# MingyuKim87/Safe_Denoiser

Hardware: AMD Instinct MI355X
Metric: images/sec (512x512, 50 steps, SD-v1.4 + repellency) (higher is better)
Workload: dtype bf16; 1 GPU; README-default end to end (safree = svf = lra = true, safree_neg_prompt_config.json:26-28): token ids -> CLIP -> SAFREE projection -> DDPM 50 steps x UNet on 3 guidance branches with per-prompt text switching + safe_denoiser.yaml repellency (kernel_fast, M=515, sigma 3.15, scale .33, margin 1.6, window 780<=t<=1000) -> VAE decode -> uint8 512x512 images; SD-v1.4 UNet / CLIP / VAE with random weigh; guidance_branches=3, text_encoder_precision=bf16x3, prompts_per_batch=64, latent_repeat=3, renoise_draws_rank0=3520, parallelism=prompt-shard x1

## Files before the change

### include/sdn.h

```cpp
#ifndef SDN_H_
#define SDN_H_

#include <stddef.h>
#include <stdint.h>

#ifdef __cplusplus
extern "C" {
#endif

#define SDN_OK            0
#define SDN_E_INVALID    -1
#define SDN_E_LAUNCH     -2
#define SDN_E_WORKSPACE  -3
#define SDN_E_ARCH       -4

int sdn_abi_version(void);
const char* sdn_device_arch_host(void);


#define SDN_REPEL_RBF     0
#define SDN_REPEL_SPARSE  1
#define SDN_QNORM_NONE    0
#define SDN_QNORM_CHANNEL 1
#define SDN_OUT_REPELLED  0
#define SDN_OUT_NEG       1

typedef struct sdn_repel_params {
  int32_t n_query;
  int32_t n_ref;
  int32_t channels;
  int32_t hw;
  int32_t weight_fn;
  int32_t qnorm;
  float   sigma;
  float   radius;
  float   scale;
  float   epsilon;
  float   gate;
} sdn_repel_params;

size_t sdn_repel_workspace_bytes(int32_t n_query, int32_t n_ref, int32_t channels, int32_t hw);

int sdn_repel_apply(const sdn_repel_params* p_host, float* x, const float* proj_ref,
                    float* out_neg, float* out_den, int32_t* out_isneg,
                    void* workspace, size_t workspace_bytes, void* stream);

int sdn_repel_calibrate(const sdn_repel_params* p_host, const float* queries, const float* proj_ref,
                        float* out, void* workspace, size_t workspace_bytes, void* stream);


int sdn_cfg_combine(const float* model_out, int32_t n_prompt, int32_t n_branch, int64_t d,
                    float guidance_scale, float* eps, void* stream);

int sdn_sld_guidance(const float* model_out, int32_t n_prompt, int64_t d, float guidance_scale,
                     float sld_guidance_scale, float sld_threshold, float sld_momentum_scale, float sld_mom_beta,
                     int32_t apply_safety, float* momentum, float* eps, void* stream);

int sdn_cfg_combine_rows(const float* model_out, int32_t n_prompt, int32_t n_branch, int64_t d,
                         const float* guidance_rows, float* eps, void* stream);
int sdn_sld_guidance_rows(const float* model_out, int32_t n_prompt, int64_t d, const float* guidance_rows,
                          float sld_guidance_scale, float sld_threshold, float sld_momentum_scale, float sld_mom_beta,
                          int32_t apply_safety, float* momentum, float* eps, void* stream);

int sdn_pred_x0(const float* x, const float* eps, int64_t n, float sqrt_ac, float sqrt_one_minus_ac,
                float clip, float* x0, void* stream);

int sdn_sched_step(const float* x, const float* eps, const float* noise, int64_t n,
                   float sqrt_ac, float sqrt_one_minus_ac, float c_x0, float c_x, float c_eps, float sigma,
                   float clip, float* prev, void* stream);

int sdn_add_noise(const float* x0, const float* noise, int64_t n, float sqrt_ac, float sqrt_one_minus_ac,
                  float* out, void* stream);

int sdn_renoise_select(float* latents, const float* x0r, const float* noise, const int32_t* isneg,
                       int32_t n_prompt, int64_t d, float sqrt_ac, float sqrt_one_minus_ac, void* stream);

int sdn_flow_euler_step(const float* x, const float* v, int64_t n, float sigma, float sigma_next,
                        float* prev, void* stream);

int sdn_flow_endpoints(const float* x, const float* v, int64_t n, float sigma, float* x0, float* x1, void* stream);
int sdn_flow_renoise(const float* x0r, const float* x1, const float* z, int64_t n, float sigma_next,
                     float* out, void* stream);


#define SDN_A_PLAIN    0
#define SDN_A_CONV3X3  1
#define SDN_ACT_NONE   0
#define SDN_ACT_SILU   1
#define SDN_ACT_GEGLU  2
#define SDN_ACT_GELU_TANH 3
#define SDN_ACT_QUICK_GELU 4
#define SDN_ACT_GEGLU_TANH 5
#define SDN_ACT_GELU      7
#define SDN_ACT_RELU      9
#define SDN_OUT_BF16      0
#define SDN_OUT_F32       1
#define SDN_OUT_F32_NCHW  2

typedef struct sdn_gemm_desc {
  int32_t M, N, K;
  int32_t a_mode;
  int32_t K1;
  int32_t Hs, Ws, Cin;
  int32_t Ho, Wo, stride;
  int32_t upsample;
  int32_t act;
  int32_t out_kind;
  int32_t rows_per_batch;
  int32_t ld_rowbias;
  int32_t ld_rowgate;
  int32_t residual_bcast;
  int32_t n_valid;
  int32_t ldc;
  int32_t asym_pad;
  int32_t split_k;
  int32_t res_pre;
  int32_t x3_out;
  int32_t f32_stream;
} sdn_gemm_desc;

int sdn_gemm_bf16(const sdn_gemm_desc* d_host, const void* a, const void* a2, const void* w,
                  const float* bias, const float* rowbias, const float* rowgate, const void* residual, void* out,
                  void* stream);
int sdn_gemm_f16(const sdn_gemm_desc* d_host, const void* a, const void* a2, const void* w,
                 const float* bias, const float* rowbias, const float* rowgate, const void* residual, void* out,
                 void* stream);

int sdn_groupnorm_bf16(const void* x, const void* x2, int32_t batch, int32_t hw, int32_t c1, int32_t c2,
                       int32_t groups, float eps, int32_t silu, const float* gamma, const float* beta,
                       void* out, float* stats_ws, void* stream);
int sdn_groupnorm_f16(const void* x, const void* x2, int32_t batch, int32_t hw, int32_t c1, int32_t c2,
                      int32_t groups, float eps, int32_t silu, const float* gamma, const float* beta,
                      void* out, float* stats_ws, void* stream);

int sdn_layernorm_bf16(const void* x, int64_t rows, int32_t c, float eps, const float* gamma,
                       const float* beta, void* out, void* stream);
int sdn_layernorm_f16(const void* x, int64_t rows, int32_t c, float eps, const float* gamma,
                      const float* beta, void* out, void* stream);

int sdn_attention_bf16(const void* q, const void* k, const void* v, void* out, int32_t batch, int32_t heads,
                       int32_t nq, int32_t nk, int32_t head_dim, int32_t ldq, int32_t ldk, int32_t ldv,
                       int32_t ldo, float scale, void* stream);
int sdn_attention_f16(const void* q, const void* k, const void* v, void* out, int32_t batch, int32_t heads,
                      int32_t nq, int32_t nk, int32_t head_dim, int32_t ldq, int32_t ldk, int32_t ldv,
                      int32_t ldo, float scale, void* stream);

typedef struct sdn_attn_segment2 {
  const void* q2; const void* k2; const void* v2; void* out2;
  int32_t n1, ldq2, ldk2, ldv2, ldo2;
} sdn_attn_segment2;
int sdn_joint_attention(int32_t dtype, const void* q, const void* k, const void* v, void* out,
                        const sdn_attn_segment2* seg2_host, int32_t batch, int32_t heads, int32_t n_total,
                        int32_t head_dim, int32_t ldq, int32_t ldk, int32_t ldv, int32_t ldo, float scale,
                        void* stream);

int sdn_layernorm_mod_bf16(const void* x, int64_t rows, int32_t c, float eps, const float* scale, const float* shift,
                           int32_t ld_mod, int32_t rows_per_batch, void* out, void* stream);
int sdn_layernorm_mod_f16(const void* x, int64_t rows, int32_t c, float eps, const float* scale, const float* shift,
                          int32_t ld_mod, int32_t rows_per_batch, void* out, void* stream);

int sdn_patchify_bf16(const float* latents, int32_t batch, int32_t c, int32_t h, int32_t w, int32_t p, void* out, void* stream);
int sdn_patchify_f16(const float* latents, int32_t batch, int32_t c, int32_t h, int32_t w, int32_t p, void* out, void* stream);
int sdn_unpatchify_f32(const float* tokens, int32_t batch, int32_t c, int32_t h, int32_t w, int32_t p, float* out, void* stream);

int sdn_conv_in_bf16(const float* latents_nchw, const void* w, const float* bias, int32_t batch, int32_t cin,
                     int32_t h, int32_t wd, int32_t cout, void* out_nhwc, void* stream);
int sdn_conv_in_f16(const float* latents_nchw, const void* w, const float* bias, int32_t batch, int32_t cin,
                    int32_t h, int32_t wd, int32_t cout, void* out_nhwc, void* stream);

int sdn_timestep_embed_bf16(float timestep, int32_t batch, int32_t dim, void* out, void* stream);
int sdn_timestep_embed_f16(float timestep, int32_t batch, int32_t dim, void* out, void* stream);

int sdn_gemm_f32(const sdn_gemm_desc* d_host, const void* a, const void* a2, const void* w,
                 const float* bias, const float* rowbias, const float* rowgate, const void* residual, void* out,
                 void* stream);
int sdn_groupnorm_f32(const void* x, const void* x2, int32_t batch, int32_t hw, int32_t c1, int32_t c2,
                      int32_t groups, float eps, int32_t silu, const float* gamma, const float* beta,
                      void* out, float* stats_ws, void* stream);
int sdn_layernorm_f32(const void* x, int64_t rows, int32_t c, float eps, const float* gamma,
                      const float* beta, void* out, void* stream);
int sdn_attention_f32(const void* q, const void* k, const void* v, void* out, int32_t batch, int32_t heads,
                      int32_t nq, int32_t nk, int32_t head_dim, int32_t ldq, int32_t ldk, int32_t ldv,
                      int32_t ldo, float scale, void* stream);
int sdn_conv_in_f32(const float* latents_nchw, const void* w, const float* bias, int32_t batch, int32_t cin,
                    int32_t h, int32_t wd, int32_t cout, void* out_nhwc, void* stream);
int sdn_timestep_embed_f32(float timestep, int32_t batch, int32_t dim, void* out, void* stream);

int sdn_gemm_x3(const sdn_gemm_desc* d_host, const void* a, const void* a2, const void* w,
                const float* bias, const float* rowbias, const float* rowgate, const void* residual, void* out,
                void* stream);
int sdn_attention_x3(const void* q, const void* k, const void* v, void* out, int32_t batch, int32_t heads,
                     int32_t nq, int32_t nk, int32_t head_dim, int32_t ldq, int32_t ldk, int32_t ldv,
                     int32_t ldo, float scale, void* stream);

int sdn_layernorm_mod_f32(const void* x, int64_t rows, int32_t c, float eps, const float* scale, const float* shift,
                          int32_t ld_mod, int32_t rows_per_batch, void* out, void* stream);
int sdn_patchify_f32(const float* latents, int32_t batch, int32_t c, int32_t h, int32_t w, int32_t p, void* out, void* stream);
int sdn_joint_attention_f32(int32_t mode, const void* q, const void* k, const void* v, void* out,
                            const sdn_attn_segment2* seg2_host, int32_t batch, int32_t heads, int32_t n_total,
                            int32_t head_dim, int32_t ldq, int32_t ldk, int32_t ldv, int32_t ldo, float scale,
                            void* stream);

int sdn_split3(const float* x, const float* x2, int64_t rows, int32_t c1, int32_t c2, void* out_triple, void* stream);
int sdn_expand3_weights(const float* w, int64_t rows, int32_t cols, int32_t group, void* out_bf16, void* stream);
int sdn_groupnorm_f32_triple(const void* x, const void* x2, int32_t batch, int32_t hw, int32_t c1, int32_t c2, int32_t groups,
                             float eps, int32_t silu, const float* gamma, const float* beta, void* out_triple, float* stats_ws,
                             void* stream);
int sdn_layernorm_f32_triple(const void* x, int64_t rows, int32_t c, float eps, const float* gamma, const float* beta,
                             void* out_triple, void* stream);
int sdn_attention_x3_triple(const void* q, const void* k, const void* v, void* out_triple, int32_t batch, int32_t heads, int32_t nq,
                            int32_t nk, int32_t head_dim, int32_t ldq, int32_t ldk, int32_t ldv, int32_t ldo, float scale,
                            void* stream);
int sdn_attention_x3_pairs(const void* q, const void* k, const void* v, int32_t lo_offset_q, int32_t lo_offset_kv, void* out,
                           int32_t batch, int32_t heads, int32_t nq, int32_t nk, int32_t head_dim, int32_t ldq, int32_t ldk,
                           int32_t ldv, int32_t ldo, float scale, int32_t triple_out, void* stream);

int sdn_randn_philox_plan(int64_t numel, int32_t* grid_out, int64_t* offset_increment_out);
int sdn_randn_philox(const uint64_t* seeds, const uint64_t* offsets, const int32_t* rows, int32_t n_gen, int64_t numel,
                     float* out, void* stream);
int sdn_randn_philox_state(const uint64_t* seeds, uint64_t* offsets, const int32_t* flags, int32_t n_gen, int64_t numel,
                           float* out, void* stream);

typedef struct sdn_unet_config {
  int32_t in_channels, out_channels, sample_size;
  int32_t n_levels;
  int32_t block_out_channels[4];
  int32_t level_has_attn[4];
  int32_t layers_per_block;
  int32_t n_heads;
  int32_t cross_dim, text_len;
  int32_t norm_groups;
  int32_t dtype;
  int32_t latent_repeat;
} sdn_unet_config;

typedef struct sdn_unet sdn_unet;

#define SDN_P_VEC_F32     0
#define SDN_P_MAT         1
#define SDN_P_CONV3X3     2
#define SDN_P_GEGLU_MAT   3
#define SDN_P_GEGLU_VEC   4
#define SDN_P_POS_CROP    5
#define SDN_P_GLU_VALUE   7
#define SDN_P_GLU_GATE    8
#define SDN_P_DERIVED     6

typedef struct sdn_param_info {
  char     name[128];
  int32_t  kind;
  int32_t  rows, cols;
  int32_t  rows_padded;
  int64_t  offset;
} sdn_param_info;

int    sdn_unet_create(const sdn_unet_config* cfg_host, sdn_unet** out_host);
void   sdn_unet_destroy(sdn_unet* u);
int    sdn_unet_param_count(const sdn_unet* u);
int    sdn_unet_param_info(const sdn_unet* u, int32_t index, sdn_param_info* info_host);
size_t sdn_unet_weight_bytes(const sdn_unet* u);
size_t sdn_unet_workspace_bytes(sdn_unet* u, int32_t batch);
double sdn_unet_flops(sdn_unet* u, int32_t batch, double* attention_core_flops_host);

int sdn_unet_forward(sdn_unet* u, const void* weights, const float* latents, float timestep, const void* text,
                     float* out, int32_t batch, void* workspace, size_t workspace_bytes, void* stream);

typedef struct sdn_mmdit_config {
  int32_t in_channels, out_channels;
  int32_t sample_size, patch_size;
  int32_t num_layers;
  int32_t num_heads, head_dim;
  int32_t joint_dim, pooled_dim;
  int32_t text_len;
  int32_t time_dim;
  int32_t dtype;
} sdn_mmdit_config;
int sdn_mmdit_create(const sdn_mmdit_config* cfg_host, sdn_unet** out_host);
int sdn_mmdit_forward(sdn_unet* m, const void* weights, const float* latents, float timestep, const void* text,
                      const void* pooled, float* out, int32_t batch, void* workspace, size_t workspace_bytes,
                      void* stream);

int sdn_ln_fold(int32_t dtype, const void* w, const float* gamma, const float* beta, const float* bias, int32_t rows,
                int32_t cols, void* w_folded, float* c, float* d, void* stream);
int sdn_gemm_ln_bf16(const sdn_gemm_desc* desc, const void* a, const void* w_folded, const float* c, const float* d, float eps,
                     const float* row_stats, void* out, void* stream);
int sdn_gemm_ln_f16(const sdn_gemm_desc* desc, const void* a, const void* w_folded, const float* c, const float* d, float eps,
                    const float* row_stats, void* out, void* stream);
int sdn_row_stats_bf16(const void* x, int64_t rows, int32_t c, float eps, float* out, void* stream);
int sdn_row_stats_f16(const void* x, int64_t rows, int32_t c, float eps, float* out, void* stream);

int sdn_ffn_geglu_fused(int32_t dtype, int64_t M, int32_t C, const void* x, const float* row_stats, const void* w1_folded,
                        const float* c1, const float* d1, const void* w_cat, const float* b_cat, const void* residual, void* out,
                        float* col_stats, void* stream);

int sdn_gemm_k320(int32_t dtype, const sdn_gemm_desc* desc, const void* a, const void* w, const float* bias, const float* ln_c,
                  const float* ln_d, float ln_eps, const void* residual, void* out, void* stream);
int32_t sdn_gemm_k320_map(int32_t grid, int32_t col_groups, int32_t wg, int32_t* stream_out, int32_t* group_out);

int sdn_gemm_stats_bf16(const sdn_gemm_desc* desc, const void* a, const void* a2, const void* w, const float* bias,
                        const float* rowbias, const void* residual, void* out, float* col_stats, void* stream);
int sdn_gemm_stats_f16(const sdn_gemm_desc* desc, const void* a, const void* a2, const void* w, const float* bias,
                       const float* rowbias, const void* residual, void* out, float* col_stats, void* stream);
int sdn_groupnorm_cols_bf16(const void* x, const void* x2, int32_t batch, int32_t hw, int32_t c1, int32_t c2, int32_t groups,
                            float eps, int32_t silu, const float* gamma, const float* beta, void* out, float* stats_ws,
                            const float* cols1, const float* cols2, void* stream);
int sdn_groupnorm_cols_f16(const void* x, const void* x2, int32_t batch, int32_t hw, int32_t c1, int32_t c2, int32_t groups,
                           float eps, int32_t silu, const float* gamma, const float* beta, void* out, float* stats_ws,
                           const float* cols1, const float* cols2, void* stream);

int sdn_gemm_splitk_bf16(const sdn_gemm_desc* d, const void* a, const void* a2, const void* w, const float* bias,
                         const float* rowbias, const float* rowgate, const void* residual, void* out, void* partials,
                         size_t partial_bytes, void* stream);
int sdn_gemm_splitk_f16(const sdn_gemm_desc* d, const void* a, const void* a2, const void* w, const float* bias,
                        const float* rowbias, const float* rowgate, const void* residual, void* out, void* partials,
                        size_t partial_bytes, void* stream);

int sdn_conv_up4_weights(int32_t dtype, const void* w9, int32_t N, int32_t Cin, void* out, void* stream);

int sdn_repeat(const void* in, size_t bytes, int32_t rep, void* out, void* stream);

int sdn_unet_prepare(sdn_unet* u, void* weights, void* stream);

typedef struct sdn_vae_config {
  int32_t latent_channels, out_channels;
  int32_t sample_size;
  int32_t n_levels;
  int32_t block_out_channels[4];
  int32_t layers_per_block;
  int32_t norm_groups;
  int32_t dtype;
} sdn_vae_config;
int sdn_vae_decoder_create(const sdn_vae_config* cfg_host, sdn_unet** out_host);
int sdn_vae_decode(sdn_unet* vae, const void* weights, const float* latents, float latent_scale, float* image,
                   int32_t batch, void* workspace, size_t workspace_bytes, void* stream);
int sdn_vae_encoder_create(const sdn_vae_config* cfg_host, sdn_unet** out_host);
int sdn_vae_encode(sdn_unet* vae_encoder, const void* weights, const float* image, float* moments, int32_t batch,
                   void* workspace, size_t workspace_bytes, void* stream);
int sdn_gaussian_sample(const float* moments, const float* noise, int32_t batch, int32_t latent_channels, int32_t hw,
                        float scale, float* out, void* stream);
int sdn_image_postprocess(const float* image_nchw, int32_t batch, int32_t channels, int32_t height, int32_t width,
                          float* out_nhwc01, uint8_t* out_nhwc_u8, void* stream);
int sdn_latent_mix(const float* z, const float* w, const float* bias, int32_t batch, int32_t channels, int32_t hw,
                   float in_scale, float* out, void* stream);
int sdn_softmax_rows(int32_t dtype, const float* scores, int64_t ld_scores, int64_t rows, int32_t n, float scale,
                     void* out, int64_t ld_out, void* stream);
int sdn_transpose16(const void* in, int32_t rows, int32_t cols, int64_t ld_in, void* out, int64_t ld_out, void* stream);
int sdn_transpose32(const void* in, int32_t rows, int32_t cols, int64_t ld_in, void* out, int64_t ld_out, void* stream);

typedef struct sdn_clip_config {
  int32_t vocab_size;
  int32_t hidden_size, intermediate_size;
  int32_t num_layers, num_heads;
  int32_t max_position_embeddings;
  int32_t dtype;
} sdn_clip_config;
int sdn_clip_create(const sdn_clip_config* cfg_host, sdn_unet** out_host);
int sdn_clip_forward(sdn_unet* clip, const void* weights, const int32_t* input_ids, const int32_t* attention_mask,
                     void* last_hidden_state, int32_t batch, void* workspace, size_t workspace_bytes, void* stream);
int sdn_clip_embed(int32_t dtype, const int32_t* input_ids, const void* token_embedding, const void* position_embedding,
                   int64_t rows, int32_t seq_len, int32_t hidden, int32_t vocab, void* out, void* stream);
int sdn_masked_attention(int32_t dtype, const void* q, const void* k, const void* v, void* out, const int32_t* key_mask,
                         int32_t causal, int32_t batch, int32_t heads, int32_t n, int32_t head_dim, int32_t ldq,
                         int32_t ldk, int32_t ldv, int32_t ldo, float scale, void* stream);
int sdn_clip_embed_f32(const int32_t* input_ids, const void* token_embedding, const void* position_embedding, int64_t rows,
                       int32_t seq_len, int32_t hidden, int32_t vocab, void* out, void* stream);
int sdn_masked_attention_f32(const void* q, const void* k, const void* v, void* out, const int32_t* key_mask, int32_t causal,
                             int32_t batch, int32_t heads, int32_t n, int32_t head_dim, int32_t ldq, int32_t ldk, int32_t ldv,
                             int32_t ldo, float scale, void* stream);

typedef struct sdn_clip_proj_config {
  int32_t vocab_size;
  int32_t hidden_size, intermediate_size;
  int32_t num_layers, num_heads;
  int32_t max_position_embeddings;
  int32_t dtype;
  int32_t projection_dim;
  int32_t act;
  int32_t eos_token_id;
  int32_t hidden_tap;
} sdn_clip_proj_config;
int sdn_clip_proj_create(const sdn_clip_proj_config* cfg_host, sdn_unet** out_host);
int sdn_clip_proj_forward(sdn_unet* clip, const void* weights, const int32_t* input_ids, void* hidden, int64_t hidden_batch_stride,
                          int64_t hidden_row_stride, void* text_embeds, int64_t embeds_row_stride, int32_t batch, void* workspace,
                          size_t workspace_bytes, void* stream);
int sdn_clip_eos_rows(int32_t dtype, const int32_t* input_ids, const void* x, const float* gamma, const float* beta, int32_t batch,
                      int32_t seq_len, int32_t hidden, int32_t vocab, int32_t eos_token_id, float eps, void* out,
                      int32_t* positions, void* stream);
int sdn_copy_rows_strided(const void* src, int32_t batch, int32_t rows_per_batch, int32_t cols, int32_t elem_bytes, void* dst,
                          int64_t dst_batch_stride, int64_t dst_row_stride, void* stream);

typedef struct sdn_clip_vision_config {
  int32_t image_size, patch_size;
  int32_t hidden_size, intermediate_size;
  int32_t num_layers, num_heads;
  int32_t projection_dim;
  int32_t act;
  int32_t dtype;
} sdn_clip_vision_config;
int sdn_clip_vision_create(const sdn_clip_vision_config* cfg_host, sdn_unet** out_host);
int sdn_clip_vision_forward(sdn_unet* vision, const void* weights, const float* pixel_values, void* last_hidden_state,
                            void* image_embeds, int32_t batch, void* workspace, size_t workspace_bytes, void* stream);
int sdn_clip_patch_rows(int32_t dtype, const float* pixels, int32_t batch, int32_t image_size, int32_t patch_size, int32_t kpad,
                        void* out, void* stream);
int sdn_clip_vision_embed(int32_t dtype, const void* patch_proj, const float* class_embedding, const void* position_embedding,
                          const float* gamma, const float* beta, int32_t batch, int32_t tokens, int32_t hidden, float eps, void* out,
                          void* stream);
int sdn_clip_class_rows(int32_t dtype, const void* x, const float* gamma, const float* beta, int32_t batch, int32_t seq_len,
                        int32_t hidden, float eps, void* out, void* stream);
int sdn_image_resize_u8(const uint8_t* in, int32_t batch, int32_t in_size, int32_t out_size, const int32_t* coeffs,
                        const int32_t* bounds, int32_t ksize, uint8_t* tmp, uint8_t* out, void* stream);
int sdn_clip_normalize_u8(const uint8_t* in, int32_t batch, int32_t size, float mean_r, float mean_g, float mean_b, float std_r,
                          float std_g, float std_b, float* out, void* stream);
int sdn_embed_row_scores(const void* x, int32_t dtype_x, int64_t ldx, const void* y, int32_t dtype_y, int64_t ldy,
                         int32_t y_rows, int32_t rows, int32_t dim, int32_t normalize_y, float scale, float bias,
                         float* out, void* stream);
int sdn_embed_cross_mean(const void* x, int32_t dtype_x, int64_t ldx, int32_t rx, const void* y, int32_t dtype_y, int64_t ldy,
                         int32_t ry, int32_t dim, float* scratch, float* out, void* stream);
int sdn_image_resize_rect_u8(const uint8_t* in, int32_t batch, int32_t in_h, int32_t in_w, int32_t out_h, int32_t out_w,
                             const int32_t* coeffs_x, const int32_t* bounds_x, int32_t ksize_x, const int32_t* coeffs_y,
                             const int32_t* bounds_y, int32_t ksize_y, uint8_t* tmp, uint8_t* out_u8, float* out_f32, float mean_r,
                             float mean_g, float mean_b, float std_r, float std_g, float std_b, void* stream);

typedef struct sdn_t5_config {
  int32_t vocab_size;
  int32_t d_model, d_kv, d_ff;
  int32_t num_layers, num_heads;
  int32_t num_buckets, max_distance;
  float   eps;
  int32_t dtype;
} sdn_t5_config;
int sdn_t5_create(const sdn_t5_config* cfg_host, sdn_unet** out_host);
size_t sdn_t5_workspace_bytes(sdn_unet* t5, int32_t batch, int32_t n);
double sdn_t5_flops(sdn_unet* t5, int32_t batch, int32_t n, double* attention_core_flops_host);
int sdn_t5_forward(sdn_unet* t5, const void* weights, const int32_t* input_ids, const int32_t* attention_mask, int32_t n,
                   void* out, int32_t batch, void* workspace, size_t workspace_bytes, void* stream);
int sdn_rmsnorm(int32_t dtype, const void* x, int32_t x_is_f32, int64_t rows, int32_t c, float eps, const float* weight, void* out,
                void* stream);
int sdn_embed_tokens(int32_t dtype, const int32_t* input_ids, const void* token_embedding, int64_t rows, int32_t hidden,
                     int32_t vocab, float* out, void* stream);
int sdn_t5_bucket(int32_t relative_position, int32_t num_buckets, int32_t max_distance);
int sdn_t5_relative_bias(int32_t dtype, const void* table, int32_t num_buckets, int32_t max_distance, int32_t heads, int32_t n,
                         float* out, void* stream);
int sdn_bias_attention(int32_t dtype, const void* q, const void* k, const void* v, void* out, const float* bias,
                       const int32_t* key_mask, int32_t batch, int32_t heads, int32_t n, int32_t head_dim, int32_t ldq,
                       int32_t ldk, int32_t ldv, int32_t ldo, float scale, void* stream);

void sdn_unet_set_text_version(sdn_unet* u, uint64_t version);

void sdn_unet_set_graph_mode(sdn_unet* u, int32_t on);
void sdn_unet_set_split_k(sdn_unet* u, int32_t on);
void sdn_unet_set_conv_up4(sdn_unet* u, int32_t on);

typedef struct sdn_inception_config {
  int32_t image_size;
  int32_t normalize_input;
  int32_t dtype;
} sdn_inception_config;
typedef struct sdn_inception_conv {
  char    name[64];
  int32_t cin, cout, kh, kw, stride, pad_h, pad_w;
  int32_t kpad, n_padded;
} sdn_inception_conv;
int sdn_inception_create(const sdn_inception_config* cfg_host, sdn_unet** out_host);
int sdn_inception_conv_count(const sdn_unet* inception);
int sdn_inception_conv_info(const sdn_unet* inception, int32_t index, sdn_inception_conv* info_host);
int sdn_inception_forward(sdn_unet* inception, const void* weights, const float* pixels, float* features, int32_t batch, int32_t h,
                          int32_t w, int32_t resize, void* workspace, size_t workspace_bytes, void* stream);
#define SDN_POOL_MAX        0
#define SDN_POOL_AVG_NOPAD  1
int sdn_patch_rows_f32(const float* in, int32_t batch, int32_t h, int32_t w, int32_t c, int32_t kh, int32_t kw, int32_t stride_h,
                       int32_t stride_w, int32_t pad_h, int32_t pad_w, int32_t kpad, float* out, void* stream);
int sdn_pool3_f32(int32_t mode, const float* in, int32_t batch, int32_t h, int32_t w, int32_t c, int32_t stride, int32_t pad,
                  float* out, int32_t ldo, int32_t c0, void* stream);
int sdn_resize_bilinear_f32(const float* in_nchw, int32_t batch, int32_t h, int32_t w, int32_t out_h, int32_t out_w, float scale,
                            float shift, float* out_nhwc, void* stream);
int sdn_spatial_mean_f32(const float* in, int32_t batch, int32_t hw, int32_t c, float* out, void* stream);

typedef struct sdn_profile_row {
  char    kernel[24];
  int32_t launches;
  double  ms;
  double  flops;
  double  bytes;
} sdn_profile_row;
void sdn_unet_profile_next(sdn_unet* u);
int  sdn_unet_profile_read(sdn_unet* u, sdn_profile_row* rows_host, int32_t max_rows);

#ifdef __cplusplus
}
#endif
#endif
```

### safe_denoiser_amd/_lib.py

```python
from __future__ import annotations

import ctypes as C
import os

import torch

_HERE = os.path.dirname(os.path.abspath(__file__))
_LIB = None


class SdnUnavailable(RuntimeError):
    """libsdn.so is missing/unloadable, or there is no gfx950 device for a compute call."""


class SdnError(RuntimeError):
    """A libsdn entry point returned a negative status."""


_ERR = {-1: "SDN_E_INVALID (bad shape / null or misaligned pointer)", -2: "SDN_E_LAUNCH", -3: "SDN_E_WORKSPACE",
        -4: "SDN_E_ARCH"}


def lib_path() -> str:
    return os.environ.get("SDN_LIB", os.path.join(_HERE, "libsdn.so"))


class RepelParams(C.Structure):
    _fields_ = [("n_query", C.c_int32), ("n_ref", C.c_int32), ("channels", C.c_int32), ("hw", C.c_int32),
                ("weight_fn", C.c_int32), ("qnorm", C.c_int32), ("sigma", C.c_float), ("radius", C.c_float),
                ("scale", C.c_float), ("epsilon", C.c_float), ("gate", C.c_float)]


class GemmDesc(C.Structure):
    _fields_ = [(n, C.c_int32) for n in ("M", "N", "K", "a_mode", "K1", "Hs", "Ws", "Cin", "Ho", "Wo", "stride",
                                         "upsample", "act", "out_kind", "rows_per_batch", "ld_rowbias", "ld_rowgate",
                                         "residual_bcast", "n_valid", "ldc", "asym_pad", "split_k", "res_pre", "x3_out",
                                         "f32_stream")]


class UnetConfig(C.Structure):
    _fields_ = [("in_channels", C.c_int32), ("out_channels", C.c_int32), ("sample_size", C.c_int32),
                ("n_levels", C.c_int32), ("block_out_channels", C.c_int32 * 4), ("level_has_attn", C.c_int32 * 4),
                ("layers_per_block", C.c_int32), ("n_heads", C.c_int32), ("cross_dim", C.c_int32),
                ("text_len", C.c_int32), ("norm_groups", C.c_int32), ("dtype", C.c_int32), ("latent_repeat", C.c_int32)]


class ProfileRow(C.Structure):
    _fields_ = [("kernel", C.c_char * 24), ("launches", C.c_int32), ("ms", C.c_double), ("flops", C.c_double),
                ("bytes", C.c_double)]


class MmditConfig(C.Structure):
    _fields_ = [(n, C.c_int32) for n in ("in_channels", "out_channels", "sample_size", "patch_size", "num_layers",
                                         "num_heads", "head_dim", "joint_dim", "pooled_dim", "text_len", "time_dim",
                                         "dtype")]


class VaeConfig(C.Structure):
    _fields_ = [("latent_channels", C.c_int32), ("out_channels", C.c_int32), ("sample_size", C.c_int32),
                ("n_levels", C.c_int32), ("block_out_channels", C.c_int32 * 4), ("layers_per_block", C.c_int32),
                ("norm_groups", C.c_int32), ("dtype", C.c_int32)]


class ClipConfig(C.Structure):
    _fields_ = [(n, C.c_int32) for n in ("vocab_size", "hidden_size", "intermediate_size", "num_layers", "num_heads",
                                         "max_position_embeddings", "dtype")]


class ClipProjConfig(C.Structure):
    _fields_ = [(n, C.c_int32) for n in ("vocab_size", "hidden_size", "intermediate_size", "num_layers", "num_heads",
                                         "max_position_embeddings", "dtype", "projection_dim", "act", "eos_token_id", "hidden_tap")]


class ClipVisionConfig(C.Structure):
    _fields_ = [(n, C.c_int32) for n in ("image_size", "patch_size", "hidden_size", "intermediate_size", "num_layers", "num_heads",
                                         "projection_dim", "act", "dtype")]


class InceptionConfig(C.Structure):
    _fields_ = [(n, C.c_int32) for n in ("image_size", "normalize_input", "dtype")]


class InceptionConv(C.Structure):
    _fields_ = [("name", C.c_char * 64)] + [(n, C.c_int32) for n in ("cin", "cout", "kh", "kw", "stride", "pad_h", "pad_w", "kpad",
                                                                     "n_padded")]


class T5Config(C.Structure):
    _fields_ = [(n, C.c_int32) for n in ("vocab_size", "d_model", "d_kv", "d_ff", "num_layers", "num_heads", "num_buckets",
                                         "max_distance")] + [("eps", C.c_float), ("dtype", C.c_int32)]


class AttnSegment2(C.Structure):
    _fields_ = [("q2", C.c_void_p), ("k2", C.c_void_p), ("v2", C.c_void_p), ("out2", C.c_void_p), ("n1", C.c_int32),
                ("ldq2", C.c_int32), ("ldk2", C.c_int32), ("ldv2", C.c_int32), ("ldo2", C.c_int32)]


class ParamInfo(C.Structure):
    _fields_ = [("name", C.c_char * 128), ("kind", C.c_int32), ("rows", C.c_int32), ("cols", C.c_int32),
                ("rows_padded", C.c_int32), ("offset", C.c_int64)]


_vp, _i32, _i64, _f32, _sz = C.c_void_p, C.c_int32, C.c_int64, C.c_float, C.c_size_t

SIGNATURES = {
    "sdn_abi_version": (C.c_int, []),
    "sdn_device_arch_host": (C.c_char_p, []),
    "sdn_repel_workspace_bytes": (_sz, [_i32, _i32, _i32, _i32]),
    "sdn_repel_apply": (C.c_int, [C.POINTER(RepelParams), _vp, _vp, _vp, _vp, _vp, _vp, _sz, _vp]),
    "sdn_repel_calibrate": (C.c_int, [C.POINTER(RepelParams), _vp, _vp, _vp, _vp, _sz, _vp]),
    "sdn_cfg_combine": (C.c_int, [_vp, _i32, _i32, _i64, _f32, _vp, _vp]),
    "sdn_sld_guidance": (C.c_int, [_vp, _i32, _i64, _f32, _f32, _f32, _f32, _f32, _i32, _vp, _vp, _vp]),
    "sdn_cfg_combine_rows": (C.c_int, [_vp, _i32, _i32, _i64, _vp, _vp, _vp]),
    "sdn_sld_guidance_rows": (C.c_int, [_vp, _i32, _i64, _vp, _f32, _f32, _f32, _f32, _i32, _vp, _vp, _vp]),
    "sdn_pred_x0": (C.c_int, [_vp, _vp, _i64, _f32, _f32, _f32, _vp, _vp]),
    "sdn_sched_step": (C.c_int, [_vp, _vp, _vp, _i64, _f32, _f32, _f32, _f32, _f32, _f32, _f32, _vp, _vp]),
    "sdn_add_noise": (C.c_int, [_vp, _vp, _i64, _f32, _f32, _vp, _vp]),
    "sdn_renoise_select": (C.c_int, [_vp, _vp, _vp, _vp, _i32, _i64, _f32, _f32, _vp]),
    "sdn_flow_euler_step": (C.c_int, [_vp, _vp, _i64, _f32, _f32, _vp, _vp]),
    "sdn_flow_endpoints": (C.c_int, [_vp, _vp, _i64, _f32, _vp, _vp, _vp]),
    "sdn_flow_renoise": (C.c_int, [_vp, _vp, _vp, _i64, _f32, _vp, _vp]),
    "sdn_gemm_bf16": (C.c_int, [C.POINTER(GemmDesc), _vp, _vp, _vp, _vp, _vp, _vp, _vp, _vp, _vp]),
    "sdn_gemm_f16": (C.c_int, [C.POINTER(GemmDesc), _vp, _vp, _vp, _vp, _vp, _vp, _vp, _vp, _vp]),
    "sdn_ln_fold": (C.c_int, [_i32, _vp, _vp, _vp, _vp, _i32, _i32, _vp, _vp, _vp, _vp]),
    "sdn_gemm_ln_bf16": (C.c_int, [C.POINTER(GemmDesc), _vp, _vp, _vp, _vp, _f32, _vp, _vp, _vp]),
    "sdn_gemm_ln_f16": (C.c_int, [C.POINTER(GemmDesc), _vp, _vp, _vp, _vp, _f32, _vp, _vp, _vp]),
    "sdn_row_stats_bf16": (C.c_int, [_vp, _i64, _i32, _f32, _vp, _vp]),
    "sdn_row_stats_f16": (C.c_int, [_vp, _i64, _i32, _f32, _vp, _vp]),
    "sdn_ffn_geglu_fused": (C.c_int, [_i32, _i64, _i32, _vp, _vp, _vp, _vp, _vp, _vp, _vp, _vp, _vp, _vp, _vp]),
    "sdn_gemm_k320": (C.c_int, [_i32, C.POINTER(GemmDesc), _vp, _vp, _vp, _vp, _vp, _f32, _vp, _vp, _vp]),
    "sdn_gemm_k320_map": (_i32, [_i32, _i32, _i32, C.POINTER(_i32), C.POINTER(_i32)]),
    "sdn_gemm_stats_bf16": (C.c_int, [C.POINTER(GemmDesc), _vp, _vp, _vp, _vp, _vp, _vp, _vp, _vp, _vp]),
    "sdn_gemm_stats_f16": (C.c_int, [C.POINTER(GemmDesc), _vp, _vp, _vp, _vp, _vp, _vp, _vp, _vp, _vp]),
    "sdn_groupnorm_cols_bf16": (C.c_int, [_vp, _vp, _i32, _i32, _i32, _i32, _i32, _f32, _i32, _vp, _vp, _vp, _vp, _vp, _vp, _vp]),
    "sdn_groupnorm_cols_f16": (C.c_int, [_vp, _vp, _i32, _i32, _i32, _i32, _i32, _f32, _i32, _vp, _vp, _vp, _vp, _vp, _vp, _vp]),
    "sdn_gemm_splitk_bf16": (C.c_int, [C.POINTER(GemmDesc), _vp, _vp, _vp, _vp, _vp, _vp, _vp, _vp, _vp, _sz, _vp]),
    "sdn_gemm_splitk_f16": (C.c_int, [C.POINTER(GemmDesc), _vp, _vp, _vp, _vp, _vp, _vp, _vp, _vp, _vp, _sz, _vp]),
    "sdn_groupnorm_bf16": (C.c_int, [_vp, _vp, _i32, _i32, _i32, _i32, _i32, _f32, _i32, _vp, _vp, _vp, _vp, _vp]),
    "sdn_groupnorm_f16": (C.c_int, [_vp, _vp, _i32, _i32, _i32, _i32, _i32, _f32, _i32, _vp, _vp, _vp, _vp, _vp]),
    "sdn_layernorm_f16": (C.c_int, [_vp, _i64, _i32, _f32, _vp, _vp, _vp, _vp]),
    "sdn_conv_in_f16": (C.c_int, [_vp, _vp, _vp, _i32, _i32, _i32, _i32, _i32, _vp, _vp]),
    "sdn_timestep_embed_f16": (C.c_int, [_f32, _i32, _i32, _vp, _vp]),
    "sdn_layernorm_bf16": (C.c_int, [_vp, _i64, _i32, _f32, _vp, _vp, _vp, _vp]),
    "sdn_attention_bf16": (C.c_int, [_vp, _vp, _vp, _vp, _i32, _i32, _i32, _i32, _i32, _i32, _i32, _i32, _i32, _f32,
                                     _vp]),
    "sdn_attention_f16": (C.c_int, [_vp, _vp, _vp, _vp, _i32, _i32, _i32, _i32, _i32, _i32, _i32, _i32, _i32, _f32,
                                    _vp]),
    "sdn_conv_in_bf16": (C.c_int, [_vp, _vp, _vp, _i32, _i32, _i32, _i32, _i32, _vp, _vp]),
    "sdn_timestep_embed_bf16": (C.c_int, [_f32, _i32, _i32, _vp, _vp]),
    "sdn_gemm_f32": (C.c_int, [C.POINTER(GemmDesc), _vp, _vp, _vp, _vp, _vp, _vp, _vp, _vp, _vp]),
    "sdn_groupnorm_f32": (C.c_int, [_vp, _vp, _i32, _i32, _i32, _i32, _i32, _f32, _i32, _vp, _vp, _vp, _vp, _vp]),
    "sdn_layernorm_f32": (C.c_int, [_vp, _i64, _i32, _f32, _vp, _vp, _vp, _vp]),
    "sdn_attention_f32": (C.c_int, [_vp, _vp, _vp, _vp, _i32, _i32, _i32, _i32, _i32, _i32, _i32, _i32, _i32, _f32, _vp]),
    "sdn_randn_philox_plan": (C.c_int, [C.c_int64, C.POINTER(C.c_int32), C.POINTER(C.c_int64)]),
    "sdn_randn_philox": (C.c_int, [_vp, _vp, _vp, _i32, C.c_int64, _vp, _vp]),
    "sdn_randn_philox_state": (C.c_int, [_vp, _vp, _vp, _i32, C.c_int64, _vp, _vp]),
    "sdn_gemm_x3": (C.c_int, [C.POINTER(GemmDesc), _vp, _vp, _vp, _vp, _vp, _vp, _vp, _vp, _vp]),
    "sdn_attention_x3": (C.c_int, [_vp, _vp, _vp, _vp, _i32, _i32, _i32, _i32, _i32, _i32, _i32, _i32, _i32, _f32, _vp]),
    "sdn_conv_in_f32": (C.c_int, [_vp, _vp, _vp, _i32, _i32, _i32, _i32, _i32, _vp, _vp]),
    "sdn_timestep_embed_f32": (C.c_int, [_f32, _i32, _i32, _vp, _vp]),
    "sdn_unet_create": (C.c_int, [C.POINTER(UnetConfig), C.POINTER(_vp)]),
    "sdn_unet_destroy": (None, [_vp]),
    "sdn_unet_param_count": (C.c_int, [_vp]),
    "sdn_unet_param_info": (C.c_int, [_vp, _i32, C.POINTER(ParamInfo)]),
    "sdn_unet_weight_bytes": (_sz, [_vp]),
    "sdn_unet_workspace_bytes": (_sz, [_vp, _i32]),
    "sdn_unet_flops": (C.c_double, [_vp, _i32, C.POINTER(C.c_double)]),
    "sdn_unet_forward": (C.c_int, [_vp, _vp, _vp, _f32, _vp, _vp, _i32, _vp, _sz, _vp]),
    "sdn_mmdit_create": (C.c_int, [C.POINTER(MmditConfig), C.POINTER(_vp)]),
    "sdn_mmdit_forward": (C.c_int, [_vp, _vp, _vp, _f32, _vp, _vp, _vp, _i32, _vp, _sz, _vp]),
    "sdn_joint_attention": (C.c_int, [_i32, _vp, _vp, _vp, _vp, C.POINTER(AttnSegment2), _i32, _i32, _i32, _i32, _i32,
                                      _i32, _i32, _i32, _f32, _vp]),
    "sdn_layernorm_mod_bf16": (C.c_int, [_vp, _i64, _i32, _f32, _vp, _vp, _i32, _i32, _vp, _vp]),
    "sdn_layernorm_mod_f16": (C.c_int, [_vp, _i64, _i32, _f32, _vp, _vp, _i32, _i32, _vp, _vp]),
    "sdn_patchify_bf16": (C.c_int, [_vp, _i32, _i32, _i32, _i32, _i32, _vp, _vp]),
    "sdn_patchify_f16": (C.c_int, [_vp, _i32, _i32, _i32, _i32, _i32, _vp, _vp]),
    "sdn_unpatchify_f32": (C.c_int, [_vp, _i32, _i32, _i32, _i32, _i32, _vp, _vp]),
    "sdn_layernorm_mod_f32": (C.c_int, [_vp, _i64, _i32, _f32, _vp, _vp, _i32, _i32, _vp, _vp]),
    "sdn_patchify_f32": (C.c_int, [_vp, _i32, _i32, _i32, _i32, _i32, _vp, _vp]),
    "sdn_joint_attention_f32": (C.c_int, [_i32, _vp, _vp, _vp, _vp, C.POINTER(AttnSegment2), _i32, _i32, _i32, _i32, _i32,
                                          _i32, _i32, _i32, _f32, _vp]),
    "sdn_repeat": (C.c_int, [_vp, _sz, _i32, _vp, _vp]),
    "sdn_vae_decoder_create": (C.c_int, [C.POINTER(VaeConfig), C.POINTER(_vp)]),
    "sdn_vae_decode": (C.c_int, [_vp, _vp, _vp, _f32, _vp, _i32, _vp, _sz, _vp]),
    "sdn_vae_encoder_create": (C.c_int, [C.POINTER(VaeConfig), C.POINTER(_vp)]),
    "sdn_vae_encode": (C.c_int, [_vp, _vp, _vp, _vp, _i32, _vp, _sz, _vp]),
    "sdn_gaussian_sample": (C.c_int, [_vp, _vp, _i32, _i32, _i32, _f32, _vp, _vp]),
    "sdn_image_postprocess": (C.c_int, [_vp, _i32, _i32, _i32, _i32, _vp, _vp, _vp]),
    "sdn_latent_mix": (C.c_int, [_vp, _vp, _vp, _i32, _i32, _i32, _f32, _vp, _vp]),
    "sdn_softmax_rows": (C.c_int, [_i32, _vp, _i64, _i64, _i32, _f32, _vp, _i64, _vp]),
    "sdn_transpose16": (C.c_int, [_vp, _i32, _i32, _i64, _vp, _i64, _vp]),
    "sdn_transpose32": (C.c_int, [_vp, _i32, _i32, _i64, _vp, _i64, _vp]),
    "sdn_clip_create": (C.c_int, [C.POINTER(ClipConfig), C.POINTER(_vp)]),
    "sdn_clip_forward": (C.c_int, [_vp, _vp, _vp, _vp, _vp, _i32, _vp, _sz, _vp]),
    "sdn_clip_embed": (C.c_int, [_i32, _vp, _vp, _vp, _i64, _i32, _i32, _i32, _vp, _vp]),
    "sdn_masked_attention": (C.c_int, [_i32, _vp, _vp, _vp, _vp, _vp, _i32, _i32, _i32, _i32, _i32, _i32, _i32, _i32, _i32,
                                       _f32, _vp]),
    "sdn_clip_proj_create": (C.c_int, [C.POINTER(ClipProjConfig), C.POINTER(_vp)]),
    "sdn_clip_proj_forward": (C.c_int, [_vp, _vp, _vp, _vp, _i64, _i64, _vp, _i64, _i32, _vp, _sz, _vp]),
    "sdn_clip_eos_rows": (C.c_int, [_i32, _vp, _vp, _vp, _vp, _i32, _i32, _i32, _i32, _i32, _f32, _vp, _vp, _vp]),
    "sdn_copy_rows_strided": (C.c_int, [_vp, _i32, _i32, _i32, _i32, _vp, _i64, _i64, _vp]),
    "sdn_clip_vision_create": (C.c_int, [C.POINTER(ClipVisionConfig), C.POINTER(_vp)]),
    "sdn_clip_vision_forward": (C.c_int, [_vp, _vp, _vp, _vp, _vp, _i32, _vp, _sz, _vp]),
    "sdn_clip_patch_rows": (C.c_int, [_i32, _vp, _i32, _i32, _i32, _i32, _vp, _vp]),
    "sdn_clip_vision_embed": (C.c_int, [_i32, _vp, _vp, _vp, _vp, _vp, _i32, _i32, _i32, _f32, _vp, _vp]),
    "sdn_clip_class_rows": (C.c_int, [_i32, _vp, _vp, _vp, _i32, _i32, _i32, _f32, _vp, _vp]),
    "sdn_image_resize_u8": (C.c_int, [_vp, _i32, _i32, _i32, _vp, _vp, _i32, _vp, _vp, _vp]),
    "sdn_clip_normalize_u8": (C.c_int, [_vp, _i32, _i32, _f32, _f32, _f32, _f32, _f32, _f32, _vp, _vp]),
    "sdn_image_resize_rect_u8": (C.c_int, [_vp, _i32, _i32, _i32, _i32, _i32, _vp, _vp, _i32, _vp, _vp, _i32, _vp, _vp, _vp, _f32, _f32,
                                           _f32, _f32, _f32, _f32, _vp]),
    "sdn_inception_create": (C.c_int, [C.POINTER(InceptionConfig), C.POINTER(_vp)]),
    "sdn_inception_conv_count": (C.c_int, [_vp]),
    "sdn_inception_conv_info": (C.c_int, [_vp, _i32, C.POINTER(InceptionConv)]),
    "sdn_inception_forward": (C.c_int, [_vp, _vp, _vp, _vp, _i32, _i32, _i32, _i32, _vp, _sz, _vp]),
    "sdn_patch_rows_f32": (C.c_int, [_vp, _i32, _i32, _i32, _i32, _i32, _i32, _i32, _i32, _i32, _i32, _i32, _vp, _vp]),
    "sdn_pool3_f32": (C.c_int, [_i32, _vp, _i32, _i32, _i32, _i32, _i32, _i32, _vp, _i32, _i32, _vp]),
    "sdn_resize_bilinear_f32": (C.c_int, [_vp, _i32, _i32, _i32, _i32, _i32, _f32, _f32, _vp, _vp]),
    "sdn_spatial_mean_f32": (C.c_int, [_vp, _i32, _i32, _i32, _vp, _vp]),
    "sdn_embed_row_scores": (C.c_int, [_vp, _i32, _i64, _vp, _i32, _i64, _i32, _i32, _i32, _i32, _f32, _f32, _vp, _vp]),
    "sdn_embed_cross_mean": (C.c_int, [_vp, _i32, _i64, _i32, _vp, _i32, _i64, _i32, _i32, _vp, _vp, _vp]),
    "sdn_t5_create": (C.c_int, [C.POINTER(T5Config), C.POINTER(_vp)]),
    "sdn_t5_workspace_bytes": (_sz, [_vp, _i32, _i32]),
    "sdn_t5_flops": (C.c_double, [_vp, _i32, _i32, C.POINTER(C.c_double)]),
    "sdn_t5_forward": (C.c_int, [_vp, _vp, _vp, _vp, _i32, _vp, _i32, _vp, _sz, _vp]),
    "sdn_rmsnorm": (C.c_int, [_i32, _vp, _i32, _i64, _i32, _f32, _vp, _vp, _vp]),
    "sdn_embed_tokens": (C.c_int, [_i32, _vp, _vp, _i64, _i32, _i32, _vp, _vp]),
    "sdn_t5_bucket": (C.c_int, [_i32, _i32, _i32]),
    "sdn_t5_relative_bias": (C.c_int, [_i32, _vp, _i32, _i32, _i32, _i32, _vp, _vp]),
    "sdn_bias_attention": (C.c_int, [_i32, _vp, _vp, _vp, _vp, _vp, _vp, _i32, _i32, _i32, _i32, _i32, _i32, _i32, _i32, _f32,
                                     _vp]),
    "sdn_split3": (C.c_int, [_vp, _vp, _i64, _i32, _i32, _vp, _vp]),
    "sdn_expand3_weights": (C.c_int, [_vp, _i64, _i32, _i32, _vp, _vp]),
    "sdn_groupnorm_f32_triple": (C.c_int, [_vp, _vp, _i32, _i32, _i32, _i32, _i32, _f32, _i32, _vp, _vp, _vp, _vp, _vp]),
    "sdn_layernorm_f32_triple": (C.c_int, [_vp, _i64, _i32, _f32, _vp, _vp, _vp, _vp]),
    "sdn_attention_x3_triple": (C.c_int, [_vp, _vp, _vp, _vp, _i32, _i32, _i32, _i32, _i32, _i32, _i32, _i32, _i32, _f32, _vp]),
    "sdn_attention_x3_pairs": (C.c_int, [_vp, _vp, _vp, _i32, _i32, _vp, _i32, _i32, _i32, _i32, _i32, _i32, _i32, _i32, _i32, _f32, _i32, _vp]),
    "sdn_clip_embed_f32": (C.c_int, [_vp, _vp, _vp, _i64, _i32, _i32, _i32, _vp, _vp]),
    "sdn_masked_attention_f32": (C.c_int, [_vp, _vp, _vp, _vp, _vp, _i32, _i32, _i32, _i32, _i32, _i32, _i32, _i32, _i32, _f32, _vp]),
    "sdn_unet_prepare": (C.c_int, [_vp, _vp, _vp]),
    "sdn_unet_set_graph_mode": (None, [_vp, _i32]),
    "sdn_unet_set_text_version": (None, [_vp, C.c_uint64]),
    "sdn_unet_set_split_k": (None, [_vp, _i32]),
    "sdn_unet_set_conv_up4": (None, [_vp, _i32]),
    "sdn_conv_up4_weights": (C.c_int, [_i32, _vp, _i32, _i32, _vp, _vp]),
    "sdn_unet_profile_next": (None, [_vp]),
    "sdn_unet_profile_read": (C.c_int, [_vp, C.POINTER(ProfileRow), _i32]),
}


def lib():
    global _LIB
    if _LIB is None:
        path = lib_path()
        if not os.path.exists(path):
            raise SdnUnavailable(f"{path} not found: build it with `python -c 'import __graft_entry__ as g; g.build()'` "
                                 f"(or `make -C safe_denoiser_amd/csrc`).  There is no CPU fallback.")
        try:
            handle = C.CDLL(path)
        except OSError as e:
            raise SdnUnavailable(f"cannot load {path}: {e}") from e
        for name, (res, args) in SIGNATURES.items():
            fn = getattr(handle, name)
            fn.restype, fn.argtypes = res, args
        _LIB = handle
    return _LIB


def check(rc: int, what: str):
    if rc != 0:
        raise SdnError(f"{what} failed: {_ERR.get(rc, rc)}")


def require_gpu():
    if not torch.cuda.is_available():
        raise SdnUnavailable("no GPU visible: the safe-denoiser hot path only runs on an MI355X (gfx950); "
                             "there is no CPU fallback")


def dptr(t: torch.Tensor | None, dtype=None) -> int | None:
    if t is None:
        return None
    if not t.is_cuda:
        raise SdnUnavailable("tensor is not on the GPU: libsdn takes device pointers only (no CPU fallback)")
    if not t.is_contiguous():
        raise SdnError("tensor must be contiguous")
    if dtype is not None and t.dtype != dtype:
        raise SdnError(f"expected {dtype}, got {t.dtype}")
    return t.data_ptr()


def stream_ptr() -> int:
    return torch.cuda.current_stream().cuda_stream
```

### safe_denoiser_amd/csrc/sdn_norm.hip

```cpp
#include "sdn_common.h"
#include "sdn_ops.h"

namespace sdn_norm_detail {

typedef __attribute__((ext_vector_type(4))) unsigned int u32x4;
constexpr int THREADS = 256;
constexpr int GN_MAX_TILES = 128;

template <typename T>
__device__ __forceinline__ void unpack8(const u32x4 v, float* f) {
  f[0] = T::to_f(v.x & 0xffff); f[1] = T::to_f(v.x >> 16); f[2] = T::to_f(v.y & 0xffff); f[3] = T::to_f(v.y >> 16);
  f[4] = T::to_f(v.z & 0xffff); f[5] = T::to_f(v.z >> 16); f[6] = T::to_f(v.w & 0xffff); f[7] = T::to_f(v.w >> 16);
}
template <typename T>
__device__ __forceinline__ u32x4 pack8(const float* f) {
  return (u32x4){T::pack2(f[0], f[1]), T::pack2(f[2], f[3]), T::pack2(f[4], f[5]), T::pack2(f[6], f[7])};
}
__device__ __forceinline__ float silu_f(float v) { return v / (1.f + __expf(-v)); }

template <typename T>
__global__ void __launch_bounds__(THREADS)
k_gn_stats(const unsigned short* __restrict__ x, const unsigned short* __restrict__ x2, int hw, int c1, int c2,
           int groups, int rows_per_tile, int ct, int nch, float* __restrict__ partials) {
  extern __shared__ float lds[];
  const int C = c1 + c2, cpg = C / groups;
  const int b = blockIdx.x, tile = blockIdx.y, ntiles = gridDim.y;
  const int rt = THREADS / ct;
  const int cl = threadIdx.x % ct, rl = threadIdx.x / ct;
  const int r_lo = tile * rows_per_tile, r_hi = min(hw, r_lo + rows_per_tile);
  if (rl < rt) {
    for (int q = 0; q < nch; ++q) {
      const int ch0 = (cl + q * ct) * 8;
      const unsigned short* src; int ld, cc;
      if (ch0 < c1) { src = x; ld = c1; cc = ch0; } else { src = x2; ld = c2; cc = ch0 - c1; }
      float s[8], ss[8];
#pragma unroll
      for (int e = 0; e < 8; ++e) { s[e] = 0.f; ss[e] = 0.f; }
      for (int r = r_lo + rl; r < r_hi; r += 4 * rt) {
        u32x4 v[4];
#pragma unroll
        for (int j = 0; j < 4; ++j) {
          const int rr = min(r + j * rt, r_hi - 1);
          v[j] = *reinterpret_cast<const u32x4*>(src + ((long)b * hw + rr) * ld + cc);
        }
#pragma unroll
        for (int j = 0; j < 4; ++j) {
          if (r + j * rt < r_hi) {
            float f[8];
            unpack8<T>(v[j], f);
#pragma unroll
            for (int e = 0; e < 8; ++e) { s[e] += f[e]; ss[e] = fmaf(f[e], f[e], ss[e]); }
          }
        }
      }
#pragma unroll
      for (int e = 0; e < 8; ++e) {
        lds[((long)rl * C + ch0 + e) * 2 + 0] = s[e];
        lds[((long)rl * C + ch0 + e) * 2 + 1] = ss[e];
      }
    }
  }
  __syncthreads();
  if (threadIdx.x < groups) {
    const int gidx = threadIdx.x;
    float s = 0.f, ss = 0.f;
    for (int r = 0; r < rt; ++r)
      for (int c = gidx * cpg; c < (gidx + 1) * cpg; ++c) {
        s += lds[((long)r * C + c) * 2 + 0];
        ss += lds[((long)r * C + c) * 2 + 1];
      }
    float* o = partials + (((long)b * ntiles + tile) * groups + gidx) * 2;
    o[0] = s; o[1] = ss;
  }
}

__global__ void __launch_bounds__(512)
k_gn_finalize(const float* __restrict__ partials, int ntiles, int groups, float n, float eps,
              float* __restrict__ stats) {
  __shared__ float sh[64][8][2];
  const int b = blockIdx.x, gi = threadIdx.x >> 3, part = threadIdx.x & 7;
  if (gi < groups) {
    float s = 0.f, ss = 0.f;
    for (int t = part; t < ntiles; t += 8) {
      const float* p = partials + (((long)b * ntiles + t) * groups + gi) * 2;
      s += p[0]; ss += p[1];
    }
    sh[gi][part][0] = s; sh[gi][part][1] = ss;
  }
  __syncthreads();
  if (gi < groups && part == 0) {
    float s = 0.f, ss = 0.f;
#pragma unroll
    for (int k = 0; k < 8; ++k) { s += sh[gi][k][0]; ss += sh[gi][k][1]; }
    const float mean = s / n;
    const float var = fmaxf(ss / n - mean * mean, 0.f);
    stats[((long)b * groups + gi) * 2 + 0] = mean;
    stats[((long)b * groups + gi) * 2 + 1] = rsqrtf(var + eps);
  }
}

__global__ void __launch_bounds__(256)
k_gn_finalize_cols(const float* __restrict__ cols1, const float* __restrict__ cols2, int blocks_per_sample, int c1, int c2,
                   int groups, float n, float eps, float* __restrict__ stats) {
  __shared__ float red[8];
  const int C = c1 + c2, cpg = C / groups, b = blockIdx.x, gi = blockIdx.y;
  const int total = blocks_per_sample * cpg;
  float s = 0.f, q = 0.f;
  for (int e = threadIdx.x; e < total; e += 256) {
    const int t = e / cpg, c = gi * cpg + (e - t * cpg);
    const bool second = c >= c1;
    const float* src = second ? cols2 : cols1;
    const int cw = second ? c2 : c1, cc = second ? c - c1 : c;
    const float2 v = *reinterpret_cast<const float2*>(src + 2 * (((long)b * blocks_per_sample + t) * cw + cc));
    s += v.x; q += v.y;
  }
  s = block_sum<4>(s, red);
  q = block_sum<4>(q, red + 4);
  if (threadIdx.x == 0) {
    const float mean = s / n;
    const float var = fmaxf(q / n - mean * mean, 0.f);
    stats[((long)b * groups + gi) * 2 + 0] = mean;
    stats[((long)b * groups + gi) * 2 + 1] = rsqrtf(var + eps);
  }
}

template <typename T>
__global__ void __launch_bounds__(THREADS)
k_gn_apply(const unsigned short* __restrict__ x, const unsigned short* __restrict__ x2, int hw, int c1, int c2,
           int groups, int rows_per_block, int silu, const float* __restrict__ gamma,
           const float* __restrict__ beta, const float* __restrict__ stats, unsigned short* __restrict__ out) {
  extern __shared__ float aff[];
  const int C = c1 + c2, cpg = C / groups, cchunks = C / 8;
  const int b = blockIdx.x;
  float* ca = aff; float* cb = aff + C;
  for (int c = threadIdx.x; c < C; c += THREADS) {
    const int gi = c / cpg;
    const float mean = stats[((long)b * groups + gi) * 2 + 0], rstd = stats[((long)b * groups + gi) * 2 + 1];
    const float a = rstd * gamma[c];
    ca[c] = a; cb[c] = beta[c] - mean * a;
  }
  __syncthreads();
  const int r_lo = blockIdx.y * rows_per_block, r_hi = min(hw, r_lo + rows_per_block);
  const long total = (long)(r_hi - r_lo) * cchunks;
  for (long e = threadIdx.x; e < total; e += THREADS) {
    const int r = r_lo + (int)(e / cchunks), ch0 = (int)(e % cchunks) * 8;
    const unsigned short* src; int ld, cc;
    if (ch0 < c1) { src = x; ld = c1; cc = ch0; } else { src = x2; ld = c2; cc = ch0 - c1; }
    const u32x4 v = *reinterpret_cast<const u32x4*>(src + ((long)b * hw + r) * ld + cc);
    float f[8];
    unpack8<T>(v, f);
    const float4 a0 = *reinterpret_cast<const float4*>(ca + ch0), a1 = *reinterpret_cast<const float4*>(ca + ch0 + 4);
    const float4 b0 = *reinterpret_cast<const float4*>(cb + ch0), b1 = *reinterpret_cast<const float4*>(cb + ch0 + 4);
    const float am[8] = {a0.x, a0.y, a0.z, a0.w, a1.x, a1.y, a1.z, a1.w};
    const float bm[8] = {b0.x, b0.y, b0.z, b0.w, b1.x, b1.y, b1.z, b1.w};
#pragma unroll
    for (int k = 0; k < 8; ++k) {
      const float y = fmaf(f[k], am[k], bm[k]);
      f[k] = silu ? silu_f(y) : y;
    }
    *reinterpret_cast<u32x4*>(out + ((long)b * hw + r) * C + ch0) = pack8<T>(f);
  }
}

template <typename T, int NQ, int R>
__global__ void __launch_bounds__(THREADS)
k_layernorm(const unsigned short* __restrict__ x, long rows, int C, float eps, const float* __restrict__ gamma,
            const float* __restrict__ beta, unsigned short* __restrict__ out, int mod, int rows_per_batch, int ld_mod) {
  const int lane = threadIdx.x & 63;
  const long row0 = ((long)blockIdx.x * 4 + (threadIdx.x >> 6)) * R;
  if (row0 >= rows) return;
  const int cchunks = C / 8;
  float f[R][NQ][8];
  float s[R];
#pragma unroll
  for (int r = 0; r < R; ++r) {
    s[r] = 0.f;
    const long row = row0 + r < rows ? row0 + r : rows - 1;
#pragma unroll
    for (int q = 0; q < NQ; ++q) {
      const int cc = lane + q * 64;
      if (cc < cchunks) {
        unpack8<T>(*reinterpret_cast<const u32x4*>(x + row * C + cc * 8), f[r][q]);
#pragma unroll
        for (int k = 0; k < 8; ++k) s[r] += f[r][q][k];
      }
    }
  }
  float mean[R], rstd[R];
#pragma unroll
  for (int r = 0; r < R; ++r) mean[r] = wave_sum(s[r]) / (float)C;
#pragma unroll
  for (int r = 0; r < R; ++r) {
    float ss = 0.f;
#pragma unroll
    for (int q = 0; q < NQ; ++q) {
      const int cc = lane + q * 64;
      if (cc < cchunks) {
#pragma unroll
        for (int k = 0; k < 8; ++k) { const float d = f[r][q][k] - mean[r]; ss = fmaf(d, d, ss); }
      }
    }
    s[r] = ss;
  }
#pragma unroll
  for (int r = 0; r < R; ++r) rstd[r] = rsqrtf(wave_sum(s[r]) / (float)C + eps);
#pragma unroll
  for (int q = 0; q < NQ; ++q) {
    const int cc = lane + q * 64;
    if (cc < cchunks) {
      float gm[8], bt[8];
      auto load_affine = [&](const float* gp, const float* bp) {
        const float4 g0 = *reinterpret_cast<const float4*>(gp + cc * 8), g1 = *reinterpret_cast<const float4*>(gp + cc * 8 + 4);
        const float4 b0 = *reinterpret_cast<const float4*>(bp + cc * 8), b1 = *reinterpret_cast<const float4*>(bp + cc * 8 + 4);
        gm[0] = g0.x; gm[1] = g0.y; gm[2] = g0.z; gm[3] = g0.w; gm[4] = g1.x; gm[5] = g1.y; gm[6] = g1.z; gm[7] = g1.w;
        bt[0] = b0.x; bt[1] = b0.y; bt[2] = b0.z; bt[3] = b0.w; bt[4] = b1.x; bt[5] = b1.y; bt[6] = b1.z; bt[7] = b1.w;
      };
      if (!mod) load_affine(gamma, beta);
#pragma unroll
      for (int r = 0; r < R; ++r) {
        const long row = row0 + r;
        if (row < rows) {
          if (mod) {
            const long b = row / rows_per_batch;
            load_affine(gamma + b * ld_mod, beta + b * ld_mod);
          }
          float y[8];
#pragma unroll
          for (int k = 0; k < 8; ++k) y[k] = (f[r][q][k] - mean[r]) * rstd[r] * (mod ? 1.f + gm[k] : gm[k]) + bt[k];
          *reinterpret_cast<u32x4*>(out + row * C + cc * 8) = pack8<T>(y);
        }
      }
    }
  }
}

template <typename T, int NQ, int R>
__global__ void __launch_bounds__(THREADS)
k_row_stats(const unsigned short* __restrict__ x, long rows, int C, float eps, float* __restrict__ out) {
  const int lane = threadIdx.x & 63;
  const long row0 = ((long)blockIdx.x * 4 + (threadIdx.x >> 6)) * R;
  if (row0 >= rows) return;
  const int cchunks = C / 8;
  float f[R][NQ][8];
  float s[R];
#pragma unroll
  for (int r = 0; r < R; ++r) {
    s[r] = 0.f;
    const long row = row0 + r < rows ? row0 + r : rows - 1;
#pragma unroll
    for (int q = 0; q < NQ; ++q) {
      const int cc = lane + q * 64;
      if (cc < cchunks) {
        unpack8<T>(*reinterpret_cast<const u32x4*>(x + row * C + cc * 8), f[r][q]);
#pragma unroll
        for (int k = 0; k < 8; ++k) s[r] += f[r][q][k];
      }
    }
  }
  float mean[R];
#pragma unroll
  for (int r = 0; r < R; ++r) mean[r] = wave_sum(s[r]) / (float)C;
#pragma unroll
  for (int r = 0; r < R; ++r) {
    float ss = 0.f;
#pragma unroll
    for (int q = 0; q < NQ; ++q) {
      const int cc = lane + q * 64;
      if (cc < cchunks) {
#pragma unroll
        for (int k = 0; k < 8; ++k) { const float d = f[r][q][k] - mean[r]; ss = fmaf(d, d, ss); }
      }
    }
    s[r] = ss;
  }
#pragma unroll
  for (int r = 0; r < R; ++r) {
    const float rstd = rsqrtf(wave_sum(s[r]) / (float)C + eps);
    if (lane == 0 && row0 + r < rows) *reinterpret_cast<float2*>(out + 2 * (row0 + r)) = make_float2(mean[r], rstd);
  }
}

template <typename T>
__global__ void __launch_bounds__(THREADS)
k_conv_in(const float* __restrict__ lat, const unsigned short* __restrict__ w, const float* __restrict__ bias,
          int B, int cin, int H, int W, int cout, int ldo, unsigned short* __restrict__ out) {
  extern __shared__ float wl[];
  const int kk = 9 * cin;
  for (int i = threadIdx.x; i < cout * kk; i += THREADS) {
    const int co = i / kk, k = i - co * kk;
    wl[((k * 2 + ((co >> 2) & 1)) * (cout / 8) + (co >> 3)) * 4 + (co & 3)] = T::to_f(w[i]);
  }
  __syncthreads();
  constexpr int PX = 4;
  const int cchunks = cout / 8;
  const int WQ = (W + PX - 1) / PX;
  const int total = B * H * WQ * cchunks;
  const int HWQ = H * WQ;
  for (int e = blockIdx.x * THREADS + threadIdx.x; e < total; e += gridDim.x * THREADS) {
    const int pq = e / cchunks, cc = e - pq * cchunks;
    const int b = pq / HWQ, rem = pq - b * HWQ;
    const int yh = rem / WQ, x0 = (rem - yh * WQ) * PX;
    float acc[PX][8];
    {
      const float4 b0 = *reinterpret_cast<const float4*>(bias + cc * 8), b1 = *reinterpret_cast<const float4*>(bias + cc * 8 + 4);
#pragma unroll
      for (int p = 0; p < PX; ++p) {
        acc[p][0] = b0.x; acc[p][1] = b0.y; acc[p][2] = b0.z; acc[p][3] = b0.w;
        acc[p][4] = b1.x; acc[p][5] = b1.y; acc[p][6] = b1.z; acc[p][7] = b1.w;
      }
    }
    const float* lb = lat + (long)b * cin * H * W;
    for (int c = 0; c < cin; ++c) {
      float v[3][PX + 2];
#pragma unroll
      for (int ty = 0; ty < 3; ++ty)
#pragma unroll
        for (int tx = 0; tx < PX + 2; ++tx) {
          const int iy = yh + ty - 1, ix = x0 + tx - 1;
          const bool ok = iy >= 0 && iy < H && ix >= 0 && ix < W;
          const float t = lb[((long)c * H + min(max(iy, 0), H - 1)) * W + min(max(ix, 0), W - 1)];
          v[ty][tx] = ok ? t : 0.f;
        }
#pragma unroll
      for (int tap = 0; tap < 9; ++tap) {
        const float4 w0 = *reinterpret_cast<const float4*>(&wl[(((tap * cin + c) * 2 + 0) * cchunks + cc) * 4]);
        const float4 w1 = *reinterpret_cast<const float4*>(&wl[(((tap * cin + c) * 2 + 1) * cchunks + cc) * 4]);
#pragma unroll
        for (int p = 0; p < PX; ++p) {
          const float x = v[tap / 3][tap % 3 + p];
          acc[p][0] = fmaf(x, w0.x, acc[p][0]); acc[p][1] = fmaf(x, w0.y, acc[p][1]);
          acc[p][2] = fmaf(x, w0.z, acc[p][2]); acc[p][3] = fmaf(x, w0.w, acc[p][3]);
          acc[p][4] = fmaf(x, w1.x, acc[p][4]); acc[p][5] = fmaf(x, w1.y, acc[p][5]);
          acc[p][6] = fmaf(x, w1.z, acc[p][6]); acc[p][7] = fmaf(x, w1.w, acc[p][7]);
        }
      }
    }
    const long pix0 = ((long)b * H + yh) * W + x0;
#pragma unroll
    for (int p = 0; p < PX; ++p)
      if (x0 + p < W) *reinterpret_cast<u32x4*>(out + (pix0 + p) * ldo + cc * 8) = pack8<T>(acc[p]);
  }
}

template <typename T>
__global__ void k_temb(float t_val, const float* __restrict__ t_dev, int B, int dim, unsigned short* __restrict__ out) {
  const float t = t_dev ? *t_dev : t_val;
  const int half = dim / 2;
  for (int i = blockIdx.x * blockDim.x + threadIdx.x; i < B * dim; i += gridDim.x * blockDim.x) {
    const int k = i % dim;
    const int kk = k < half ? k : k - half;
    const float f = expf(-9.210340371976184f * (float)kk / (float)half);
    const float a = t * f;
    const float v = k < half ? cosf(a) : sinf(a);
    out[i] = (unsigned short)(T::pack2(v, 0.f) & 0xffff);
  }
}

inline bool al16(const void* p) { return (reinterpret_cast<uintptr_t>(p) & 15) == 0; }


template <typename T>
int groupnorm_impl(const void* x, const void* x2, int32_t batch, int32_t hw, int32_t c1, int32_t c2, int32_t groups,
                   float eps, int32_t silu, const float* gamma, const float* beta, void* out, float* stats_ws,
                   void* stream, const float* cols1 = nullptr, const float* cols2 = nullptr) {
  if (!x || !gamma || !beta || !out || !stats_ws || batch < 0 || hw <= 0 || c1 <= 0 || c2 < 0 || groups <= 0 ||
      groups > 64)
    return SDN_E_INVALID;
  if (c2 > 0 && !x2) return SDN_E_INVALID;
  const int C = c1 + c2;
  if ((c1 & 7) || (c2 & 7) || C % groups != 0 || C > 4096) return SDN_E_INVALID;
  if (!al16(x) || (x2 && !al16(x2)) || !al16(out) || !al16(gamma) || !al16(beta)) return SDN_E_INVALID;
  if (batch == 0) return SDN_OK;
  const int cch = C / 8;
  int nch = (cch + THREADS - 1) / THREADS;
  while (cch % nch != 0) ++nch;
  const int ct = cch / nch;
  if (ct > THREADS) return SDN_E_INVALID;
  const int rt = THREADS / ct;
  int ntiles = (hw + 31) / 32;
  if (ntiles > GN_MAX_TILES) ntiles = GN_MAX_TILES;
  const int rows_per_tile = (hw + ntiles - 1) / ntiles;
  ntiles = (hw + rows_per_tile - 1) / rows_per_tile;
  hipStream_t st = (hipStream_t)stream;
  const size_t lds = (size_t)rt * C * 2 * sizeof(float);
  if (lds > 64 * 1024) return SDN_E_INVALID;
  if (cols1) {
    if ((hw & 127) || (c2 > 0 && !cols2)) return SDN_E_INVALID;
    record_norm_launch({2, T::kDtype, 0, 0, 0, 0, 0, 0, 0, 0, 1, 0});
    hipLaunchKernelGGL(k_gn_finalize_cols, dim3(batch, groups), dim3(256), 0, st, cols1, cols2, hw / 128, c1, c2, groups,
                       (float)hw * (float)(C / groups), eps, stats_ws);
  } else {
    float* partials = stats_ws + (size_t)batch * groups * 2;
    record_norm_launch({1, T::kDtype, 0, 0, nch, ct, ntiles, rows_per_tile, 0, 0, 0, 0});
    hipLaunchKernelGGL((k_gn_stats<T>), dim3(batch, ntiles), dim3(THREADS), lds, st, (const unsigned short*)x,
                       (const unsigned short*)x2, hw, c1, c2, groups, rows_per_tile, ct, nch, partials);
    hipLaunchKernelGGL(k_gn_finalize, dim3(batch), dim3(512), 0, st, partials, ntiles, groups,
                       (float)hw * (float)(C / groups), eps, stats_ws);
  }
  int rows_per_block = (256 * 8 * 16) / C;
  if (rows_per_block < 1) rows_per_block = 1;
  const int nblk = (hw + rows_per_block - 1) / rows_per_block;
  hipLaunchKernelGGL((k_gn_apply<T>), dim3(batch, nblk), dim3(THREADS), (size_t)2 * C * sizeof(float), st, (const unsigned short*)x,
                     (const unsigned short*)x2, hw, c1, c2, groups, rows_per_block, silu, gamma, beta, stats_ws,
                     (unsigned short*)out);
  return sdn_launch_status();
}

template <typename T>
int layernorm_impl(const void* x, int64_t rows, int32_t c, float eps, const float* gamma, const float* beta, void* out,
                   void* stream, int mod = 0, int rows_per_batch = 0, int ld_mod = 0) {
  if (!x || !gamma || !beta || !out || rows < 0 || c <= 0 || (c & 7) || c > 2048) return SDN_E_INVALID;
  if (!al16(x) || !al16(out) || !al16(gamma) || !al16(beta)) return SDN_E_INVALID;
  if (mod && (rows_per_batch <= 0 || ld_mod < c || (ld_mod & 3))) return SDN_E_INVALID;
  if (rows == 0) return SDN_OK;
#define SDN_LN_LAUNCH(NQ, R)                                                                                          \
  do { hipLaunchKernelGGL((k_layernorm<T, NQ, R>), dim3((unsigned)((rows + 4 * (R) - 1) / (4 * (R)))), dim3(THREADS), 0,      \
                     (hipStream_t)stream, (const unsigned short*)x, (long)rows, c, eps, gamma, beta, (unsigned short*)out, \
                     mod, rows_per_batch, ld_mod);                                                                     \
  record_norm_launch({mod ? 4 : 3, T::kDtype, NQ, R, 0, 0, 0, 0, 0, 0, 0, 0}); } while (0)
  if (c <= 512) SDN_LN_LAUNCH(1, 4);
  else if (c <= 1024) SDN_LN_LAUNCH(2, 2);
  else SDN_LN_LAUNCH(4, 1);
#undef SDN_LN_LAUNCH
  return sdn_launch_status();
}

template <typename T>
__global__ void __launch_bounds__(THREADS)
k_patchify(const float* __restrict__ lat, int B, int C, int H, int W, int p, unsigned short* __restrict__ out) {
  const int hp = H / p, wp = W / p, K = C * p * p;
  const long total = (long)B * hp * wp * K;
  for (long e = (long)blockIdx.x * THREADS + threadIdx.x; e < total; e += (long)gridDim.x * THREADS) {
    const int k = (int)(e % K);
    const long tok = e / K;
    const int px = k % p, py = (k / p) % p, c = k / (p * p);
    const int tx = (int)(tok % wp), ty = (int)((tok / wp) % hp), b = (int)(tok / ((long)wp * hp));
    const float v = lat[(((long)b * C + c) * H + ty * p + py) * W + tx * p + px];
    out[e] = (unsigned short)(T::pack2(v, 0.f) & 0xffff);
  }
}
__global__ void __launch_bounds__(THREADS)
k_unpatchify(const float* __restrict__ tok, int B, int C, int H, int W, int p, float* __restrict__ out) {
  const int hp = H / p, wp = W / p;
  const long total = (long)B * C * H * W;
  for (long e = (long)blockIdx.x * THREADS + threadIdx.x; e < total; e += (long)gridDim.x * THREADS) {
    const int x = (int)(e % W), y = (int)((e / W) % H), c = (int)((e / ((long)W * H)) % C), b = (int)(e / ((long)W * H * C));
    const long t = ((long)b * hp + y / p) * wp + x / p;
    out[e] = tok[t * (p * p * C) + ((y % p) * p + (x % p)) * C + c];
  }
}
template <typename T>
int patchify_impl(const float* lat, int32_t B, int32_t C, int32_t H, int32_t W, int32_t p, void* out, void* stream) {
  if (!lat || !out || B < 0 || C <= 0 || H <= 0 || W <= 0 || p <= 0 || H % p || W % p) return SDN_E_INVALID;
  if (B == 0) return SDN_OK;
  const long total = (long)B * C * H * W;
  long grid = (total + THREADS - 1) / THREADS;
  if (grid > 2048) grid = 2048;
  hipLaunchKernelGGL((k_patchify<T>), dim3((unsigned)grid), dim3(THREADS), 0, (hipStream_t)stream, lat, B, C, H, W, p,
                     (unsigned short*)out);
  return sdn_launch_status();
}

template <typename T>
int conv_in_impl(const float* lat, const void* w, const float* bias, int32_t batch, int32_t cin, int32_t h, int32_t wd,
                 int32_t cout, void* out, void* stream) {
  if (!lat || !w || !bias || !out || batch < 0 || cin <= 0 || cin > 16 || h <= 0 || wd <= 0 || cout <= 0 ||
      (cout & 7) || !al16(out))
    return SDN_E_INVALID;
  if (batch == 0) return SDN_OK;
  int chunk = (int)((64 * 1024) / ((size_t)9 * cin * sizeof(float))) & ~7;
  if (chunk < 8) return SDN_E_INVALID;
  if (chunk > cout) chunk = cout;
  if ((long)batch * h * wd * (chunk / 8) >= (1L << 31)) return SDN_E_INVALID;
  for (int co0 = 0; co0 < cout; co0 += chunk) {
    const int cc = cout - co0 < chunk ? cout - co0 : chunk;
    const size_t lds = (size_t)cc * 9 * cin * sizeof(float);
    const long total = (long)batch * h * ((wd + 3) / 4) * (cc / 8);
    long grid = (total + THREADS - 1) / THREADS;
    if (grid > 4096) grid = 4096;
    hipLaunchKernelGGL((k_conv_in<T>), dim3((unsigned)grid), dim3(THREADS), lds, (hipStream_t)stream, lat,
                       (const unsigned short*)w + (size_t)co0 * 9 * cin, bias + co0, batch, cin, h, wd, cc, cout,
                       (unsigned short*)out + co0);
  }
  return sdn_launch_status();
}

template <typename T>
int temb_impl(float timestep, int32_t batch, int32_t dim, void* out, void* stream, const float* t_dev = nullptr) {
  if (!out || batch < 0 || dim <= 0 || (dim & 1)) return SDN_E_INVALID;
  if (batch == 0) return SDN_OK;
  const int n = batch * dim;
  hipLaunchKernelGGL((k_temb<T>), dim3((n + 255) / 256), dim3(256), 0, (hipStream_t)stream, timestep, t_dev, batch, dim,
                     (unsigned short*)out);
  return sdn_launch_status();
}

template <typename T>
int row_stats_impl(const void* x, int64_t rows, int32_t c, float eps, float* out, void* stream) {
  if (!x || !out || rows < 0 || c <= 0 || (c & 7) || c > 2048 || !al16(x) || (reinterpret_cast<uintptr_t>(out) & 7)) return SDN_E_INVALID;
  if (rows == 0) return SDN_OK;
#define SDN_RS_LAUNCH(NQ, R)                                                                                          \
  do { hipLaunchKernelGGL((k_row_stats<T, NQ, R>), dim3((unsigned)((rows + 4 * (R) - 1) / (4 * (R)))), dim3(THREADS), 0,      \
                     (hipStream_t)stream, (const unsigned short*)x, (long)rows, c, eps, out);                            \
  record_norm_launch({5, T::kDtype, NQ, R, 0, 0, 0, 0, 0, 0, 0, 0}); } while (0)
  if (c <= 512) SDN_RS_LAUNCH(1, 4);
  else if (c <= 1024) SDN_RS_LAUNCH(2, 2);
  else SDN_RS_LAUNCH(4, 1);
#undef SDN_RS_LAUNCH
  return sdn_launch_status();
}

}

int sdn_temb_from_device(int dtype, const float* t_dev, int batch, int dim, void* out, void* stream) {
  if (!t_dev) return SDN_E_INVALID;
  return dtype == 1 ? sdn_norm_detail::temb_impl<SdnF16>(0.f, batch, dim, out, stream, t_dev)
                    : sdn_norm_detail::temb_impl<SdnBF16>(0.f, batch, dim, out, stream, t_dev);
}
namespace { __global__ void k_set_scalar(float* dst, float v) { *dst = v; } }
int sdn_set_scalar(float* dst, float v, void* stream) {
  if (!dst) return SDN_E_INVALID;
  hipLaunchKernelGGL(k_set_scalar, dim3(1), dim3(1), 0, (hipStream_t)stream, dst, v);
  return sdn_launch_status();
}
using namespace sdn_norm_detail;

static int g_last_norm_launch[SDN_NL_COUNT] = {0};
void record_norm_launch(const sdn_norm_launch& l) {
  const int v[SDN_NL_COUNT] = {l.kernel, l.dtype, l.nq, l.r, l.nch, l.ct, l.ntiles, l.rows_per_tile, l.rpc, l.nchunk, l.stats_src, l.triple};
  for (int i = 0; i < SDN_NL_COUNT; ++i) g_last_norm_launch[i] = v[i];
}
extern "C" void sdn_debug_norm_last_launch(int* out, int n) {
  for (int i = 0; out && i < n; ++i) out[i] = i < SDN_NL_COUNT ? g_last_norm_launch[i] : 0;
}

#define SDN_NORM_ENTRY(SUF, T)                                                                                          \
  extern "C" int sdn_groupnorm_##SUF(const void* x, const void* x2, int32_t batch, int32_t hw, int32_t c1, int32_t c2, \
                                     int32_t groups, float eps, int32_t silu, const float* gamma, const float* beta,   \
                                     void* out, float* stats_ws, void* stream) {                                        \
    return groupnorm_impl<T>(x, x2, batch, hw, c1, c2, groups, eps, silu, gamma, beta, out, stats_ws, stream);         \
  }                                                                                                                     \
  extern "C" int sdn_groupnorm_cols_##SUF(const void* x, const void* x2, int32_t batch, int32_t hw, int32_t c1,         \
                                          int32_t c2, int32_t groups, float eps, int32_t silu, const float* gamma,      \
                                          const float* beta, void* out, float* stats_ws, const float* cols1,            \
                                          const float* cols2, void* stream) {                                           \
    if (!cols1) return SDN_E_INVALID;                                                                                   \
    return groupnorm_impl<T>(x, x2, batch, hw, c1, c2, groups, eps, silu, gamma, beta, out, stats_ws, stream, cols1,    \
                             cols2);                                                                                    \
  }                                                                                                                     \
  extern "C" int sdn_layernorm_##SUF(const void* x, int64_t rows, int32_t c, float eps, const float* gamma,            \
                                     const float* beta, void* out, void* stream) {                                      \
    return layernorm_impl<T>(x, rows, c, eps, gamma, beta, out, stream);                                                \
  }                                                                                                                     \
  extern "C" int sdn_layernorm_mod_##SUF(const void* x, int64_t rows, int32_t c, float eps, const float* scale,        \
                                         const float* shift, int32_t ld_mod, int32_t rows_per_batch, void* out,        \
                                         void* stream) {                                                                \
    return layernorm_impl<T>(x, rows, c, eps, scale, shift, out, stream, 1, rows_per_batch, ld_mod);                    \
  }                                                                                                                     \
  extern "C" int sdn_patchify_##SUF(const float* lat, int32_t B, int32_t C, int32_t H, int32_t W, int32_t p, void* out, \
                                    void* stream) {                                                                     \
    return patchify_impl<T>(lat, B, C, H, W, p, out, stream);                                                           \
  }                                                                                                                     \
  extern "C" int sdn_conv_in_##SUF(const float* lat, const void* w, const float* bias, int32_t batch, int32_t cin,     \
                                   int32_t h, int32_t wd, int32_t cout, void* out, void* stream) {                      \
    return conv_in_impl<T>(lat, w, bias, batch, cin, h, wd, cout, out, stream);                                         \
  }                                                                                                                     \
  extern "C" int sdn_timestep_embed_##SUF(float timestep, int32_t batch, int32_t dim, void* out, void* stream) {       \
    return temb_impl<T>(timestep, batch, dim, out, stream);                                                             \
  }
SDN_NORM_ENTRY(bf16, SdnBF16)
SDN_NORM_ENTRY(f16, SdnF16)

extern "C" int sdn_row_stats_bf16(const void* x, int64_t rows, int32_t c, float eps, float* out, void* stream) {
  return sdn_norm_detail::row_stats_impl<SdnBF16>(x, rows, c, eps, out, stream);
}
extern "C" int sdn_row_stats_f16(const void* x, int64_t rows, int32_t c, float eps, float* out, void* stream) {
  return sdn_norm_detail::row_stats_impl<SdnF16>(x, rows, c, eps, out, stream);
}

extern "C" int sdn_unpatchify_f32(const float* tok, int32_t B, int32_t C, int32_t H, int32_t W, int32_t p, float* out,
                                  void* stream) {
  if (!tok || !out || B < 0 || C <= 0 || H <= 0 || W <= 0 || p <= 0 || H % p || W % p) return SDN_E_INVALID;
  if (B == 0) return SDN_OK;
  const long total = (long)B * C * H * W;
  long grid = (total + THREADS - 1) / THREADS;
  if (grid > 2048) grid = 2048;
  hipLaunchKernelGGL(k_unpatchify, dim3((unsigned)grid), dim3(THREADS), 0, (hipStream_t)stream, tok, B, C, H, W, p, out);
  return sdn_launch_status();
}
```

### safe_denoiser_amd/csrc/sdn_plan.h

```cpp
#pragma once
#include <stdio.h>
#include <string.h>

#include <map>
#include <set>
#include <string>
#include <tuple>
#include <vector>

#include "sdn_common.h"
#include "sdn_ops.h"

namespace sdn_plan {

enum ModelKind { UNET, MMDIT, VAE_DECODER, VAE_ENCODER, CLIP, CLIP_PROJ, T5, CLIP_VISION, INCEPTION };

enum Space { SP_NONE = 0, SP_W = 1, SP_WS = 2, SP_IN = 3, SP_TEXT = 4, SP_OUT = 5, SP_POOLED = 6, SP_KV = 7, SP_OUT2 = 8 };
struct Ref { int space = SP_NONE; int64_t off = 0; };

struct Call {
  const void* weights; void* workspace; size_t workspace_bytes; int32_t batch; void* stream;
  const void *in = nullptr, *text = nullptr, *pooled = nullptr;
  void *out = nullptr, *out2 = nullptr;
  float scalar = 0.f; int n = 0;
  const int32_t* mask = nullptr;
  int64_t out_bs = 0, out_rs = 0, out2_rs = 0;
  int64_t kv_base = 0;
  int in_h = 0, in_w = 0;
  Call(const void* w, void* ws, size_t ws_bytes, int32_t b, void* s) : weights(w), workspace(ws), workspace_bytes(ws_bytes), batch(b), stream(s) {}
  const char* operator()(const Ref& r) const {
    switch (r.space) {
      case SP_W: return (const char*)weights + r.off;
      case SP_WS: return (const char*)workspace + r.off;
      case SP_KV: return (const char*)workspace + kv_base + r.off;
      case SP_IN: return (const char*)in + r.off;
      case SP_TEXT: return (const char*)text + r.off;
      case SP_OUT: return (const char*)out + r.off;
      case SP_OUT2: return (const char*)out2 + r.off;
      case SP_POOLED: return (const char*)pooled + r.off;
      default: return nullptr;
    }
  }
};

enum OpKind { OP_TEMB, OP_CONV_IN, OP_GEMM, OP_GN, OP_LN, OP_ATTN, OP_PATCHIFY, OP_UNPATCHIFY, OP_LATENT_MIX, OP_SOFTMAX,
              OP_TRANSPOSE, OP_GAUSS, OP_REPEAT, OP_CLIP_EMBED, OP_MATTN, OP_ROWSTATS, OP_FFN, OP_SPLIT3,
              OP_RMSNORM, OP_EMBED, OP_T5_BIAS, OP_BATTN, OP_EOS_ROWS, OP_COPY_ROWS, OP_PATCH_ROWS, OP_VISION_EMBED, OP_CLASS_ROWS,
              OP_CONV_ROWS, OP_POOL3, OP_RESIZE, OP_SPATIAL_MEAN };

struct Op {
  int kind;
  sdn_gemm_desc gd;
  Ref a, a2, w, bias, rowbias, rowgate, residual, out, aux;
  Ref q2, k2, v2, out2;
  Ref col, cols1, cols2;
  Ref ln_c, ln_d, ln_stats;
  int ln = 0;
  int text_kv = 0;
  int x3t = 0;
  int pair_in = 0;
  int tri_out = 0;
  int dyn_ldc = 0;
  int k320 = 0;
  int n1 = 0, mod = 0, ld_mod = 0, patch = 0;
  int batch = 0, hw = 0, c1 = 0, c2 = 0, groups = 0, silu = 0;
  float eps = 0.f;
  int64_t rows = 0;
  int heads = 0, nq = 0, nk = 0, hd = 0, ldq = 0, ldk = 0, ldv = 0, ldo = 0;
  float scale = 0.f;
  Ref k, v;
  int kh = 0, kw = 0, sh = 0, sw = 0, ph = 0, pw = 0;
  char label[24] = {0};
  double flops = 0.0;
  double bytes = 0.0;
};

struct Arena {
  std::map<int64_t, int64_t> free_;
  int64_t top = 0, peak = 0;
  static int64_t up(int64_t v) { return (v + 255) & ~(int64_t)255; }
  int64_t alloc(int64_t bytes) {
    bytes = up(bytes);
    for (auto it = free_.begin(); it != free_.end(); ++it) {
      if (it->second >= bytes) {
        const int64_t off = it->first, rest = it->second - bytes;
        free_.erase(it);
        if (rest > 0) free_[off + bytes] = rest;
        return off;
      }
    }
    if (!free_.empty()) {
      auto last = std::prev(free_.end());
      if (last->first + last->second == top) {
        const int64_t off = last->first;
        free_.erase(last);
        top = off + bytes;
        if (top > peak) peak = top;
        return off;
      }
    }
    const int64_t off = top;
    top += bytes;
    if (top > peak) peak = top;
    return off;
  }
  void release(int64_t off, int64_t bytes) {
    bytes = up(bytes);
    auto it = free_.emplace(off, bytes).first;
    auto nx = std::next(it);
    if (nx != free_.end() && it->first + it->second == nx->first) { it->second += nx->second; free_.erase(nx); }
    if (it != free_.begin()) {
      auto pv = std::prev(it);
      if (pv->first + pv->second == it->first) { pv->second += it->second; free_.erase(it); }
    }
  }
};

struct Act {
  int64_t off = -1, bytes = 0; int C = 0, hw = 0, side = 0;
  int64_t content = 0;
  int64_t st_off = -1, st_bytes = 0;
};

struct Plan {
  int batch = 0;
  int64_t tscalar_off = -1;
  std::vector<Op> ops;
  int64_t ws_bytes = 0;
  int64_t kv_base = 0;
  double flops = 0.0, attn_flops = 0.0;
};

}

struct sdn_unet {
  sdn_plan::ModelKind kind = sdn_plan::UNET;
  sdn_unet_config cfg;
  sdn_mmdit_config mcfg;
  sdn_vae_config vcfg;
  sdn_clip_config ccfg;
  sdn_clip_proj_config pcfg;
  sdn_t5_config tcfg;
  sdn_clip_vision_config vis;
  sdn_inception_config icfg;
  std::vector<sdn_inception_conv> convs;
  std::vector<sdn_param_info> params;
  std::map<std::string, int> param_index;
  int64_t weight_bytes = 0;
  std::map<int, sdn_plan::Plan> plans;
  int tproj_total = 0;
  int64_t subbatch_bytes = 0;
  bool profile_next = false;
  bool use_graph = false;
  bool gn_fuse = true;
  bool ln_fold = true;
  int ln_prepass_all = 0;
  bool ff_fuse = true;
  bool ffn_own_stats = true;
  bool ffn_fuse = true;
  struct FoldJob { int64_t w, gamma, beta, bias, wf, c, d; int rows, cols; int kind = 0; int group = 0; };
  std::vector<FoldJob> fold_jobs;
  uint64_t text_version = 0, kv_version = 0;
  int kv_batch = 0;
  const void *kv_w = nullptr, *kv_text = nullptr, *kv_ws = nullptr;
  bool x3_pairs = true;
  bool res_pre = true;
  bool gemm_k320 = true;
  bool x3_expand = true;
  bool split_k = false;
  bool conv_up4 = true;
  struct GraphKey {
    int batch; const void *w, *lat, *text, *pooled, *out, *ws;
    bool operator<(const GraphKey& o) const {
      return std::tie(batch, w, lat, text, pooled, out, ws) < std::tie(o.batch, o.w, o.lat, o.text, o.pooled, o.out, o.ws);
    }
  };
  std::map<GraphKey, hipGraphExec_t> graphs;
  hipStream_t cap_stream = nullptr;
  ~sdn_unet() {
    for (auto& kv : graphs) (void)hipGraphExecDestroy(kv.second);
    for (auto e : ev) (void)hipEventDestroy(e);
    if (cap_stream) (void)hipStreamDestroy(cap_stream);
  }
  std::vector<hipEvent_t> ev;
  int profiled_batch = 0;
  int profiled_n = 0;
  int dtype() const {
    switch (kind) {
      case sdn_plan::MMDIT: return mcfg.dtype;
      case sdn_plan::VAE_DECODER: case sdn_plan::VAE_ENCODER: return vcfg.dtype;
      case sdn_plan::CLIP: return ccfg.dtype;
      case sdn_plan::CLIP_PROJ: return pcfg.dtype;
      case sdn_plan::T5: return tcfg.dtype;
      case sdn_plan::CLIP_VISION: return vis.dtype;
      case sdn_plan::INCEPTION: return icfg.dtype;
      default: return cfg.dtype;
    }
  }
  bool is_vae() const { return kind == sdn_plan::VAE_DECODER || kind == sdn_plan::VAE_ENCODER; }
  bool is_clip() const { return kind == sdn_plan::CLIP || kind == sdn_plan::CLIP_PROJ; }
};

namespace sdn_plan {

constexpr bool kK320Plain = true, kK320Ln = true, kK320Rp = true;

struct Builder {
  sdn_unet* u;
  Plan* plan;
  Arena arena;
  int B;
  int seq = 0;
  int es = 2;
  bool x3t = false;
  bool x3t_hold = false;
  std::set<int64_t> tri;
  Ref tproj;
  int tproj_cursor = 0;
  Ref gn_stats;
  Ref pending_cols;
  int64_t kv_top = 0;
  bool res_pre_next = false;
  bool k320_next = false;
  bool triple_out_next = false;
  bool pair_out_next = false;
  bool plan_bad = false;
  bool force_x3t_next = false;
  std::set<int64_t> pairs;
  struct Up4 { int64_t op; int64_t w9; int N, Cin; };
  std::vector<Up4> up4_pending;
  void finish_up4();
  struct Res { std::string pfx; int cout; };

  Ref param(const std::string& name, int kind, int rows, int cols, int rows_padded = 0);
  Ref stacked(const std::vector<std::string>& names, int rows_each, int cols);
  Ref stacked_vec(const std::vector<std::string>& names, int n_each);
  Ref derived(const std::string& name, int64_t bytes);
  Act act(int64_t rows, int C, int hw = 0, int side = 0, int esz = 0);
  Act act_gn(int64_t rows, int C, int hw, int side);
  void want_stats(const Act& out) { pending_cols = out.st_off >= 0 ? Ref{SP_WS, out.st_off} : Ref(); }
  void drop(Act& t);
  static Ref R(const Act& t) { return Ref{SP_WS, t.off}; }
  Ref x3_weight(Ref w, int rows, int cols, int group);
  Act split3(Ref a, Ref a2, int64_t rows, int c1, int c2, int hw = 0, int side = 0);
  bool x3t_on(const Ref& a) const { return x3t && !x3t_hold && a.space == SP_WS; }
  void gemm(int64_t M, int N, int K, Ref a, Ref w, Ref bias, Ref out, int act_ = SDN_ACT_NONE, Ref residual = Ref(),
            int out_kind = SDN_OUT_BF16, int n_valid = 0, Ref a2 = Ref(), int K1 = 0, Ref rowbias = Ref(),
            int rows_per_batch = 0, int ld_rowbias = 0);
  void push_gemm(Op& o);
  void conv3x3(const Act& in, int cout, int n_pad, Ref w, Ref bias, Ref out, int stride, int upsample, Ref residual,
               Ref rowbias, int ld_rowbias, int out_kind = SDN_OUT_BF16, int n_valid = 0, int asym_pad = 0);
  void groupnorm(const Act& x, const Act* x2, float eps, int silu, Ref gamma, Ref beta, const Act& out);
  void layernorm(const Act& x, Ref gamma, Ref beta, const Act& out);
  void repeat(const Act& in, const Act& out, int rep);
  void attention(Ref q, Ref k, Ref v, Ref out, int nq, int nk, int C, int ldq, int ldk, int ldv, bool kv_pairs = false);

  void gemm_ln(const Act& x, int64_t rows, int N, int K, const std::string& wname, Ref w, Ref gamma, Ref beta, Ref bias,
               Ref out, int act_, bool prepass);
  Act resnet(const std::string& pfx, Act& x, Act* skip, int cout);
  Act transformer(const std::string& pfx, Act& x);
  void transformer_body(const std::string& pfx, Act& x, const Act& out, int64_t text_off, int rep = 1,
                        const Act* x_full = nullptr);
  std::vector<Res> enumerate_resnets() const;
  void build();

  void gemm_ex(int64_t M, int N, int K, Ref a, Ref w, Ref bias, Ref out, int act_, Ref residual, int out_kind,
               Ref rowbias, Ref rowgate, int rows_per_batch, int ld_row, int residual_bcast = 0);
  void ln_mod(const Act& x, int64_t rows, int rows_per_batch, Ref scale, Ref shift, int ld, const Act& out);
  Ref fcol(int col) const { return Ref{SP_WS, tproj.off + (int64_t)col * 4}; }
  void build_mmdit();

  Act vae_resnet(const std::string& pfx, Act& x, int cout);
  Act vae_attention(const std::string& pfx, Act& x);
  void vae_f32_rows();
  void build_vae();
  void build_vae_encoder();

  void build_clip();
  Ref glu_pair(const std::string& value_name, const std::string& gate_name, int F, int K);
  void t5_gemm(int64_t M, int N, int K, Ref a, Ref w, Ref out, int act_, bool into_stream);
  void t5_rmsnorm(Ref x, bool x_f32, int64_t rows, int C, Ref w, Ref out);
  void build_t5();

  void build_clip_vision();

  void inception_conv(const std::string& name, const Act& in, int cout, int kh, int kw, int stride, int ph, int pw, const Act& out,
                      int c0);
  Act inception_conv_new(const std::string& name, const Act& in, int cout, int kh = 1, int kw = 1, int stride = 1, int ph = 0, int pw = 0);
  void inception_pool(int mode, const Act& in, int stride, int pad, const Act& out, int c0);
  void build_inception();
};

Plan* get_plan(sdn_unet* u, int batch, int n = 0);
int run_plan(sdn_unet* u, const Call& c);
void drop_graphs(sdn_unet* u);

}
```

### safe_denoiser_amd/csrc/sdn_plan_api.hip

```cpp
#include <algorithm>

#include "sdn_plan.h"

using namespace sdn_plan;

template <class F, class V> static void set_plan_toggle(sdn_unet* u, F sdn_unet::*field, V value) {
  u->*field = value;
  drop_graphs(u);
  u->plans.clear();
}

extern "C" {

int sdn_unet_create(const sdn_unet_config* cfg, sdn_unet** out) {
  if (!cfg || !out) return SDN_E_INVALID;
  if (cfg->n_levels < 1 || cfg->n_levels > 4 || cfg->layers_per_block < 1 || cfg->n_heads <= 0 ||
      cfg->in_channels <= 0 || cfg->in_channels > 16 || cfg->out_channels <= 0 || cfg->out_channels > 32 ||
      cfg->sample_size <= 0 || (cfg->sample_size % (1 << (cfg->n_levels - 1))) != 0 || cfg->cross_dim % 64 != 0 ||
      cfg->text_len <= 0 || cfg->norm_groups <= 0 || cfg->norm_groups > 64 || cfg->dtype < 0 || cfg->dtype > 3 ||
      cfg->latent_repeat < 0 || cfg->latent_repeat > 8)
    return SDN_E_INVALID;
  for (int i = 0; i < cfg->n_levels; ++i) {
    const int c = cfg->block_out_channels[i];
    if (c <= 0 || c % 64 != 0 || c % cfg->norm_groups != 0 || c % cfg->n_heads != 0) return SDN_E_INVALID;
    const int hd = c / cfg->n_heads;
    if (cfg->level_has_attn[i] && hd != 40 && hd != 64 && hd != 80 && hd != 160) return SDN_E_INVALID;
    if (sdn_gemm_pick_nrep(c, SDN_ACT_NONE) == 0 || sdn_gemm_pick_nrep(8 * c, SDN_ACT_GEGLU) == 0) return SDN_E_INVALID;
  }
  {
    const int hd_mid = cfg->block_out_channels[cfg->n_levels - 1] / cfg->n_heads;
    if (hd_mid != 40 && hd_mid != 64 && hd_mid != 80 && hd_mid != 160) return SDN_E_INVALID;
  }
  sdn_unet* u = new sdn_unet();
  u->cfg = *cfg;
  if (cfg->dtype >= 2) { u->gn_fuse = false; u->ln_fold = false; u->ff_fuse = false; }
  get_plan(u, cfg->latent_repeat > 1 ? cfg->latent_repeat : 1);
  *out = u;
  return SDN_OK;
}

int sdn_mmdit_create(const sdn_mmdit_config* cfg, sdn_unet** out) {
  if (!cfg || !out) return SDN_E_INVALID;
  const int C = cfg->num_heads * cfg->head_dim;
  if (cfg->in_channels <= 0 || cfg->out_channels <= 0 || cfg->sample_size <= 0 || cfg->patch_size <= 0 ||
      cfg->sample_size % cfg->patch_size != 0 || cfg->num_layers <= 0 || cfg->num_heads <= 0 || cfg->head_dim != 64 ||
      C % 128 != 0 || cfg->joint_dim % 64 != 0 || cfg->pooled_dim % 64 != 0 || cfg->time_dim % 64 != 0 ||
      (cfg->in_channels * cfg->patch_size * cfg->patch_size) % 64 != 0 ||
      (cfg->out_channels * cfg->patch_size * cfg->patch_size) % 32 != 0 || cfg->text_len <= 0 || cfg->dtype < 0 ||
      cfg->dtype > 3 || C > 2048)
    return SDN_E_INVALID;
  sdn_unet* u = new sdn_unet();
  memset(&u->cfg, 0, sizeof(u->cfg));
  u->mcfg = *cfg;
  u->kind = MMDIT;
  get_plan(u, 1);
  *out = u;
  return SDN_OK;
}

int sdn_vae_decoder_create(const sdn_vae_config* cfg, sdn_unet** out) {
  if (!cfg || !out) return SDN_E_INVALID;
  if (cfg->n_levels < 1 || cfg->n_levels > 4 || cfg->layers_per_block < 1 || cfg->latent_channels <= 0 ||
      cfg->latent_channels > 16 || cfg->out_channels <= 0 || cfg->out_channels > 32 || cfg->sample_size <= 0 ||
      cfg->norm_groups <= 0 || cfg->norm_groups > 64 || cfg->dtype < 0 || cfg->dtype > 3)
    return SDN_E_INVALID;
  for (int i = 0; i < cfg->n_levels; ++i) {
    const int c = cfg->block_out_channels[i];
    if (c <= 0 || c % 64 != 0 || c % cfg->norm_groups != 0 || sdn_gemm_pick_nrep(c, SDN_ACT_NONE) == 0) return SDN_E_INVALID;
  }
  const int hw = cfg->sample_size * cfg->sample_size;
  if (hw % 64 != 0 || hw > 16384 || (hw > 4096 && hw % 4096 != 0) || sdn_gemm_pick_nrep(hw, SDN_ACT_NONE) == 0) return SDN_E_INVALID;
  sdn_unet* u = new sdn_unet();
  memset(&u->cfg, 0, sizeof(u->cfg));
  u->cfg.norm_groups = cfg->norm_groups;
  if (cfg->dtype >= 2) { u->gn_fuse = false; u->ln_fold = false; u->ff_fuse = false; }
  u->vcfg = *cfg;
  u->kind = VAE_DECODER;
  get_plan(u, 1);
  *out = u;
  return SDN_OK;
}

int sdn_vae_encoder_create(const sdn_vae_config* cfg, sdn_unet** out) {
  if (!cfg || !out) return SDN_E_INVALID;
  sdn_unet* u = nullptr;
  const int rc = sdn_vae_decoder_create(cfg, &u);
  if (rc != SDN_OK) return rc;
  if (2 * cfg->latent_channels > 32) { delete u; return SDN_E_INVALID; }
  u->kind = VAE_ENCODER;
  u->plans.clear(); u->params.clear(); u->param_index.clear(); u->weight_bytes = 0;
  get_plan(u, 1);
  *out = u;
  return SDN_OK;
}

int sdn_clip_create(const sdn_clip_config* cfg, sdn_unet** out) {
  if (!cfg || !out) return SDN_E_INVALID;
  if (cfg->vocab_size <= 0 || cfg->hidden_size <= 0 || cfg->hidden_size % 128 != 0 || cfg->hidden_size > 1024 ||
      cfg->intermediate_size <= 0 || cfg->intermediate_size % 128 != 0 || cfg->num_layers <= 0 || cfg->num_heads <= 0 ||
      cfg->hidden_size != 64 * cfg->num_heads || cfg->max_position_embeddings <= 0 || cfg->max_position_embeddings > 4096 ||
      cfg->dtype < 0 || cfg->dtype > 3)
    return SDN_E_INVALID;
  sdn_unet* u = new sdn_unet();
  memset(&u->cfg, 0, sizeof(u->cfg));
  if (cfg->dtype >= 2) { u->gn_fuse = false; u->ln_fold = false; u->ff_fuse = false; }
  u->ccfg = *cfg;
  u->kind = CLIP;
  get_plan(u, 1);
  *out = u;
  return SDN_OK;
}

int sdn_clip_proj_create(const sdn_clip_proj_config* cfg, sdn_unet** out) {
  if (!cfg || !out) return SDN_E_INVALID;
  if (cfg->vocab_size <= 0 || cfg->hidden_size <= 0 || cfg->hidden_size % 128 != 0 || cfg->hidden_size > 1280 ||
      cfg->intermediate_size <= 0 || cfg->intermediate_size % 128 != 0 || cfg->num_layers <= 0 || cfg->num_heads <= 0 ||
      cfg->hidden_size != 64 * cfg->num_heads || cfg->max_position_embeddings <= 0 || cfg->max_position_embeddings > 4096 ||
      cfg->dtype < 0 || cfg->dtype > 3 || cfg->projection_dim <= 0 || cfg->projection_dim % 32 != 0 ||
      (cfg->act != SDN_ACT_QUICK_GELU && cfg->act != SDN_ACT_GELU) || cfg->eos_token_id < 0 || cfg->hidden_tap < 1 ||
      cfg->hidden_tap > cfg->num_layers)
    return SDN_E_INVALID;
  sdn_unet* u = new sdn_unet();
  memset(&u->cfg, 0, sizeof(u->cfg));
  if (cfg->dtype >= 2) { u->gn_fuse = false; u->ln_fold = false; u->ff_fuse = false; }
  u->pcfg = *cfg;
  u->ccfg.vocab_size = cfg->vocab_size; u->ccfg.hidden_size = cfg->hidden_size; u->ccfg.intermediate_size = cfg->intermediate_size;
  u->ccfg.num_layers = cfg->num_layers; u->ccfg.num_heads = cfg->num_heads; u->ccfg.max_position_embeddings = cfg->max_position_embeddings;
  u->ccfg.dtype = cfg->dtype;
  u->kind = CLIP_PROJ;
  get_plan(u, 1);
  *out = u;
  return SDN_OK;
}

int sdn_t5_create(const sdn_t5_config* cfg, sdn_unet** out) {
  if (!cfg || !out) return SDN_E_INVALID;
  if (cfg->vocab_size <= 0 || cfg->d_model <= 0 || cfg->d_model % 64 != 0 || cfg->d_kv != 64 || cfg->d_ff <= 0 || cfg->d_ff % 64 != 0 ||
      cfg->num_layers <= 0 || cfg->num_heads <= 0 || cfg->num_heads > 512 || cfg->num_buckets < 4 || cfg->num_buckets > 64 ||
      (cfg->num_buckets & 3) || cfg->max_distance <= cfg->num_buckets / 4 || !(cfg->eps > 0.f) || cfg->dtype < 0 || cfg->dtype > 1)
    return SDN_E_INVALID;
  sdn_unet* u = new sdn_unet();
  memset(&u->cfg, 0, sizeof(u->cfg));
  u->tcfg = *cfg;
  u->kind = T5;
  get_plan(u, 1);
  *out = u;
  return SDN_OK;
}

int sdn_unet_prepare(sdn_unet* u, void* weights, void* stream) {
  if (!u || !weights) return SDN_E_INVALID;
  char* W = (char*)weights;
  const int dt = u->dtype() == 1 ? 1 : 0;
  for (const auto& j : u->fold_jobs) {
    if (j.kind == 2) {
      const int rc2 = sdn_expand3_weights((const float*)(W + j.w), j.rows, j.cols, j.group, W + j.wf, stream);
      if (rc2 != SDN_OK) return rc2;
      continue;
    }
    if (j.kind == 3) {
      const int rc3 = sdn_conv_up4_weights(dt, W + j.w, j.rows, j.cols, W + j.wf, stream);
      if (rc3 != SDN_OK) return rc3;
      continue;
    }
    if (j.kind == 1) {
      const int rc1 = sdn_linear_pair_fold(dt, W + j.w, W + j.gamma, (const float*)(W + j.beta), (const float*)(W + j.bias), j.rows, j.cols,
                                           W + j.wf, (float*)(W + j.c), stream);
      if (rc1 != SDN_OK) return rc1;
      continue;
    }
    const int rc = sdn_ln_fold(dt, W + j.w, (const float*)(W + j.gamma), (const float*)(W + j.beta),
                               j.bias >= 0 ? (const float*)(W + j.bias) : nullptr, j.rows, j.cols, W + j.wf, (float*)(W + j.c),
                               (float*)(W + j.d), stream);
    if (rc != SDN_OK) return rc;
  }
  return SDN_OK;
}

void sdn_unet_destroy(sdn_unet* u) { delete u; }

int sdn_unet_param_count(const sdn_unet* u) { return u ? (int)u->params.size() : 0; }

int sdn_unet_param_info(const sdn_unet* u, int32_t index, sdn_param_info* info) {
  if (!u || !info || index < 0 || index >= (int)u->params.size()) return SDN_E_INVALID;
  *info = u->params[index];
  return SDN_OK;
}

size_t sdn_unet_weight_bytes(const sdn_unet* u) { return u ? (size_t)u->weight_bytes : 0; }

static int vae_chunk(const sdn_unet* v) {
  const sdn_vae_config& c = v->vcfg;
  const int64_t side = (int64_t)c.sample_size << (c.n_levels - 1);
  if (c.dtype >= 2) {
    int64_t largest = 0;
    for (int j = 0; j < c.n_levels; ++j) {
      const int64_t s = side >> j, ch = std::max(c.block_out_channels[j], c.block_out_channels[j + 1 < c.n_levels ? j + 1 : j]);
      largest = std::max(largest, s * s * ch * 4);
    }
    const int64_t cap = std::min<int64_t>(4, (((int64_t)1 << 31) - 1) / largest);
    return cap < 1 ? 0 : (int)cap;
  }
  int64_t cmax = 0;
  for (int i = 0; i < c.n_levels; ++i) if (c.block_out_channels[i] > cmax) cmax = c.block_out_channels[i];
  int64_t cap = (((int64_t)1 << 32) - 1) / (side * side * cmax * 2);
  if (cap > 8) cap = 8;
  return cap < 1 ? 0 : (int)cap;
}

size_t sdn_unet_workspace_bytes(sdn_unet* u, int32_t batch) {
  if (!u || batch <= 0) return 0;
  if (u->kind == T5) return sdn_t5_workspace_bytes(u, batch, 512);
  if (u->is_vae()) {
    const int cap = vae_chunk(u);
    if (cap == 0) return 0;
    if (batch > cap) batch = cap;
  }
  const int64_t b = get_plan(u, batch)->ws_bytes;
  return b < 0 ? 0 : (size_t)b;
}

double sdn_unet_flops(sdn_unet* u, int32_t batch, double* attn) {
  if (!u || batch <= 0) return 0.0;
  Plan* p = get_plan(u, batch);
  if (attn) *attn = p->attn_flops;
  return p->flops;
}

static int vae_run(sdn_unet* v, Call call, const float* in, int64_t in_n, float* out, int64_t out_n, int32_t batch) {
  if (batch < 0 || (batch > 0 && (!in || !out))) return SDN_E_INVALID;
  const int cap = vae_chunk(v);
  if (cap == 0) return SDN_E_INVALID;
  for (int lo = 0; lo < batch; lo += cap) {
    call.batch = batch - lo < cap ? batch - lo : cap;
    call.in = in + lo * in_n; call.out = out + lo * out_n;
    const int rc = run_plan(v, call);
    if (rc != SDN_OK) return rc;
  }
  return SDN_OK;
}

int sdn_vae_decode(sdn_unet* v, const void* weights, const float* latents, float latent_scale, float* image, int32_t batch,
                   void* workspace, size_t workspace_bytes, void* stream) {
  if (!v || v->kind != VAE_DECODER) return SDN_E_INVALID;
  const sdn_vae_config& c = v->vcfg;
  const int64_t side = (int64_t)c.sample_size << (c.n_levels - 1);
  Call call(weights, workspace, workspace_bytes, 0, stream);
  call.scalar = latent_scale;
  return vae_run(v, call, latents, (int64_t)c.latent_channels * c.sample_size * c.sample_size, image, (int64_t)c.out_channels * side * side, batch);
}

int sdn_vae_encode(sdn_unet* v, const void* weights, const float* image, float* moments, int32_t batch, void* workspace,
                   size_t workspace_bytes, void* stream) {
  if (!v || v->kind != VAE_ENCODER) return SDN_E_INVALID;
  const sdn_vae_config& c = v->vcfg;
  const int64_t side = (int64_t)c.sample_size << (c.n_levels - 1);
  return vae_run(v, Call(weights, workspace, workspace_bytes, 0, stream), image, (int64_t)c.out_channels * side * side, moments,
                 (int64_t)2 * c.latent_channels * c.sample_size * c.sample_size, batch);
}

int sdn_clip_forward(sdn_unet* m, const void* weights, const int32_t* input_ids, const int32_t* attention_mask,
                     void* last_hidden_state, int32_t batch, void* workspace, size_t workspace_bytes, void* stream) {
  if (!m || m->kind != CLIP || !input_ids || !last_hidden_state) return SDN_E_INVALID;
  Call call(weights, workspace, workspace_bytes, batch, stream);
  call.in = input_ids; call.mask = attention_mask; call.out = last_hidden_state;
  return run_plan(m, call);
}

int sdn_clip_proj_forward(sdn_unet* m, const void* weights, const int32_t* input_ids, void* hidden, int64_t hidden_batch_stride,
                          int64_t hidden_row_stride, void* text_embeds, int64_t embeds_row_stride, int32_t batch, void* workspace,
                          size_t workspace_bytes, void* stream) {
  if (!m || m->kind != CLIP_PROJ || !input_ids || !hidden || !text_embeds) return SDN_E_INVALID;
  const sdn_clip_proj_config& c = m->pcfg;
  if (hidden_row_stride < c.hidden_size || hidden_batch_stride < (int64_t)c.max_position_embeddings * hidden_row_stride ||
      embeds_row_stride < c.projection_dim || embeds_row_stride > 0x7fffffff || (hidden_row_stride & 7) || (hidden_batch_stride & 7) ||
      (embeds_row_stride & 7) || (reinterpret_cast<uintptr_t>(hidden) & 15) || (reinterpret_cast<uintptr_t>(text_embeds) & 15))
    return SDN_E_INVALID;
  Call call(weights, workspace, workspace_bytes, batch, stream);
  call.in = input_ids; call.out = hidden; call.out2 = text_embeds;
  call.out_bs = hidden_batch_stride; call.out_rs = hidden_row_stride; call.out2_rs = embeds_row_stride;
  return run_plan(m, call);
}

size_t sdn_t5_workspace_bytes(sdn_unet* m, int32_t batch, int32_t n) {
  if (!m || m->kind != T5 || batch <= 0 || batch > (1 << 20) || n < 2 || n > 512) return 0;
  const int64_t b = get_plan(m, batch, n)->ws_bytes;
  return b < 0 ? 0 : (size_t)b;
}

double sdn_t5_flops(sdn_unet* m, int32_t batch, int32_t n, double* attn) {
  if (!m || m->kind != T5 || batch <= 0 || batch > (1 << 20) || n < 2 || n > 512) return 0.0;
  Plan* p = get_plan(m, batch, n);
  if (attn) *attn = p->attn_flops;
  return p->flops;
}

int sdn_t5_forward(sdn_unet* m, const void* weights, const int32_t* input_ids, const int32_t* attention_mask, int32_t n,
                   void* out, int32_t batch, void* workspace, size_t workspace_bytes, void* stream) {
  if (!m || m->kind != T5 || n < 2 || n > 512 || batch > (1 << 20) || !input_ids || !out) return SDN_E_INVALID;
  Call call(weights, workspace, workspace_bytes, batch, stream);
  call.in = input_ids; call.mask = attention_mask; call.n = n; call.out = out;
  return run_plan(m, call);
}

int sdn_unet_forward(sdn_unet* u, const void* weights, const float* latents, float timestep, const void* text,
                     float* out, int32_t batch, void* workspace, size_t workspace_bytes, void* stream) {
  if (!u || u->kind != UNET || !latents || !text || !out) return SDN_E_INVALID;
  Call call(weights, workspace, workspace_bytes, batch, stream);
  call.in = latents; call.scalar = timestep; call.text = text; call.out = out;
  return run_plan(u, call);
}

int sdn_mmdit_forward(sdn_unet* u, const void* weights, const float* latents, float timestep, const void* text,
                      const void* pooled, float* out, int32_t batch, void* workspace, size_t workspace_bytes,
                      void* stream) {
  if (!u || u->kind != MMDIT || !latents || !text || !pooled || !out) return SDN_E_INVALID;
  Call call(weights, workspace, workspace_bytes, batch, stream);
  call.in = latents; call.scalar = timestep; call.text = text; call.pooled = pooled; call.out = out;
  return run_plan(u, call);
}

void sdn_unet_set_text_version(sdn_unet* u, uint64_t version) {
  if (!u) return;
  u->text_version = version;
  if (version == 0) u->kv_version = 0;
}

void sdn_unet_profile_next(sdn_unet* u) { if (u) u->profile_next = true; }

void sdn_unet_set_split_k(sdn_unet* u, int32_t on) {
  if (!u || u->kind == T5 || u->kind == CLIP_PROJ || u->kind == CLIP_VISION || u->split_k == (on != 0)) return;
  if (u->dtype() >= 2) return;
  set_plan_toggle(u, &sdn_unet::split_k, on != 0);
}

void sdn_unet_set_conv_up4(sdn_unet* u, int32_t on) {
  if (!u || u->kind != UNET || u->dtype() >= 2 || u->conv_up4 == (on != 0)) return;
  set_plan_toggle(u, &sdn_unet::conv_up4, on != 0);
}

void sdn_unet_set_graph_mode(sdn_unet* u, int32_t on) {
  if (!u) return;
  u->use_graph = on != 0;
  if (!on) drop_graphs(u);
}


void sdn_debug_set_x3_expand(sdn_unet* u, int on) { if (u && u->x3_expand != (on != 0)) set_plan_toggle(u, &sdn_unet::x3_expand, on != 0); }

void sdn_debug_set_res_pre(sdn_unet* u, int on) { if (u && u->res_pre != (on != 0)) set_plan_toggle(u, &sdn_unet::res_pre, on != 0); }

void sdn_debug_set_gemm_k320(sdn_unet* u, int on) { if (u && u->gemm_k320 != (on != 0)) set_plan_toggle(u, &sdn_unet::gemm_k320, on != 0); }

void sdn_debug_set_ln_fold(sdn_unet* u, int on) { if (u) set_plan_toggle(u, &sdn_unet::ln_fold, on != 0); }

void sdn_debug_set_ln_prepass_all(sdn_unet* u, int on) { if (u) set_plan_toggle(u, &sdn_unet::ln_prepass_all, on); }

void sdn_debug_set_ffn_fuse(sdn_unet* u, int on) { if (u) set_plan_toggle(u, &sdn_unet::ffn_fuse, on != 0); }

void sdn_debug_set_ff_fuse(sdn_unet* u, int on) { if (u) set_plan_toggle(u, &sdn_unet::ff_fuse, on != 0); }

void sdn_debug_set_ffn_own_stats(sdn_unet* u, int on) { if (u) set_plan_toggle(u, &sdn_unet::ffn_own_stats, on != 0); }

void sdn_debug_set_x3_pairs(sdn_unet* u, int on) { if (u) set_plan_toggle(u, &sdn_unet::x3_pairs, on != 0); }

void sdn_debug_set_gn_fuse(sdn_unet* u, int on) { if (u) set_plan_toggle(u, &sdn_unet::gn_fuse, on != 0); }

void sdn_debug_set_subbatch_bytes(sdn_unet* u, long long bytes) {
  if (u && u->kind != MMDIT) set_plan_toggle(u, &sdn_unet::subbatch_bytes, (int64_t)bytes);
}

}
```

### safe_denoiser_amd/csrc/sdn_plan_core.hip

```cpp
#include <math.h>

#include "sdn_plan.h"

namespace sdn_plan {

Ref Builder::param(const std::string& name, int kind, int rows, int cols, int rows_padded) {
  auto it = u->param_index.find(name);
  if (it != u->param_index.end()) return Ref{SP_W, u->params[it->second].offset};
  sdn_param_info pi;
  memset(&pi, 0, sizeof(pi));
  snprintf(pi.name, sizeof(pi.name), "%s", name.c_str());
  pi.kind = kind; pi.rows = rows; pi.cols = cols; pi.rows_padded = rows_padded > rows ? rows_padded : rows;
  const int64_t esz = (kind == SDN_P_VEC_F32 || kind == SDN_P_GEGLU_VEC) ? 4 : es;
  const int64_t bytes = (int64_t)pi.rows_padded * (cols > 0 ? cols : 1) * esz;
  pi.offset = u->weight_bytes;
  u->weight_bytes += (bytes + 255) & ~(int64_t)255;
  u->param_index[name] = (int)u->params.size();
  u->params.push_back(pi);
  return Ref{SP_W, pi.offset};
}
Ref Builder::stacked(const std::vector<std::string>& names, int rows_each, int cols) {
  Ref first;
  int64_t expect = -1;
  for (size_t i = 0; i < names.size(); ++i) {
    Ref r = param(names[i], SDN_P_MAT, rows_each, cols);
    if (i == 0) first = r;
    else if (r.off != expect) { fprintf(stderr, "libsdn: stacked weight %s is not contiguous\n", names[i].c_str()); abort(); }
    expect = r.off + (int64_t)rows_each * cols * es;
  }
  return first;
}
Ref Builder::stacked_vec(const std::vector<std::string>& names, int n_each) {
  Ref first; int64_t expect = -1;
  for (size_t i = 0; i < names.size(); ++i) {
    Ref r = param(names[i], SDN_P_VEC_F32, n_each, 0);
    if (i == 0) first = r;
    else if (r.off != expect) { fprintf(stderr, "libsdn: stacked bias %s is not contiguous\n", names[i].c_str()); abort(); }
    expect = r.off + (int64_t)n_each * 4;
  }
  return first;
}
Ref Builder::derived(const std::string& name, int64_t bytes) {
  auto it = u->param_index.find(name);
  if (it != u->param_index.end()) return Ref{SP_W, u->params[it->second].offset};
  sdn_param_info pi; memset(&pi, 0, sizeof(pi));
  snprintf(pi.name, sizeof(pi.name), "%s", name.c_str());
  pi.kind = SDN_P_DERIVED; pi.rows = (int)bytes; pi.cols = 0; pi.rows_padded = (int)bytes;
  pi.offset = u->weight_bytes;
  u->weight_bytes += (bytes + 255) & ~(int64_t)255;
  u->param_index[name] = (int)u->params.size();
  u->params.push_back(pi);
  return Ref{SP_W, pi.offset};
}

Act Builder::act(int64_t rows, int C, int hw, int side, int esz) {
  const bool dflt = esz == 0;
  if (esz == 0) esz = es;
  Act t; t.content = rows * C * esz;
  t.bytes = (x3t && dflt) ? rows * C * 6 : t.content;
  t.off = arena.alloc(t.bytes); t.C = C; t.hw = hw; t.side = side; return t;
}
Act Builder::act_gn(int64_t rows, int C, int hw, int side) {
  Act t = act(rows, C, hw, side);
  if (u->gn_fuse && !u->split_k && hw > 0 && hw % 128 == 0) {
    t.st_bytes = ((rows + 127) / 128) * (int64_t)C * 8;
    t.st_off = arena.alloc(t.st_bytes);
  }
  return t;
}
void Builder::drop(Act& t) {
  if (t.off >= 0) { arena.release(t.off, t.bytes); tri.erase(t.off); pairs.erase(t.off); }
  if (t.st_off >= 0) arena.release(t.st_off, t.st_bytes);
  t.off = -1; t.st_off = -1;
}

Ref Builder::x3_weight(Ref w, int rows, int cols, int group) {
  const std::string name = "x3@" + std::to_string((long long)w.off);
  const bool fresh = u->param_index.find(name) == u->param_index.end();
  Ref d = derived(name, (int64_t)rows * 3 * cols * 2);
  if (fresh) { sdn_unet::FoldJob j{w.off, -1, -1, -1, d.off, -1, -1, rows, cols}; j.kind = 2; j.group = group; u->fold_jobs.push_back(j); }
  return d;
}
Act Builder::split3(Ref a, Ref a2, int64_t rows, int c1, int c2, int hw, int side) {
  Act t = act(rows, c1 + c2, hw, side);
  Op o; o.kind = OP_SPLIT3; o.a = a; o.a2 = a2; o.rows = rows; o.c1 = c1; o.c2 = c2; o.out = R(t);
  o.bytes = 10.0 * (double)rows * (c1 + c2);
  snprintf(o.label, sizeof(o.label), "k_split3");
  plan->ops.push_back(o);
  tri.insert(t.off);
  return t;
}

void Builder::gemm(int64_t M, int N, int K, Ref a, Ref w, Ref bias, Ref out, int act_, Ref residual,
                   int out_kind, int n_valid, Ref a2, int K1, Ref rowbias,
                   int rows_per_batch, int ld_rowbias) {
  const bool forced = force_x3t_next && x3t && !x3t_hold;
  force_x3t_next = false;
  if (x3t) k320_next = false;
  if ((x3t_on(a) || forced) && (act_ == SDN_ACT_NONE || act_ == SDN_ACT_GEGLU) && out_kind != SDN_OUT_F32_NCHW && n_valid == 0) {
    Act tmp; Ref au = a;
    if (a.space != SP_WS || !tri.count(a.off)) { tmp = split3(a, a2, M, a2.space != SP_NONE ? K1 : K, a2.space != SP_NONE ? K - K1 : 0); au = R(tmp); }
    Op o; o.kind = OP_GEMM; memset(&o.gd, 0, sizeof(o.gd));
    o.x3t = 1;
    o.gd.M = (int)M; o.gd.N = N; o.gd.K = 3 * K; o.gd.a_mode = SDN_A_PLAIN; o.gd.act = act_; o.gd.out_kind = SDN_OUT_F32;
    const bool tri_o = triple_out_next && act_ == SDN_ACT_NONE;
    const bool pair_o = pair_out_next && act_ == SDN_ACT_NONE && !tri_o && residual.space == SP_NONE;
    triple_out_next = false; pair_out_next = false;
    o.gd.x3_out = act_ == SDN_ACT_GEGLU ? 2 : (tri_o ? 3 : (pair_o ? 4 : 1)); o.gd.rows_per_batch = rows_per_batch; o.gd.ld_rowbias = ld_rowbias;
    if (pair_o && out.space == SP_WS) pairs.insert(out.off);
    o.a = au; o.w = x3_weight(w, N, K, K); o.bias = bias; o.rowbias = rowbias; o.residual = residual; o.out = out;
    o.flops = 2.0 * (double)M * (double)N * (double)K;
    o.bytes = 6.0 * ((double)M * K + (double)N * K) + 4.0 * (double)M * (act_ == SDN_ACT_GEGLU ? 0.75 * N : N) +
              (residual.space != SP_NONE ? 4.0 * (double)M * N : 0.0);
    snprintf(o.label, sizeof(o.label), "k_gemm<%d>x3", sdn_gemm_pick_tile((int)M, N, 3 * K, act_));
    push_gemm(o);
    if ((act_ == SDN_ACT_GEGLU || tri_o) && out.space == SP_WS) tri.insert(out.off);
    if (tmp.off >= 0) drop(tmp);
    return;
  }
  triple_out_next = false; pair_out_next = false;
  const bool k320_ok = k320_next;
  k320_next = false;
  const bool rp = res_pre_next && residual.space != SP_NONE && act_ == SDN_ACT_NONE && out_kind == SDN_OUT_BF16 && n_valid == 0 && es == 2;
  res_pre_next = false;
  Op o; o.kind = OP_GEMM; memset(&o.gd, 0, sizeof(o.gd));
  o.gd.res_pre = rp ? 1 : 0;
  o.gd.M = (int)M; o.gd.N = N; o.gd.K = K; o.gd.a_mode = SDN_A_PLAIN; o.gd.K1 = K1; o.gd.act = act_;
  o.gd.out_kind = out_kind; o.gd.n_valid = n_valid; o.gd.rows_per_batch = rows_per_batch; o.gd.ld_rowbias = ld_rowbias;
  o.a = a; o.a2 = a2; o.w = w; o.bias = bias; o.rowbias = rowbias; o.residual = residual; o.out = out;
  o.flops = 2.0 * (double)M * (double)(n_valid > 0 ? n_valid : N) * (double)K;
  o.bytes = 2.0 * ((double)M * K + (double)N * K + (double)M * (act_ == SDN_ACT_GEGLU ? N / 2 : N)) +
            (residual.space != SP_NONE ? 2.0 * (double)M * N : 0.0);
  snprintf(o.label, sizeof(o.label), "k_gemm<%d>%s", sdn_gemm_pick_tile((int)M, N, K, act_, residual.space != SP_NONE && !rp), rp ? "/rp" : "");
  if (k320_ok && K == 320 && N % 320 == 0 && act_ == SDN_ACT_NONE && out_kind == SDN_OUT_BF16 && n_valid == 0 && a2.space == SP_NONE &&
      rowbias.space == SP_NONE && (residual.space == SP_NONE || rp) && pending_cols.space == SP_NONE && !u->split_k &&
      (rp ? kK320Rp : kK320Plain)) {
    o.k320 = 1;
    snprintf(o.label, sizeof(o.label), "k_gemm_k320%s", rp ? "/rp" : "");
  }
  push_gemm(o);
}
void Builder::push_gemm(Op& o) {
  o.col = pending_cols; pending_cols = Ref();
  const int nv = o.gd.n_valid > 0 ? o.gd.n_valid : o.gd.N;
  const int split = (!u->split_k || nv != o.gd.N || (o.gd.a_mode == SDN_A_CONV3X3 && o.gd.upsample == 2)) ? 1
                    : sdn_gemm_pick_split(o.gd.M, o.gd.N, o.gd.K, o.gd.act, o.gd.out_kind);
  if (split > 1) {
    const int64_t bytes = (int64_t)split * o.gd.M * o.gd.N * 4;
    const int64_t off = arena.alloc(bytes);
    o.gd.split_k = split; o.aux = Ref{SP_WS, off}; o.rows = bytes;
    arena.release(off, bytes);
    const size_t L = strlen(o.label);
    if (L + 3 < sizeof(o.label)) snprintf(o.label + L, sizeof(o.label) - L, "/s%d", split);
  }
  plan->ops.push_back(o);
  plan->flops += o.flops;
}
void Builder::conv3x3(const Act& in, int cout, int n_pad, Ref w, Ref bias, Ref out, int stride, int upsample, Ref residual,
                      Ref rowbias, int ld_rowbias, int out_kind, int n_valid, int asym_pad) {
  const int Hi = upsample ? in.side * 2 : in.side;
  const int Ho = (Hi + (asym_pad ? 1 : 2) - 3) / stride + 1;
  if (x3t_on(R(in))) {
    Act tmp; Ref au = R(in);
    if (!tri.count(in.off)) { tmp = split3(R(in), Ref(), (int64_t)B * in.side * in.side, in.C, 0, in.hw, in.side); au = R(tmp); }
    Op o; o.kind = OP_GEMM; memset(&o.gd, 0, sizeof(o.gd));
    o.x3t = 1;
    o.gd.M = B * Ho * Ho; o.gd.N = n_pad; o.gd.K = 27 * in.C; o.gd.a_mode = SDN_A_CONV3X3;
    o.gd.Hs = in.side; o.gd.Ws = in.side; o.gd.Cin = 3 * in.C; o.gd.Ho = Ho; o.gd.Wo = Ho; o.gd.stride = stride;
    o.gd.upsample = upsample; o.gd.asym_pad = asym_pad; o.gd.n_valid = n_valid; o.gd.rows_per_batch = Ho * Ho; o.gd.ld_rowbias = ld_rowbias;
    if (out_kind == SDN_OUT_F32_NCHW) { o.gd.out_kind = out_kind; o.gd.x3_out = 0; }
    else { o.gd.out_kind = SDN_OUT_F32; o.gd.x3_out = 1; }
    o.a = au; o.w = x3_weight(w, n_pad, 9 * in.C, in.C); o.bias = bias; o.rowbias = rowbias; o.residual = residual; o.out = out;
    o.flops = 2.0 * (double)o.gd.M * (double)cout * 9.0 * in.C;
    o.bytes = 6.0 * ((double)B * in.side * in.side * in.C + (double)n_pad * 9 * in.C) + 4.0 * (double)o.gd.M * cout +
              (residual.space != SP_NONE ? 4.0 * (double)o.gd.M * cout : 0.0);
    if (Ho == in.side && sdn_conv_slab_shape_ok(o.gd.M, n_pad, 3 * in.C, in.side, stride, upsample, asym_pad, SDN_OUT_BF16, n_valid) &&
        sdn_gemm_pick_tile(o.gd.M, n_pad, o.gd.K, SDN_ACT_NONE) == 10)
      snprintf(o.label, sizeof(o.label), "k_conv_slab<%d>/x3", in.side);
    else
      snprintf(o.label, sizeof(o.label), "k_gemm<%d>x3", sdn_gemm_pick_tile(o.gd.M, n_pad, o.gd.K, SDN_ACT_NONE));
    push_gemm(o);
    if (tmp.off >= 0) drop(tmp);
    return;
  }
  Op o; o.kind = OP_GEMM; memset(&o.gd, 0, sizeof(o.gd));
  o.gd.res_pre = (res_pre_next && residual.space != SP_NONE && out_kind == SDN_OUT_BF16 && n_valid == 0 && es == 2) ? 1 : 0;
  res_pre_next = false;
  o.gd.M = B * Ho * Ho; o.gd.N = n_pad; o.gd.K = 9 * in.C; o.gd.a_mode = SDN_A_CONV3X3;
  o.gd.Hs = in.side; o.gd.Ws = in.side; o.gd.Cin = in.C; o.gd.Ho = Ho; o.gd.Wo = Ho; o.gd.stride = stride;
  o.gd.upsample = upsample; o.gd.asym_pad = asym_pad; o.gd.out_kind = out_kind; o.gd.n_valid = n_valid; o.gd.rows_per_batch = Ho * Ho;
  o.gd.ld_rowbias = ld_rowbias;
  o.a = R(in); o.w = w; o.bias = bias; o.rowbias = rowbias; o.residual = residual; o.out = out;
  o.flops = 2.0 * (double)o.gd.M * (double)cout * (double)o.gd.K;
  o.bytes = 2.0 * ((double)B * in.side * in.side * in.C + (double)n_pad * o.gd.K + (double)o.gd.M * cout) +
            (residual.space != SP_NONE ? 2.0 * (double)o.gd.M * cout : 0.0);
  const int up4 = (upsample == 1 && u->kind == UNET && es == 2 && stride == 1 && !asym_pad && out_kind == SDN_OUT_BF16 && n_valid == 0 &&
                   n_pad == cout && residual.space == SP_NONE && rowbias.space == SP_NONE && w.space == SP_W)
                      ? sdn_conv_up4_tile(in.side, in.side, in.C, n_pad) : 0;
  if (up4) {
    up4_pending.push_back({u->conv_up4 ? (int64_t)plan->ops.size() : -1, w.off, n_pad, in.C});
    if (u->conv_up4) {
      o.gd.K = 4 * in.C; o.gd.upsample = 2; o.gd.res_pre = 0;
      o.bytes = 2.0 * ((double)B * in.side * in.side * in.C + 4.0 * n_pad * o.gd.K + (double)o.gd.M * cout);
      snprintf(o.label, sizeof(o.label), "k_conv_up4<%d>", up4);
      push_gemm(o);
      return;
    }
  }
  if (Ho == in.side && sdn_conv_slab_shape_ok(o.gd.M, n_pad, in.C, in.side, stride, upsample, asym_pad, out_kind, n_valid) &&
      sdn_gemm_pick_tile(o.gd.M, n_pad, o.gd.K, SDN_ACT_NONE) == 10)
    snprintf(o.label, sizeof(o.label), "k_conv_slab<%d>", in.side);
  else
    snprintf(o.label, sizeof(o.label), "k_gemm<%d>", sdn_gemm_pick_tile(o.gd.M, n_pad, o.gd.K, SDN_ACT_NONE));
  push_gemm(o);
}
void Builder::finish_up4() {
  for (const Up4& p : up4_pending) {
    const std::string name = "up4@" + std::to_string((long long)p.w9);
    const bool fresh = u->param_index.find(name) == u->param_index.end();
    Ref d = derived(name, (int64_t)16 * p.N * p.Cin * 2);
    if (fresh) { sdn_unet::FoldJob j{p.w9, -1, -1, -1, d.off, -1, -1, p.N, p.Cin}; j.kind = 3; u->fold_jobs.push_back(j); }
    if (p.op >= 0) plan->ops[(size_t)p.op].w = d;
  }
  up4_pending.clear();
}
void Builder::groupnorm(const Act& x, const Act* x2, float eps, int silu, Ref gamma, Ref beta, const Act& out) {
  Op o; o.kind = OP_GN; o.a = R(x); if (x2) o.a2 = R(*x2);
  o.batch = B; o.hw = x.hw; o.c1 = x.C; o.c2 = x2 ? x2->C : 0; o.groups = u->cfg.norm_groups; o.eps = eps;
  o.silu = silu; o.w = gamma; o.bias = beta; o.out = R(out); o.aux = gn_stats;
  if (x3t) { o.tri_out = 1; tri.insert(out.off); }
  if (x.st_off >= 0 && (!x2 || x2->st_off >= 0)) {
    o.cols1 = Ref{SP_WS, x.st_off};
    if (x2) o.cols2 = Ref{SP_WS, x2->st_off};
  }
  o.bytes = 2.0 * (o.cols1.space != SP_NONE ? 2.0 : 3.0) * (double)B * x.hw * (o.c1 + o.c2);
  snprintf(o.label, sizeof(o.label), o.cols1.space != SP_NONE ? "k_gn_apply" : "k_gn_stats+apply");
  plan->ops.push_back(o);
}
void Builder::layernorm(const Act& x, Ref gamma, Ref beta, const Act& out) {
  Op o; o.kind = OP_LN; o.a = R(x); o.rows = (int64_t)B * x.hw; o.c1 = x.C; o.eps = 1e-5f; o.w = gamma; o.bias = beta;
  o.out = R(out);
  if (x3t) { o.tri_out = 1; tri.insert(out.off); }
  o.bytes = 2.0 * 2.0 * (double)o.rows * x.C;
  snprintf(o.label, sizeof(o.label), "k_layernorm");
  plan->ops.push_back(o);
}
void Builder::repeat(const Act& in, const Act& out, int rep) {
  Op o; o.kind = OP_REPEAT; o.a = R(in); o.out = R(out); o.rows = in.content; o.c1 = rep;
  o.bytes = (double)in.content * (1 + rep);
  snprintf(o.label, sizeof(o.label), "k_repeat");
  plan->ops.push_back(o);
}
void Builder::attention(Ref q, Ref k, Ref v, Ref out, int nq, int nk, int C, int ldq, int ldk, int ldv, bool kv_pairs) {
  Op o; o.kind = OP_ATTN; o.a = q; o.k = k; o.v = v; o.out = out; o.batch = B; o.heads = u->cfg.n_heads;
  o.nq = nq; o.nk = nk; o.hd = C / u->cfg.n_heads; o.ldq = ldq; o.ldk = ldk; o.ldv = ldv; o.ldo = C;
  o.scale = 1.0f / sqrtf((float)o.hd);
  if (x3t && out.space == SP_WS) { o.tri_out = 1; tri.insert(out.off); }
  if (q.space == SP_WS && pairs.count(q.off)) {
    o.pair_in = kv_pairs ? 2 : 1; pairs.erase(q.off);
  } else if (kv_pairs) {
    plan_bad = true;
  }
  const double f = 4.0 * (double)B * o.heads * (double)nq * (double)nk * (double)o.hd;
  o.flops = f;
  o.bytes = 2.0 * (double)B * C * (2.0 * nq + 2.0 * nk);
  snprintf(o.label, sizeof(o.label), "k_attn<%d>", o.hd);
  plan->ops.push_back(o);
  plan->flops += f; plan->attn_flops += f;
}

Plan* get_plan(sdn_unet* u, int batch, int n) {
  if (u->kind == T5 && n == 0) n = 512;
  const int key = u->kind == T5 ? batch * 1024 + n : batch;
  auto it = u->plans.find(key);
  if (it != u->plans.end()) return &it->second;
  if (u->kind == T5 && u->plans.size() >= 64) {
    u->plans.clear();
    u->profiled_batch = 0;
  }
  Plan& p = u->plans[key];
  p.batch = batch;
  Builder b{u, &p};
  b.B = batch;
  b.seq = n;
  b.es = u->dtype() >= 2 ? 4 : 2;
  b.x3t = u->kind == UNET && u->dtype() == 3 && u->x3_expand;
  switch (u->kind) {
    case UNET: b.build(); break;
    case MMDIT: b.build_mmdit(); break;
    case VAE_DECODER: b.build_vae(); break;
    case VAE_ENCODER: b.build_vae_encoder(); break;
    case CLIP: case CLIP_PROJ: b.build_clip(); break;
    case T5: b.build_t5(); break;
    case CLIP_VISION: b.build_clip_vision(); break;
    case INCEPTION: b.build_inception(); break;
  }
  return &p;
}

}
```

### safe_denoiser_amd/csrc/sdn_plan_run.hip

```cpp
#include "sdn_plan.h"

namespace sdn_plan {

static long g_x3_chunk_limit = (1L << 31) - 4096;
extern "C" void sdn_debug_set_x3_chunk_bytes(long long bytes) { g_x3_chunk_limit = bytes > 0 ? (long)bytes : (1L << 31) - 4096; }

static int launch_x3t_gemm(const Op& o, const char* a, const char* w, const float* bias, const float* rowbias, const char* residual,
                           void* out, void* stream) {
  const sdn_gemm_desc& d = o.gd;
  const bool conv = d.a_mode == SDN_A_CONV3X3;
  const long rows_out_unit = conv ? (long)d.Ho * d.Wo : 256;
  const long a_bytes_unit = conv ? (long)d.Hs * d.Ws * d.Cin * 2 : 256L * d.K * 2;
  const long units = conv ? d.M / rows_out_unit : (d.M + 255) / 256;
  long per = g_x3_chunk_limit / a_bytes_unit;
  if (per < 1) return SDN_E_INVALID;
  if (per > units) per = units;
  if (per < units) {
    const long n = (units + per - 1) / per;
    long even = (units + n - 1) / n;
    const int nrep = sdn_gemm_pick_tile((int)(even * rows_out_unit < d.M ? even * rows_out_unit : d.M), d.N, d.K, d.act, 0);
    const long tile_rows = nrep >= 8 ? 256 : 128, tile_cols = 32L * (nrep > 0 ? nrep : 2);
    const long tiles_per_unit = ((rows_out_unit + tile_rows - 1) / tile_rows) * ((d.N + tile_cols - 1) / tile_cols);
    long a_ = 256, b_ = tiles_per_unit % 256;
    while (b_) { const long t_ = a_ % b_; a_ = b_; b_ = t_; }
    const long q = 256 / a_;
    const long aligned = (even + q - 1) / q * q;
    if (aligned <= per) even = aligned;
    per = even;
  }
  const int n_cols = d.x3_out == 2 ? d.N / 2 : d.N;
  const long out_row_bytes = d.x3_out == 0 ? 0 : ((d.x3_out == 1 || d.x3_out == 4) ? 4L * n_cols : 6L * n_cols);
  if (d.x3_out == 0 && per < units) return SDN_E_INVALID;
  for (long u0 = 0; u0 < units; u0 += per) {
    const long nu = units - u0 < per ? units - u0 : per;
    sdn_gemm_desc c = d;
    const long r0 = u0 * rows_out_unit;
    long rn = nu * rows_out_unit;
    if (r0 + rn > d.M) rn = d.M - r0;
    c.M = (int)rn;
    const float* rb = rowbias;
    if (rowbias && d.rows_per_batch > 0) rb = rowbias + (r0 / d.rows_per_batch) * d.ld_rowbias;
    const int rc = sdn_gemm_bf16(&c, a + u0 * a_bytes_unit, nullptr, w, bias, rb, nullptr,
                                 residual ? residual + r0 * 4L * n_cols : nullptr, (char*)out + r0 * out_row_bytes, stream);
    if (rc != SDN_OK) return rc;
  }
  return SDN_OK;
}

static int launch_op_f32(const sdn_unet* u, const Op& o, const Call& P, bool x3, const float* t_dev, void* stream) {
  int rc = SDN_OK;
  switch (o.kind) {
    case OP_TEMB:
      rc = sdn_temb_f32(P.scalar, t_dev, o.batch, o.c1, (void*)P(o.out), stream);
      break;
    case OP_CONV_IN:
      rc = sdn_conv_in_f32((const float*)P(o.a), P(o.w), (const float*)P(o.bias), o.batch, o.c1, o.hw, o.hw, o.c2, (void*)P(o.out), stream);
      break;
    case OP_GEMM:
      if (o.x3t) { rc = launch_x3t_gemm(o, P(o.a), P(o.w), (const float*)P(o.bias), (const float*)P(o.rowbias), P(o.residual), (void*)P(o.out), stream); break; }
      if (o.dyn_ldc) {
        sdn_gemm_desc gd = o.gd; gd.ldc = (int)P.out2_rs;
        rc = (x3 ? sdn_gemm_x3 : sdn_gemm_f32)(&gd, P(o.a), nullptr, P(o.w), nullptr, nullptr, nullptr, nullptr, (void*)P(o.out), stream);
        break;
      }
      rc = (o.ln || o.gd.split_k > 1) ? SDN_E_INVALID
           : (x3 ? sdn_gemm_x3 : sdn_gemm_f32)(&o.gd, P(o.a), P(o.a2), P(o.w), (const float*)P(o.bias), (const float*)P(o.rowbias),
                                               (const float*)P(o.rowgate), P(o.residual), (void*)P(o.out), stream);
      break;
    case OP_SPLIT3:
      rc = sdn_split3((const float*)P(o.a), (const float*)P(o.a2), o.rows, o.c1, o.c2, (void*)P(o.out), stream);
      break;
    case OP_GN:
      rc = (o.tri_out ? sdn_groupnorm_f32_triple : sdn_groupnorm_f32)(P(o.a), P(o.a2), o.batch, o.hw, o.c1, o.c2, o.groups, o.eps, o.silu,
                                                                     (const float*)P(o.w), (const float*)P(o.bias), (void*)P(o.out),
                                                                     (float*)P(o.aux), stream);
      break;
    case OP_LN:
      if (o.mod) {
        rc = o.tri_out ? SDN_E_INVALID
                       : sdn_layernorm_mod_f32(P(o.a), o.rows, o.c1, o.eps, (const float*)P(o.w), (const float*)P(o.bias), o.ld_mod,
                                               o.hw, (void*)P(o.out), stream);
        break;
      }
      rc = (o.tri_out ? sdn_layernorm_f32_triple : sdn_layernorm_f32)(P(o.a), o.rows, o.c1, o.eps, (const float*)P(o.w),
                                                                      (const float*)P(o.bias), (void*)P(o.out), stream);
      break;
    case OP_PATCHIFY:
      rc = sdn_patchify_f32((const float*)P(o.a), o.batch, o.c1, o.hw, o.hw, o.patch, (void*)P(o.out), stream);
      break;
    case OP_UNPATCHIFY:
      rc = sdn_unpatchify_f32((const float*)P(o.a), o.batch, o.c1, o.hw, o.hw, o.patch, (float*)P(o.out), stream);
      break;
    case OP_ATTN:
      if (o.pair_in == 1) {
        rc = sdn_attention_x3_pairs(P(o.a), P(o.a) + (size_t)o.ldo * 2, P(o.a) + (size_t)o.ldo * 4, o.ldq, o.ldq, (void*)P(o.out), o.batch, o.heads,
                                    o.nq, o.nk, o.hd, 2 * o.ldq, 2 * o.ldk, 2 * o.ldv, o.ldo, o.scale, o.tri_out, stream);
        break;
      }
      if (o.pair_in == 2) {
        rc = sdn_attention_x3_pairs(P(o.a), P(o.k), P(o.k) + (size_t)o.ldo * 2, o.ldq, o.ldk, (void*)P(o.out), o.batch, o.heads,
                                    o.nq, o.nk, o.hd, 2 * o.ldq, 2 * o.ldk, 2 * o.ldv, o.ldo, o.scale, o.tri_out, stream);
        break;
      }
      if (o.n1 > 0) {
        sdn_attn_segment2 s2{P(o.q2), P(o.k2), P(o.v2), (void*)P(o.out2), o.n1, o.ldq, o.ldk, o.ldv, o.ldo};
        rc = o.tri_out ? SDN_E_INVALID
                       : sdn_joint_attention_f32(x3 ? 1 : 0, P(o.a), P(o.k), P(o.v), (void*)P(o.out), &s2, o.batch, o.heads, o.nq, o.hd,
                                                 o.ldq, o.ldk, o.ldv, o.ldo, o.scale, stream);
        break;
      }
      rc = (o.tri_out ? sdn_attention_x3_triple : (x3 ? sdn_attention_x3 : sdn_attention_f32))(
          P(o.a), P(o.k), P(o.v), (void*)P(o.out), o.batch, o.heads, o.nq, o.nk, o.hd, o.ldq, o.ldk, o.ldv, o.ldo, o.scale, stream);
      break;
    case OP_REPEAT:
      rc = sdn_repeat(P(o.a), (size_t)o.rows, o.c1, (void*)P(o.out), stream);
      break;
    case OP_CLIP_EMBED:
      rc = sdn_clip_embed_f32((const int32_t*)P(o.a), P(o.w), P(o.bias), o.rows, o.hw, o.c1, o.c2, (void*)P(o.out), stream);
      break;
    case OP_EOS_ROWS:
      rc = sdn_clip_eos_rows(2, (const int32_t*)P(o.a), P(o.k), (const float*)P(o.w), (const float*)P(o.bias), o.batch, o.hw, o.c1, o.c2,
                             u->pcfg.eos_token_id, o.eps, (void*)P(o.out), nullptr, stream);
      break;
    case OP_COPY_ROWS:
      rc = sdn_copy_rows_strided(P(o.a), o.batch, o.hw, o.c1, 4, (void*)P(o.out), P.out_bs, P.out_rs, stream);
      break;
    case OP_CONV_ROWS:
      rc = sdn_patch_rows_f32((const float*)P(o.a), o.batch, o.hw, o.hw, o.c1, o.kh, o.kw, o.sh, o.sw, o.ph, o.pw, o.c2, (float*)P(o.out), stream);
      break;
    case OP_POOL3:
      rc = sdn_pool3_f32(o.mod, (const float*)P(o.a), o.batch, o.hw, o.hw, o.c1, o.sh, o.ph, (float*)P(o.out), o.ldo, o.c2, stream);
      break;
    case OP_RESIZE:
      rc = sdn_resize_bilinear_f32((const float*)P(o.a), o.batch, P.in_h, P.in_w, o.hw, o.hw, o.scale, o.eps, (float*)P(o.out), stream);
      break;
    case OP_SPATIAL_MEAN:
      rc = sdn_spatial_mean_f32((const float*)P(o.a), o.batch, o.hw, o.c1, (float*)P(o.out), stream);
      break;
    case OP_LATENT_MIX:
      rc = sdn_latent_mix((const float*)P(o.a), (const float*)P(o.w), (const float*)P(o.bias), o.batch, o.c1, o.hw,
                          o.mod ? o.scale : P.scalar , (float*)P(o.out), stream);
      break;
    case OP_SOFTMAX:
      rc = sdn_softmax_rows(2, (const float*)P(o.a), o.c1, o.rows, o.c1, o.scale, (void*)P(o.out), o.c1, stream);
      break;
    case OP_TRANSPOSE:
      rc = sdn_transpose32(P(o.a), (int)o.rows, o.c1, o.ldq, (void*)P(o.out), o.ldo, stream);
      break;
    case OP_MATTN:
      rc = sdn_masked_attention_f32(P(o.a), P(o.k), P(o.v), (void*)P(o.out), P.mask, 1, o.batch, o.heads,
                                    o.nq, o.hd, o.ldq, o.ldk, o.ldv, o.ldo, o.scale, stream);
      break;
    default:
      rc = SDN_E_INVALID;
  }
  return rc;
}

static int launch_op_16(const sdn_unet* u, const Op& o, const Call& P, bool f16, const float* t_dev, void* stream) {
  int rc = SDN_OK;
  switch (o.kind) {
    case OP_TEMB:
      if (t_dev) rc = sdn_temb_from_device(f16 ? 1 : 0, t_dev, o.batch, o.c1, (void*)P(o.out), stream);
      else rc = (f16 ? sdn_timestep_embed_f16 : sdn_timestep_embed_bf16)(P.scalar, o.batch, o.c1, (void*)P(o.out), stream);
      break;
    case OP_CONV_IN:
      rc = (f16 ? sdn_conv_in_f16 : sdn_conv_in_bf16)((const float*)P(o.a), P(o.w), (const float*)P(o.bias), o.batch, o.c1, o.hw, o.hw, o.c2,
                            (void*)P(o.out), stream);
      break;
    case OP_ROWSTATS:
      rc = (f16 ? sdn_row_stats_f16 : sdn_row_stats_bf16)(P(o.a), o.rows, o.c1, o.eps, (float*)P(o.out), stream);
      break;
    case OP_FFN:
      rc = sdn_ffn_geglu_fused(f16 ? 1 : 0, o.rows, o.c1, P(o.a), (const float*)P(o.ln_stats), P(o.w), (const float*)P(o.ln_c),
                               (const float*)P(o.ln_d), P(o.a2), (const float*)P(o.bias), P(o.residual), (void*)P(o.out),
                               o.col.space != SP_NONE ? (float*)P(o.col) : nullptr, stream);
      break;
    case OP_EOS_ROWS:
      rc = sdn_clip_eos_rows(f16 ? 1 : 0, (const int32_t*)P(o.a), P(o.k), (const float*)P(o.w), (const float*)P(o.bias), o.batch, o.hw,
                             o.c1, o.c2, u->pcfg.eos_token_id, o.eps, (void*)P(o.out), nullptr, stream);
      break;
    case OP_COPY_ROWS:
      rc = sdn_copy_rows_strided(P(o.a), o.batch, o.hw, o.c1, 2, (void*)P(o.out), P.out_bs, P.out_rs, stream);
      break;
    case OP_PATCH_ROWS:
      rc = sdn_clip_patch_rows(f16 ? 1 : 0, (const float*)P(o.a), o.batch, o.hw, o.patch, o.c1, (void*)P(o.out), stream);
      break;
    case OP_VISION_EMBED:
      rc = sdn_clip_vision_embed(f16 ? 1 : 0, P(o.a), (const float*)P(o.a2), P(o.aux), (const float*)P(o.w), (const float*)P(o.bias), o.batch,
                                 o.hw, o.c1, o.eps, (void*)P(o.out), stream);
      break;
    case OP_CLASS_ROWS:
      rc = sdn_clip_class_rows(f16 ? 1 : 0, P(o.a), (const float*)P(o.w), (const float*)P(o.bias), o.batch, o.hw, o.c1, o.eps,
                               (void*)P(o.out), stream);
      break;
    case OP_GEMM:
      if (o.k320) {
        rc = sdn_gemm_k320(f16 ? 1 : 0, &o.gd, P(o.a), P(o.w), o.ln ? nullptr : (const float*)P(o.bias), o.ln ? (const float*)P(o.ln_c) : nullptr,
                           o.ln ? (const float*)P(o.ln_d) : nullptr, o.eps, o.ln ? nullptr : P(o.residual), (void*)P(o.out), stream);
        break;
      }
      if (o.dyn_ldc) {
        sdn_gemm_desc gd = o.gd; gd.ldc = (int)P.out2_rs;
        rc = (f16 ? sdn_gemm_f16 : sdn_gemm_bf16)(&gd, P(o.a), nullptr, P(o.w), nullptr, nullptr, nullptr, nullptr, (void*)P(o.out), stream);
        break;
      }
      if (o.ln) {
        rc = (f16 ? sdn_gemm_ln_f16 : sdn_gemm_ln_bf16)(&o.gd, P(o.a), P(o.w), (const float*)P(o.ln_c), (const float*)P(o.ln_d), o.eps,
                                                        (const float*)P(o.ln_stats), (void*)P(o.out), stream);
        break;
      }
      if (o.col.space != SP_NONE && o.gd.split_k <= 1) {
        rc = (f16 ? sdn_gemm_stats_f16 : sdn_gemm_stats_bf16)(&o.gd, P(o.a), P(o.a2), P(o.w), (const float*)P(o.bias),
                                                              (const float*)P(o.rowbias), P(o.residual), (void*)P(o.out),
                                                              (float*)P(o.col), stream);
        break;
      }
      if (o.gd.split_k > 1) {
        rc = (f16 ? sdn_gemm_splitk_f16 : sdn_gemm_splitk_bf16)(&o.gd, P(o.a), P(o.a2), P(o.w), (const float*)P(o.bias),
                                                                (const float*)P(o.rowbias), (const float*)P(o.rowgate), P(o.residual),
                                                                (void*)P(o.out), (void*)P(o.aux), (size_t)o.rows, stream);
        break;
      }
      rc = (f16 ? sdn_gemm_f16 : sdn_gemm_bf16)(&o.gd, P(o.a), P(o.a2), P(o.w), (const float*)P(o.bias), (const float*)P(o.rowbias),
                         (const float*)P(o.rowgate), P(o.residual), (void*)P(o.out), stream);
      break;
    case OP_GN:
      if (o.cols1.space != SP_NONE) {
        rc = (f16 ? sdn_groupnorm_cols_f16 : sdn_groupnorm_cols_bf16)(P(o.a), P(o.a2), o.batch, o.hw, o.c1, o.c2, o.groups, o.eps,
                                                                      o.silu, (const float*)P(o.w), (const float*)P(o.bias),
                                                                      (void*)P(o.out), (float*)P(o.aux), (const float*)P(o.cols1),
                                                                      (const float*)P(o.cols2), stream);
        break;
      }
      rc = (f16 ? sdn_groupnorm_f16 : sdn_groupnorm_bf16)(P(o.a), P(o.a2), o.batch, o.hw, o.c1, o.c2, o.groups, o.eps, o.silu,
                              (const float*)P(o.w), (const float*)P(o.bias), (void*)P(o.out), (float*)P(o.aux), stream);
      break;
    case OP_CLIP_EMBED:
      rc = sdn_clip_embed(f16 ? 1 : 0, (const int32_t*)P(o.a), P(o.w), P(o.bias), o.rows, o.hw, o.c1, o.c2, (void*)P(o.out), stream);
      break;
    case OP_MATTN:
      rc = sdn_masked_attention(f16 ? 1 : 0, P(o.a), P(o.k), P(o.v), (void*)P(o.out), P.mask, 1, o.batch,
                                o.heads, o.nq, o.hd, o.ldq, o.ldk, o.ldv, o.ldo, o.scale, stream);
      break;
    case OP_RMSNORM:
      rc = sdn_rmsnorm(f16 ? 1 : 0, P(o.a), o.mod, o.rows, o.c1, o.eps, (const float*)P(o.w), (void*)P(o.out), stream);
      break;
    case OP_EMBED:
      rc = sdn_embed_tokens(f16 ? 1 : 0, (const int32_t*)P(o.a), P(o.w), o.rows, o.c1, o.c2, (float*)P(o.out), stream);
      break;
    case OP_T5_BIAS:
      rc = sdn_t5_relative_bias(f16 ? 1 : 0, P(o.w), u->tcfg.num_buckets, u->tcfg.max_distance, o.heads, o.nq, (float*)P(o.out), stream);
      break;
    case OP_BATTN:
      rc = sdn_bias_attention(f16 ? 1 : 0, P(o.a), P(o.k), P(o.v), (void*)P(o.out), (const float*)P(o.aux), P.mask,
                              o.batch, o.heads, o.nq, o.hd, o.ldq, o.ldk, o.ldv, o.ldo, o.scale, stream);
      break;
    case OP_REPEAT:
      rc = sdn_repeat(P(o.a), (size_t)o.rows, o.c1, (void*)P(o.out), stream);
      break;
    case OP_LATENT_MIX:
      rc = sdn_latent_mix((const float*)P(o.a), (const float*)P(o.w), (const float*)P(o.bias), o.batch, o.c1, o.hw,
                          o.mod ? o.scale : P.scalar ,
                          (float*)P(o.out), stream);
      break;
    case OP_SOFTMAX:
      rc = sdn_softmax_rows(f16 ? 1 : 0, (const float*)P(o.a), o.c1, o.rows, o.c1, o.scale, (void*)P(o.out), o.c1, stream);
      break;
    case OP_TRANSPOSE:
      rc = sdn_transpose16(P(o.a), (int)o.rows, o.c1, o.ldq, (void*)P(o.out), o.ldo, stream);
      break;
    case OP_PATCHIFY:
      rc = (f16 ? sdn_patchify_f16 : sdn_patchify_bf16)((const float*)P(o.a), o.batch, o.c1, o.hw, o.hw, o.patch,
                                                        (void*)P(o.out), stream);
      break;
    case OP_UNPATCHIFY:
      rc = sdn_unpatchify_f32((const float*)P(o.a), o.batch, o.c1, o.hw, o.hw, o.patch, (float*)P(o.out), stream);
      break;
    case OP_LN:
      if (o.mod) {
        rc = (f16 ? sdn_layernorm_mod_f16 : sdn_layernorm_mod_bf16)(P(o.a), o.rows, o.c1, o.eps, (const float*)P(o.w),
                                                                    (const float*)P(o.bias), o.ld_mod, o.hw,
                                                                    (void*)P(o.out), stream);
        break;
      }
      rc = (f16 ? sdn_layernorm_f16 : sdn_layernorm_bf16)(P(o.a), o.rows, o.c1, o.eps, (const float*)P(o.w), (const float*)P(o.bias),
                              (void*)P(o.out), stream);
      break;
    case OP_ATTN:
      if (o.n1 > 0) {
        sdn_attn_segment2 s2{P(o.q2), P(o.k2), P(o.v2), (void*)P(o.out2), o.n1, o.ldq, o.ldk, o.ldv, o.ldo};
        rc = sdn_joint_attention(f16 ? 1 : 0, P(o.a), P(o.k), P(o.v), (void*)P(o.out), &s2, o.batch, o.heads, o.nq, o.hd,
                                 o.ldq, o.ldk, o.ldv, o.ldo, o.scale, stream);
        break;
      }
      rc = (f16 ? sdn_attention_f16 : sdn_attention_bf16)(P(o.a), P(o.k), P(o.v), (void*)P(o.out), o.batch, o.heads, o.nq, o.nk, o.hd, o.ldq,
                              o.ldk, o.ldv, o.ldo, o.scale, stream);
      break;
  }
  return rc;
}

static int launch_ops(sdn_unet* u, const Plan* p, const Call& c, const float* t_dev, bool prof, void* stream, bool skip_text_kv = false) {
  const int sdt = u->dtype();
  const bool f32 = sdt >= 2;
  for (size_t opi = 0; opi < p->ops.size(); ++opi) {
    const Op& o = p->ops[opi];
    if ((skip_text_kv && o.text_kv) || (o.kind == OP_COPY_ROWS && !c.out)) continue;
    if (prof) (void)hipEventRecord(u->ev[2 * opi], (hipStream_t)stream);
    const int rc = f32 ? launch_op_f32(u, o, c, sdt == 3, t_dev, stream) : launch_op_16(u, o, c, sdt == 1, t_dev, stream);
    if (prof) (void)hipEventRecord(u->ev[2 * opi + 1], (hipStream_t)stream);
    if (rc != SDN_OK) return rc;
  }
  return SDN_OK;
}

int run_plan(sdn_unet* u, const Call& given) {
  if (!u || !given.weights || !given.workspace || given.batch <= 0) return SDN_E_INVALID;
  Plan* p = get_plan(u, given.batch, given.n);
  if (p->ws_bytes < 0) return SDN_E_INVALID;
  if (given.workspace_bytes < (size_t)p->ws_bytes) return SDN_E_WORKSPACE;
  Call c = given; c.kv_base = p->kv_base;
  const bool prof = u->profile_next;
  if (prof) {
    u->profile_next = false;
    while (u->ev.size() < 2 * p->ops.size()) { hipEvent_t e; if (hipEventCreate(&e) != hipSuccess) return SDN_E_LAUNCH; u->ev.push_back(e); }
    u->profiled_batch = c.batch; u->profiled_n = c.n;
  }
  hipStream_t hs = (hipStream_t)c.stream;
  if (u->use_graph && !prof && (u->kind == UNET || u->kind == MMDIT) && p->tscalar_off >= 0) {
    hipStreamCaptureStatus cs = hipStreamCaptureStatusNone;
    if (hipStreamIsCapturing(hs, &cs) == hipSuccess && cs == hipStreamCaptureStatusNone) {
      float* t_dev = (float*)((char*)c.workspace + p->tscalar_off);
      int rc = sdn_set_scalar(t_dev, c.scalar, c.stream);
      if (rc != SDN_OK) return rc;
      const sdn_unet::GraphKey key{c.batch, c.weights, c.in, c.text, c.pooled, c.out, c.workspace};
      auto it = u->graphs.find(key);
      if (it == u->graphs.end()) {
        if (u->graphs.size() >= 16) {
          (void)hipStreamSynchronize(hs);
          for (auto& kv : u->graphs) (void)hipGraphExecDestroy(kv.second);
          u->graphs.clear();
        }
        hipGraph_t graph = nullptr;
        if (!u->cap_stream && hipStreamCreateWithFlags(&u->cap_stream, hipStreamNonBlocking) != hipSuccess) return SDN_E_LAUNCH;
        if (hipStreamBeginCapture(u->cap_stream, hipStreamCaptureModeThreadLocal) != hipSuccess) return SDN_E_LAUNCH;
        rc = launch_ops(u, p, c, t_dev, false, (void*)u->cap_stream);
        const hipError_t ec = hipStreamEndCapture(u->cap_stream, &graph);
        if (rc != SDN_OK || ec != hipSuccess || !graph) { if (graph) (void)hipGraphDestroy(graph); return rc != SDN_OK ? rc : SDN_E_LAUNCH; }
        hipGraphExec_t exec = nullptr;
        const hipError_t ei = hipGraphInstantiate(&exec, graph, nullptr, nullptr, 0);
        (void)hipGraphDestroy(graph);
        if (ei != hipSuccess || !exec) return SDN_E_LAUNCH;
        it = u->graphs.emplace(key, exec).first;
      }
      u->kv_version = 0;
      return hipGraphLaunch(it->second, hs) == hipSuccess ? SDN_OK : SDN_E_LAUNCH;
    }
  }
  const bool declared = u->kind == UNET && u->text_version != 0 && u->subbatch_bytes == 0;
  const bool skip = declared && !prof && u->kv_version == u->text_version && u->kv_batch == c.batch && u->kv_w == c.weights &&
                    u->kv_text == c.text && u->kv_ws == c.workspace;
  const int rc_l = launch_ops(u, p, c, nullptr, prof, c.stream, skip);
  if (rc_l == SDN_OK && declared) { u->kv_version = u->text_version; u->kv_batch = c.batch; u->kv_w = c.weights; u->kv_text = c.text; u->kv_ws = c.workspace; }
  else if (!declared) u->kv_version = 0;
  return rc_l;
}

void drop_graphs(sdn_unet* u) {
  if (u->graphs.empty()) return;
  (void)hipDeviceSynchronize();
  for (auto& kv : u->graphs) (void)hipGraphExecDestroy(kv.second);
  u->graphs.clear();
}

}

using namespace sdn_plan;

static bool op_ms(const sdn_unet* u, size_t i, float* ms) {
  return hipEventSynchronize(u->ev[2 * i + 1]) == hipSuccess && hipEventElapsedTime(ms, u->ev[2 * i], u->ev[2 * i + 1]) == hipSuccess;
}

extern "C" int sdn_debug_profile_ops(sdn_unet* u, double* out, char* labels, int max_ops) {
  if (!u || !out || !labels || u->profiled_batch <= 0) return -1;
  Plan* p = get_plan(u, u->profiled_batch, u->profiled_n);
  int n = 0;
  for (size_t i = 0; i < p->ops.size() && n < max_ops; ++i, ++n) {
    float ms = 0.f;
    if (!op_ms(u, i, &ms)) return -2;
    const Op& o = p->ops[i];
    out[n * 6 + 0] = ms; out[n * 6 + 1] = o.flops; out[n * 6 + 2] = o.bytes;
    out[n * 6 + 3] = o.kind == OP_GEMM ? o.gd.M : (o.kind == OP_ATTN ? o.nq : o.rows);
    out[n * 6 + 4] = o.kind == OP_GEMM ? o.gd.N : (o.kind == OP_ATTN ? o.nk : o.c1);
    out[n * 6 + 5] = o.kind == OP_GEMM ? o.gd.K : (o.kind == OP_ATTN ? o.hd : o.c2);
    memcpy(labels + n * 24, o.label, 24);
  }
  return n;
}

extern "C" int sdn_unet_profile_read(sdn_unet* u, sdn_profile_row* rows, int32_t max_rows) {
  if (!u || !rows || max_rows <= 0 || u->profiled_batch <= 0) return SDN_E_INVALID;
  Plan* p = get_plan(u, u->profiled_batch, u->profiled_n);
  if (u->ev.size() < 2 * p->ops.size()) return SDN_E_INVALID;
  int n = 0;
  for (size_t i = 0; i < p->ops.size(); ++i) {
    float ms = 0.f;
    if (!op_ms(u, i, &ms)) return SDN_E_LAUNCH;
    const Op& o = p->ops[i];
    int r = 0;
    for (; r < n; ++r) if (strcmp(rows[r].kernel, o.label) == 0) break;
    if (r == n) {
      if (n == max_rows) return SDN_E_INVALID;
      memset(&rows[r], 0, sizeof(rows[r]));
      snprintf(rows[r].kernel, sizeof(rows[r].kernel), "%s", o.label);
      ++n;
    }
    rows[r].launches += 1; rows[r].ms += ms; rows[r].flops += o.flops; rows[r].bytes += o.bytes;
  }
  return n;
}
```

### safe_denoiser_amd/csrc/sdn_plan_unet.hip

```cpp
#include <math.h>

#include "sdn_plan.h"

namespace sdn_plan {

void Builder::gemm_ln(const Act& x, int64_t rows, int N, int K, const std::string& wname, Ref w, Ref gamma, Ref beta, Ref bias,
                      Ref out, int act_, bool prepass) {
  const bool fresh = u->param_index.find(wname + "#ln") == u->param_index.end();
  Ref wf = derived(wname + "#ln", (int64_t)N * K * 2), c = derived(wname + "#ln_c", (int64_t)N * 4), d = derived(wname + "#ln_d", (int64_t)N * 4);
  if (fresh) u->fold_jobs.push_back({w.off, gamma.off, beta.off, bias.space == SP_NONE ? -1 : bias.off, wf.off, c.off, d.off, N, K});
  Act st;
  if (prepass) {
    st = act(rows, 2, 0, 0, 4);
    Op o; o.kind = OP_ROWSTATS; o.a = R(x); o.rows = rows; o.c1 = K; o.eps = 1e-5f; o.out = R(st);
    o.bytes = 2.0 * rows * K; snprintf(o.label, sizeof(o.label), "k_row_stats"); plan->ops.push_back(o);
  }
  Op o; o.kind = OP_GEMM; memset(&o.gd, 0, sizeof(o.gd));
  o.gd.M = (int)rows; o.gd.N = N; o.gd.K = K; o.gd.a_mode = SDN_A_PLAIN; o.gd.act = act_; o.gd.out_kind = SDN_OUT_BF16;
  o.a = R(x); o.w = wf; o.out = out; o.ln = 1; o.ln_c = c; o.ln_d = d; o.eps = 1e-5f;
  if (prepass) o.ln_stats = R(st);
  o.flops = 2.0 * (double)rows * N * K;
  o.bytes = 2.0 * ((double)rows * K + (double)N * K + (double)rows * (act_ == SDN_ACT_GEGLU ? N / 2 : N));
  { int t = sdn_gemm_pick_tile((int)rows, N, K, act_);
    if (t == 8 && N % 320 == 0) t = 10;
    snprintf(o.label, sizeof(o.label), "k_gemm<%d>/ln%d", t, prepass ? 2 : 1); }
  if (k320_next && !prepass && K == 320 && N % 320 == 0 && act_ == SDN_ACT_NONE && pending_cols.space == SP_NONE && kK320Ln) {
    o.k320 = 1;
    snprintf(o.label, sizeof(o.label), "k_gemm_k320/ln1");
  }
  k320_next = false;
  plan->ops.push_back(o);
  plan->flops += o.flops;
  if (prepass) drop(st);
}

Act Builder::resnet(const std::string& pfx, Act& x, Act* skip, int cout) {
  const int cin = x.C + (skip ? skip->C : 0);
  Ref n1g = param(pfx + ".norm1.weight", SDN_P_VEC_F32, cin, 0), n1b = param(pfx + ".norm1.bias", SDN_P_VEC_F32, cin, 0);
  Ref c1w = param(pfx + ".conv1.weight", SDN_P_CONV3X3, cout, 9 * cin), c1b = param(pfx + ".conv1.bias", SDN_P_VEC_F32, cout, 0);
  const int tcol = tproj_cursor; tproj_cursor += cout;
  Ref n2g = param(pfx + ".norm2.weight", SDN_P_VEC_F32, cout, 0), n2b = param(pfx + ".norm2.bias", SDN_P_VEC_F32, cout, 0);
  Ref c2w = param(pfx + ".conv2.weight", SDN_P_CONV3X3, cout, 9 * cout), c2b = param(pfx + ".conv2.bias", SDN_P_VEC_F32, cout, 0);
  const int64_t rows = (int64_t)B * x.hw;
  Act g1 = act(rows, cin, x.hw, x.side);
  groupnorm(x, skip, 1e-5f, 1, n1g, n1b, g1);
  Act h = act_gn(rows, cout, x.hw, x.side);
  want_stats(h);
  conv3x3(g1, cout, cout, c1w, c1b, R(h), 1, 0, Ref(), Ref{SP_WS, tproj.off + (int64_t)tcol * 4}, u->tproj_total);
  drop(g1);
  Act g2 = act(rows, cout, x.hw, x.side);
  groupnorm(h, nullptr, 1e-5f, 1, n2g, n2b, g2);
  drop(h);
  Act out = act_gn(rows, cout, x.hw, x.side);
  if (cin != cout) {
    Ref scw = param(pfx + ".conv_shortcut.weight", SDN_P_MAT, cout, cin), scb = param(pfx + ".conv_shortcut.bias", SDN_P_VEC_F32, cout, 0);
    Act sc = act(rows, cout, x.hw, x.side);
    gemm(rows, cout, cin, R(x), scw, scb, R(sc), SDN_ACT_NONE, Ref(), SDN_OUT_BF16, 0, skip ? R(*skip) : Ref(),
         skip ? x.C : 0);
    want_stats(out);
    res_pre_next = u->res_pre;
    conv3x3(g2, cout, cout, c2w, c2b, R(out), 1, 0, R(sc), Ref(), 0);
    drop(sc);
  } else {
    want_stats(out);
    res_pre_next = u->res_pre;
    conv3x3(g2, cout, cout, c2w, c2b, R(out), 1, 0, R(x), Ref(), 0);
  }
  drop(g2);
  return out;
}

Act Builder::transformer(const std::string& pfx, Act& x) {
  const int64_t bytes_full = (int64_t)B * x.hw * x.C * es;
  int nsub = 1;
  if (u->subbatch_bytes > 0)
    while (nsub < B && bytes_full / nsub > u->subbatch_bytes && B % (nsub * 2) == 0) nsub *= 2;
  Act out = nsub == 1 ? act_gn((int64_t)B * x.hw, x.C, x.hw, x.side) : act((int64_t)B * x.hw, x.C, x.hw, x.side);
  const int Bfull = B, Bs = B / nsub;
  for (int sb = 0; sb < nsub; ++sb) {
    B = Bs;
    Act xs = x, os = out;
    xs.off += (int64_t)sb * Bs * x.hw * x.C * es; os.off += (int64_t)sb * Bs * x.hw * x.C * es;
    transformer_body(pfx, xs, os, (int64_t)sb * Bs * u->cfg.text_len * u->cfg.cross_dim * es);
  }
  B = Bfull;
  return out;
}

void Builder::transformer_body(const std::string& pfx, Act& x, const Act& out, int64_t text_off, int rep,
                               const Act* x_full) {
  const int C = x.C, hw = x.hw, T = u->cfg.text_len, X = u->cfg.cross_dim;
  const int Bfull = B;
  B = Bfull / rep;
  int64_t rows = (int64_t)B * hw;
  const std::string tb = pfx + ".transformer_blocks.0";
  Ref ng = param(pfx + ".norm.weight", SDN_P_VEC_F32, C, 0), nb = param(pfx + ".norm.bias", SDN_P_VEC_F32, C, 0);
  Ref piw = param(pfx + ".proj_in.weight", SDN_P_MAT, C, C), pib = param(pfx + ".proj_in.bias", SDN_P_VEC_F32, C, 0);
  Ref l1g = param(tb + ".norm1.weight", SDN_P_VEC_F32, C, 0), l1b = param(tb + ".norm1.bias", SDN_P_VEC_F32, C, 0);
  Ref qkv = stacked({tb + ".attn1.to_q.weight", tb + ".attn1.to_k.weight", tb + ".attn1.to_v.weight"}, C, C);
  Ref o1w = param(tb + ".attn1.to_out.0.weight", SDN_P_MAT, C, C), o1b = param(tb + ".attn1.to_out.0.bias", SDN_P_VEC_F32, C, 0);
  Ref l2g = param(tb + ".norm2.weight", SDN_P_VEC_F32, C, 0), l2b = param(tb + ".norm2.bias", SDN_P_VEC_F32, C, 0);
  Ref q2w = param(tb + ".attn2.to_q.weight", SDN_P_MAT, C, C);
  Ref kv2 = stacked({tb + ".attn2.to_k.weight", tb + ".attn2.to_v.weight"}, C, X);
  Ref o2w = param(tb + ".attn2.to_out.0.weight", SDN_P_MAT, C, C), o2b = param(tb + ".attn2.to_out.0.bias", SDN_P_VEC_F32, C, 0);
  Ref l3g = param(tb + ".norm3.weight", SDN_P_VEC_F32, C, 0), l3b = param(tb + ".norm3.bias", SDN_P_VEC_F32, C, 0);
  Ref f1w = param(tb + ".ff.net.0.proj.weight", SDN_P_GEGLU_MAT, 8 * C, C), f1b = param(tb + ".ff.net.0.proj.bias", SDN_P_GEGLU_VEC, 8 * C, 0);
  Ref f2w = param(tb + ".ff.net.2.weight", SDN_P_MAT, C, 4 * C), f2b = param(tb + ".ff.net.2.bias", SDN_P_VEC_F32, C, 0);
  Ref pow_ = param(pfx + ".proj_out.weight", SDN_P_MAT, C, C), pob = param(pfx + ".proj_out.bias", SDN_P_VEC_F32, C, 0);

  Act gn = act(rows, C, hw, x.side);
  groupnorm(x, nullptr, 1e-6f, 0, ng, nb, gn);
  Act h = act(rows, C, hw, x.side);
  const bool k320 = u->gemm_k320 && C == 320 && es == 2 && !x3t && u->subbatch_bytes == 0;
  k320_next = k320;
  gemm(rows, C, C, R(gn), piw, pib, R(h));
  drop(gn);
  const bool fold12 = u->ln_fold && C <= 640, fold3 = u->ln_fold && C == 320;
  const int hdx = C / u->cfg.n_heads;
  const bool x3p_cross = x3t && u->x3_pairs && u->subbatch_bytes == 0 && (hdx == 40 || hdx == 80 || hdx == 160);
  Act ln;
  if (!fold12 || !fold3) ln = act(rows, C, hw, x.side);
  Act qkvb = act(rows, 3 * C, hw, x.side);
  k320_next = k320;
  if (fold12) {
    gemm_ln(h, rows, 3 * C, C, tb + ".attn1.to_q.weight", qkv, l1g, l1b, Ref(), R(qkvb), SDN_ACT_NONE, 3 * C > 960 || u->ln_prepass_all);
  } else {
    layernorm(h, l1g, l1b, ln);
    const int hd1 = C / u->cfg.n_heads;
    if (x3t && u->x3_pairs && (hd1 == 40 || hd1 == 80 || hd1 == 160) && (int64_t)hw * 6 * C * 2 < (1LL << 31)) pair_out_next = true;
    gemm(rows, 3 * C, C, R(ln), qkv, Ref(), R(qkvb));
  }
  Act at = act(rows, C, hw, x.side);
  attention(R(qkvb), Ref{SP_WS, qkvb.off + (int64_t)C * es}, Ref{SP_WS, qkvb.off + (int64_t)2 * C * es}, R(at), hw, hw, C,
            3 * C, 3 * C, 3 * C);
  drop(qkvb);
  Act h2 = act(rows, C, hw, x.side);
  res_pre_next = u->res_pre;
  k320_next = k320;
  gemm(rows, C, C, R(at), o1w, o1b, R(h2), SDN_ACT_NONE, R(h));
  drop(h);
  Act qb = act(rows, C, hw, x.side);
  k320_next = k320;
  if (fold12) {
    gemm_ln(h2, rows, C, C, tb + ".attn2.to_q.weight", q2w, l2g, l2b, Ref(), R(qb), SDN_ACT_NONE, u->ln_prepass_all != 0);
  } else {
    layernorm(h2, l2g, l2b, ln);
    if (x3p_cross) pair_out_next = true;
    gemm(rows, C, C, R(ln), q2w, Ref(), R(qb));
  }
  if (rep > 1) {
    if (ln.off >= 0) drop(ln);
    drop(at);
    B = Bfull; rows = (int64_t)B * hw;
    Act h2f = act(rows, C, hw, x.side), qbf = act(rows, C, hw, x.side);
    repeat(h2, h2f, rep); repeat(qb, qbf, rep);
    const bool q_is_pairs = pairs.count(qb.off) > 0;
    drop(h2); drop(qb);
    h2 = h2f; qb = qbf;
    if (q_is_pairs) pairs.insert(qb.off);
    if (!fold3) ln = act(rows, C, hw, x.side);
    at = act(rows, C, hw, x.side);
  }
  if (u->subbatch_bytes > 0) {
    Act kvb = act((int64_t)B * T, 2 * C);
    gemm((int64_t)B * T, 2 * C, X, Ref{SP_TEXT, text_off}, kv2, Ref(), R(kvb));
    attention(R(qb), R(kvb), Ref{SP_WS, kvb.off + (int64_t)C * es}, R(at), hw, T, C, C, 2 * C, 2 * C);
    drop(qb); drop(kvb);
  } else {
    const Ref kvr{SP_KV, kv_top};
    kv_top += Arena::up((int64_t)B * T * 2 * C * es);
    if (x3p_cross) { force_x3t_next = true; pair_out_next = true; }
    gemm((int64_t)B * T, 2 * C, X, Ref{SP_TEXT, text_off}, kv2, Ref(), kvr);
    plan->ops.back().text_kv = 1;
    attention(R(qb), kvr, Ref{SP_KV, kvr.off + (int64_t)C * es}, R(at), hw, T, C, C, 2 * C, 2 * C, x3p_cross);
    drop(qb);
  }
  Act h3 = act(rows, C, hw, x.side);
  res_pre_next = u->res_pre;
  k320_next = k320;
  gemm(rows, C, C, R(at), o2w, o2b, R(h3), SDN_ACT_NONE, R(h2));
  drop(h2); drop(at);
  if (fold3 && u->ff_fuse && u->ffn_fuse && C == 320) {
    if (ln.off >= 0) drop(ln);
    const std::string wname = tb + ".ff.net.0.proj.weight";
    const bool fresh1 = u->param_index.find(wname + "#ln") == u->param_index.end();
    Ref wf = derived(wname + "#ln", (int64_t)8 * C * C * 2), c1 = derived(wname + "#ln_c", (int64_t)8 * C * 4), d1 = derived(wname + "#ln_d", (int64_t)8 * C * 4);
    if (fresh1) u->fold_jobs.push_back({f1w.off, l3g.off, l3b.off, f1b.off, wf.off, c1.off, d1.off, 8 * C, C});
    const bool fresh2 = u->param_index.find(pfx + ".proj_out.weight#ff") == u->param_index.end();
    Ref wcat = derived(pfx + ".proj_out.weight#ff", (int64_t)C * 5 * C * 2), bcat = derived(pfx + ".proj_out.bias#ff", (int64_t)C * 4);
    if (fresh2) { sdn_unet::FoldJob j{f2w.off, pow_.off, f2b.off, pob.off, wcat.off, bcat.off, -1, C, 4 * C}; j.kind = 1; u->fold_jobs.push_back(j); }
    Act st;
    if (!u->ffn_own_stats) {
      st = act(rows, 2, 0, 0, 4);
      Op o; o.kind = OP_ROWSTATS; o.a = R(h3); o.rows = rows; o.c1 = C; o.eps = 1e-5f; o.out = R(st);
      o.bytes = 2.0 * rows * C; snprintf(o.label, sizeof(o.label), "k_row_stats"); plan->ops.push_back(o);
    }
    want_stats(out);
    Op o; o.kind = OP_FFN; o.a = R(h3); if (st.off >= 0) o.ln_stats = R(st); o.w = wf; o.ln_c = c1; o.ln_d = d1; o.a2 = wcat; o.bias = bcat;
    o.residual = R(rep > 1 ? *x_full : x); o.out = R(out); o.rows = rows; o.c1 = C;
    o.col = pending_cols; pending_cols = Ref();
    o.flops = 2.0 * (double)rows * ((double)8 * C * C + (double)C * 5 * C);
    o.bytes = 2.0 * ((double)rows * C * 3 + (double)8 * C * C + (double)5 * C * C);
    snprintf(o.label, sizeof(o.label), "k_ffn320");
    plan->ops.push_back(o);
    plan->flops += o.flops;
    if (st.off >= 0) drop(st);
    drop(h3);
    return;
  }
  Act ff = act(rows, 4 * C, hw, x.side);
  if (fold3) {
    gemm_ln(h3, rows, 8 * C, C, tb + ".ff.net.0.proj.weight", f1w, l3g, l3b, f1b, R(ff), SDN_ACT_GEGLU, !u->ffn_own_stats);
  } else {
    layernorm(h3, l3g, l3b, ln);
    gemm(rows, 8 * C, C, R(ln), f1w, f1b, R(ff), SDN_ACT_GEGLU);
  }
  if (ln.off >= 0) drop(ln);
  if (u->ff_fuse) {
    const bool fresh = u->param_index.find(pfx + ".proj_out.weight#ff") == u->param_index.end();
    Ref wcat = derived(pfx + ".proj_out.weight#ff", (int64_t)C * 5 * C * 2), bcat = derived(pfx + ".proj_out.bias#ff", (int64_t)C * 4);
    if (fresh) { sdn_unet::FoldJob j{f2w.off, pow_.off, f2b.off, pob.off, wcat.off, bcat.off, -1, C, 4 * C}; j.kind = 1; u->fold_jobs.push_back(j); }
    want_stats(out);
    res_pre_next = u->res_pre && C != 320;
    gemm(rows, C, 5 * C, R(ff), wcat, bcat, R(out), SDN_ACT_NONE, R(rep > 1 ? *x_full : x), SDN_OUT_BF16, 0, R(h3), 4 * C);
    drop(ff); drop(h3);
    return;
  }
  Act h4 = act(rows, C, hw, x.side);
  triple_out_next = x3t;
  gemm(rows, C, 4 * C, R(ff), f2w, f2b, R(h4), SDN_ACT_NONE, R(h3));
  drop(ff); drop(h3);
  want_stats(out);
  gemm(rows, C, C, R(h4), pow_, pob, R(out), SDN_ACT_NONE, R(rep > 1 ? *x_full : x));
  drop(h4);
}

std::vector<Builder::Res> Builder::enumerate_resnets() const {
  const sdn_unet_config& c = u->cfg;
  std::vector<Res> v;
  char buf[96];
  for (int i = 0; i < c.n_levels; ++i)
    for (int j = 0; j < c.layers_per_block; ++j) {
      snprintf(buf, sizeof(buf), "down_blocks.%d.resnets.%d", i, j);
      v.push_back({buf, c.block_out_channels[i]});
    }
  const int top = c.block_out_channels[c.n_levels - 1];
  v.push_back({"mid_block.resnets.0", top});
  v.push_back({"mid_block.resnets.1", top});
  for (int i = 0; i < c.n_levels; ++i)
    for (int j = 0; j <= c.layers_per_block; ++j) {
      snprintf(buf, sizeof(buf), "up_blocks.%d.resnets.%d", i, j);
      v.push_back({buf, c.block_out_channels[c.n_levels - 1 - i]});
    }
  return v;
}

void Builder::build() {
  const sdn_unet_config& c = u->cfg;
  const int S = c.sample_size, ch0 = c.block_out_channels[0], tdim = 4 * ch0;
  char buf[96];

  Ref l1w = param("time_embedding.linear_1.weight", SDN_P_MAT, tdim, ch0), l1b = param("time_embedding.linear_1.bias", SDN_P_VEC_F32, tdim, 0);
  Ref l2w = param("time_embedding.linear_2.weight", SDN_P_MAT, tdim, tdim), l2b = param("time_embedding.linear_2.bias", SDN_P_VEC_F32, tdim, 0);
  const std::vector<Res> rs = enumerate_resnets();
  int total = 0;
  Ref tpw, tpb;
  {
    int64_t expect = -1;
    for (size_t i = 0; i < rs.size(); ++i) {
      Ref r = param(rs[i].pfx + ".time_emb_proj.weight", SDN_P_MAT, rs[i].cout, tdim);
      if (i == 0) tpw = r; else if (r.off != expect) { fprintf(stderr, "libsdn: time_emb_proj not contiguous\n"); abort(); }
      expect = r.off + (int64_t)rs[i].cout * tdim * es;
      total += rs[i].cout;
    }
    expect = -1;
    for (size_t i = 0; i < rs.size(); ++i) {
      Ref r = param(rs[i].pfx + ".time_emb_proj.bias", SDN_P_VEC_F32, rs[i].cout, 0);
      if (i == 0) tpb = r; else if (r.off != expect) { fprintf(stderr, "libsdn: time_emb_proj bias not contiguous\n"); abort(); }
      expect = r.off + (int64_t)rs[i].cout * 4;
    }
  }
  u->tproj_total = total;
  gn_stats = Ref{SP_WS, arena.alloc((int64_t)B * 129 * 64 * 2 * 4)};
  plan->tscalar_off = arena.alloc(256);
  Act tsin = act(B, ch0);
  { Op o; o.kind = OP_TEMB; o.batch = B; o.c1 = ch0; o.out = R(tsin); snprintf(o.label, sizeof(o.label), "k_temb"); plan->ops.push_back(o); }
  x3t_hold = true;
  Act t1 = act(B, tdim);
  gemm(B, tdim, ch0, R(tsin), l1w, l1b, R(t1), SDN_ACT_SILU);
  drop(tsin);
  Act semb = act(B, tdim);
  gemm(B, tdim, tdim, R(t1), l2w, l2b, R(semb), SDN_ACT_SILU);
  drop(t1);
  Act tp = act(B, total, 0, 0, 4);
  tproj = R(tp);
  gemm(B, total, tdim, R(semb), tpw, tpb, R(tp), SDN_ACT_NONE, Ref(), SDN_OUT_F32);
  drop(semb);
  x3t_hold = false;

  Ref ciw = param("conv_in.weight", SDN_P_CONV3X3, ch0, 9 * c.in_channels), cib = param("conv_in.bias", SDN_P_VEC_F32, ch0, 0);
  const int rep = (c.latent_repeat > 1 && c.level_has_attn[0] && u->subbatch_bytes == 0) ? c.latent_repeat : 1;
  if (B % rep != 0) { plan->ws_bytes = -1; return; }
  const int Bfull = B, Bp = B / rep;
  Act hp = act((int64_t)Bp * S * S, ch0, S * S, S);
  { Op o; o.kind = OP_CONV_IN; o.batch = Bp; o.c1 = c.in_channels; o.c2 = ch0; o.hw = S; o.a = Ref{SP_IN, 0}; o.w = ciw; o.bias = cib; o.out = R(hp);
    o.flops = 2.0 * Bp * S * S * (double)ch0 * 9 * c.in_channels; o.bytes = (double)Bp * S * S * (4.0 * c.in_channels + 2.0 * ch0);
    snprintf(o.label, sizeof(o.label), "k_conv_in"); plan->ops.push_back(o);
    plan->flops += o.flops; }
  Act h = hp;
  if (rep > 1) { h = act((int64_t)B * S * S, ch0, S * S, S); repeat(hp, h, rep); }

  std::vector<Act> skips;
  skips.push_back(h);
  Act cur = h;
  bool cur_is_skip = true;

  for (int i = 0; i < c.n_levels; ++i) {
    const int cout = c.block_out_channels[i];
    for (int j = 0; j < c.layers_per_block; ++j) {
      snprintf(buf, sizeof(buf), "down_blocks.%d.resnets.%d", i, j);
      if (rep > 1 && i == 0 && j == 0) {
        B = Bp;
        Act rp = resnet(buf, hp, nullptr, cout);
        B = Bfull;
        drop(hp);
        Act rf = act((int64_t)B * rp.hw, cout, rp.hw, rp.side);
        repeat(rp, rf, rep);
        snprintf(buf, sizeof(buf), "down_blocks.%d.attentions.%d", i, j);
        Act t = act_gn((int64_t)B * rp.hw, cout, rp.hw, rp.side);
        transformer_body(buf, rp, t, 0, rep, &rf);
        drop(rp); drop(rf);
        cur = t; skips.push_back(cur); cur_is_skip = true;
        continue;
      }
      Act r = resnet(buf, cur, nullptr, cout);
      if (!cur_is_skip) drop(cur);
      cur = r; cur_is_skip = false;
      if (c.level_has_attn[i]) {
        snprintf(buf, sizeof(buf), "down_blocks.%d.attentions.%d", i, j);
        Act t = transformer(buf, cur);
        drop(cur);
        cur = t;
      }
      skips.push_back(cur); cur_is_skip = true;
    }
    if (i + 1 < c.n_levels) {
      snprintf(buf, sizeof(buf), "down_blocks.%d.downsamplers.0.conv", i);
      Ref w = param(std::string(buf) + ".weight", SDN_P_CONV3X3, cout, 9 * cout), bb = param(std::string(buf) + ".bias", SDN_P_VEC_F32, cout, 0);
      const int s2 = cur.side / 2;
      Act d = act_gn((int64_t)B * s2 * s2, cout, s2 * s2, s2);
      want_stats(d);
      conv3x3(cur, cout, cout, w, bb, R(d), 2, 0, Ref(), Ref(), 0);
      cur = d; skips.push_back(cur); cur_is_skip = true;
    }
  }
  {
    Act r = resnet("mid_block.resnets.0", cur, nullptr, cur.C);
    cur = r; cur_is_skip = false;
    Act t = transformer("mid_block.attentions.0", cur);
    drop(cur); cur = t;
    Act r2 = resnet("mid_block.resnets.1", cur, nullptr, cur.C);
    drop(cur); cur = r2;
  }
  for (int i = 0; i < c.n_levels; ++i) {
    const int lvl = c.n_levels - 1 - i, cout = c.block_out_channels[lvl];
    for (int j = 0; j <= c.layers_per_block; ++j) {
      Act skip = skips.back(); skips.pop_back();
      snprintf(buf, sizeof(buf), "up_blocks.%d.resnets.%d", i, j);
      Act r = resnet(buf, cur, &skip, cout);
      drop(cur); drop(skip);
      cur = r;
      if (c.level_has_attn[lvl]) {
        snprintf(buf, sizeof(buf), "up_blocks.%d.attentions.%d", i, j);
        Act t = transformer(buf, cur);
        drop(cur); cur = t;
      }
    }
    if (i + 1 < c.n_levels) {
      snprintf(buf, sizeof(buf), "up_blocks.%d.upsamplers.0.conv", i);
      Ref w = param(std::string(buf) + ".weight", SDN_P_CONV3X3, cout, 9 * cout), bb = param(std::string(buf) + ".bias", SDN_P_VEC_F32, cout, 0);
      const int s2 = cur.side * 2;
      Act up = act_gn((int64_t)B * s2 * s2, cout, s2 * s2, s2);
      want_stats(up);
      conv3x3(cur, cout, cout, w, bb, R(up), 1, 1, Ref(), Ref(), 0);
      drop(cur); cur = up;
    }
  }
  Ref og = param("conv_norm_out.weight", SDN_P_VEC_F32, ch0, 0), ob = param("conv_norm_out.bias", SDN_P_VEC_F32, ch0, 0);
  const int npad = 32;
  Ref cow = param("conv_out.weight", SDN_P_CONV3X3, c.out_channels, 9 * ch0, npad);
  Ref cob = param("conv_out.bias", SDN_P_VEC_F32, c.out_channels, 0, npad);
  Act g = act((int64_t)B * S * S, ch0, S * S, S);
  groupnorm(cur, nullptr, 1e-5f, 1, og, ob, g);
  drop(cur);
  conv3x3(g, c.out_channels, npad, cow, cob, Ref{SP_OUT, 0}, 1, 0, Ref(), Ref(), 0, SDN_OUT_F32_NCHW, c.out_channels);
  drop(g);
  finish_up4();
  plan->kv_base = Arena::up(arena.peak);
  plan->ws_bytes = plan_bad ? -1 : plan->kv_base + kv_top;
}

}
```

Before: 8.727 images/sec.

## Fuse groupnorm column statistics into conv_in and share them across latent repeats

Result: no change. 8.754 images/sec (median of 6 runs) (+0.3%).

```diff
diff --git a/include/sdn.h b/include/sdn.h
--- a/include/sdn.h
+++ b/include/sdn.h
@@ -167,6 +167,10 @@
                      int32_t h, int32_t wd, int32_t cout, void* out_nhwc, void* stream);
 int sdn_conv_in_f16(const float* latents_nchw, const void* w, const float* bias, int32_t batch, int32_t cin,
                     int32_t h, int32_t wd, int32_t cout, void* out_nhwc, void* stream);
+int sdn_conv_in_stats_bf16(const float* latents_nchw, const void* w, const float* bias, int32_t batch, int32_t cin,
+                           int32_t h, int32_t wd, int32_t cout, void* out_nhwc, float* cols, void* stream);
+int sdn_conv_in_stats_f16(const float* latents_nchw, const void* w, const float* bias, int32_t batch, int32_t cin,
+                          int32_t h, int32_t wd, int32_t cout, void* out_nhwc, float* cols, void* stream);
 
 int sdn_timestep_embed_bf16(float timestep, int32_t batch, int32_t dim, void* out, void* stream);
 int sdn_timestep_embed_f16(float timestep, int32_t batch, int32_t dim, void* out, void* stream);
@@ -307,6 +311,12 @@
 int sdn_groupnorm_cols_f16(const void* x, const void* x2, int32_t batch, int32_t hw, int32_t c1, int32_t c2, int32_t groups,
                            float eps, int32_t silu, const float* gamma, const float* beta, void* out, float* stats_ws,
                            const float* cols1, const float* cols2, void* stream);
+int sdn_groupnorm_cols_mod_bf16(const void* x, const void* x2, int32_t batch, int32_t hw, int32_t c1, int32_t c2, int32_t groups,
+                                float eps, int32_t silu, const float* gamma, const float* beta, void* out, float* stats_ws,
+                                const float* cols1, const float* cols2, int32_t mod1, int32_t mod2, void* stream);
+int sdn_groupnorm_cols_mod_f16(const void* x, const void* x2, int32_t batch, int32_t hw, int32_t c1, int32_t c2, int32_t groups,
+                               float eps, int32_t silu, const float* gamma, const float* beta, void* out, float* stats_ws,
+                               const float* cols1, const float* cols2, int32_t mod1, int32_t mod2, void* stream);
 
 int sdn_gemm_splitk_bf16(const sdn_gemm_desc* d, const void* a, const void* a2, const void* w, const float* bias,
                          const float* rowbias, const float* rowgate, const void* residual, void* out, void* partials,
diff --git a/safe_denoiser_amd/_lib.py b/safe_denoiser_amd/_lib.py
--- a/safe_denoiser_amd/_lib.py
+++ b/safe_denoiser_amd/_lib.py
@@ -134,6 +134,10 @@
     "sdn_gemm_stats_f16": (C.c_int, [C.POINTER(GemmDesc), _vp, _vp, _vp, _vp, _vp, _vp, _vp, _vp, _vp]),
     "sdn_groupnorm_cols_bf16": (C.c_int, [_vp, _vp, _i32, _i32, _i32, _i32, _i32, _f32, _i32, _vp, _vp, _vp, _vp, _vp, _vp, _vp]),
     "sdn_groupnorm_cols_f16": (C.c_int, [_vp, _vp, _i32, _i32, _i32, _i32, _i32, _f32, _i32, _vp, _vp, _vp, _vp, _vp, _vp, _vp]),
+    "sdn_groupnorm_cols_mod_bf16": (C.c_int, [_vp, _vp, _i32, _i32, _i32, _i32, _i32, _f32, _i32, _vp, _vp, _vp, _vp, _vp, _vp, _i32, _i32, _vp]),
+    "sdn_groupnorm_cols_mod_f16": (C.c_int, [_vp, _vp, _i32, _i32, _i32, _i32, _i32, _f32, _i32, _vp, _vp, _vp, _vp, _vp, _vp, _i32, _i32, _vp]),
+    "sdn_conv_in_stats_bf16": (C.c_int, [_vp, _vp, _vp, _i32, _i32, _i32, _i32, _i32, _vp, _vp, _vp]),
+    "sdn_conv_in_stats_f16": (C.c_int, [_vp, _vp, _vp, _i32, _i32, _i32, _i32, _i32, _vp, _vp, _vp]),
     "sdn_gemm_splitk_bf16": (C.c_int, [C.POINTER(GemmDesc), _vp, _vp, _vp, _vp, _vp, _vp, _vp, _vp, _vp, _sz, _vp]),
     "sdn_gemm_splitk_f16": (C.c_int, [C.POINTER(GemmDesc), _vp, _vp, _vp, _vp, _vp, _vp, _vp, _vp, _vp, _sz, _vp]),
     "sdn_groupnorm_bf16": (C.c_int, [_vp, _vp, _i32, _i32, _i32, _i32, _i32, _f32, _i32, _vp, _vp, _vp, _vp, _vp]),
diff --git a/safe_denoiser_amd/csrc/sdn_norm.hip b/safe_denoiser_amd/csrc/sdn_norm.hip
--- a/safe_denoiser_amd/csrc/sdn_norm.hip
+++ b/safe_denoiser_amd/csrc/sdn_norm.hip
@@ -101,9 +101,10 @@
 
 __global__ void __launch_bounds__(256)
 k_gn_finalize_cols(const float* __restrict__ cols1, const float* __restrict__ cols2, int blocks_per_sample, int c1, int c2,
-                   int groups, float n, float eps, float* __restrict__ stats) {
+                   int groups, float n, float eps, float* __restrict__ stats, int mod1, int mod2) {
   __shared__ float red[8];
   const int C = c1 + c2, cpg = C / groups, b = blockIdx.x, gi = blockIdx.y;
+  const int b1 = mod1 > 0 ? b % mod1 : b, b2 = mod2 > 0 ? b % mod2 : b;
   const int total = blocks_per_sample * cpg;
   float s = 0.f, q = 0.f;
   for (int e = threadIdx.x; e < total; e += 256) {
@@ -111,7 +112,7 @@
     const bool second = c >= c1;
     const float* src = second ? cols2 : cols1;
     const int cw = second ? c2 : c1, cc = second ? c - c1 : c;
-    const float2 v = *reinterpret_cast<const float2*>(src + 2 * (((long)b * blocks_per_sample + t) * cw + cc));
+    const float2 v = *reinterpret_cast<const float2*>(src + 2 * (((long)(second ? b2 : b1) * blocks_per_sample + t) * cw + cc));
     s += v.x; q += v.y;
   }
   s = block_sum<4>(s, red);
@@ -343,6 +344,93 @@
 }
 
 template <typename T>
+__global__ void __launch_bounds__(THREADS)
+k_conv_in_cols(const float* __restrict__ lat, const unsigned short* __restrict__ w, const float* __restrict__ bias,
+               int B, int cin, int H, int W, int cout, int cpu, unsigned short* __restrict__ out, float* __restrict__ cols) {
+  extern __shared__ float wl[];
+  const int kk = 9 * cin;
+  unsigned short* stage = reinterpret_cast<unsigned short*>(wl + cout * kk);
+  for (int i = threadIdx.x; i < cout * kk; i += THREADS) {
+    const int co = i / kk, k = i - co * kk;
+    wl[((k * 2 + ((co >> 2) & 1)) * (cout / 8) + (co >> 3)) * 4 + (co & 3)] = T::to_f(w[i]);
+  }
+  __syncthreads();
+  constexpr int PX = 4, RG = 8;
+  const int cchunks = cout / 8, cgroups = cchunks / cpu, HW = H * W, sw = cpu * 8;
+  const int units = (B * HW / 128) * cgroups;
+  const int c = threadIdx.x % cpu, q = threadIdx.x / cpu;
+  for (int un = blockIdx.x; un < units; un += gridDim.x) {
+    const int blk = un / cgroups, cg = un - blk * cgroups;
+    if (q < 128 / PX) {
+      const int cc = cg * cpu + c;
+      const int pix = blk * 128 + q * PX;
+      const int b = pix / HW, rem = pix - b * HW;
+      const int yh = rem / W, x0 = rem - yh * W;
+      float acc[PX][8];
+      {
+        const float4 b0 = *reinterpret_cast<const float4*>(bias + cc * 8), b1 = *reinterpret_cast<const float4*>(bias + cc * 8 + 4);
+#pragma unroll
+        for (int p = 0; p < PX; ++p) {
+          acc[p][0] = b0.x; acc[p][1] = b0.y; acc[p][2] = b0.z; acc[p][3] = b0.w;
+          acc[p][4] = b1.x; acc[p][5] = b1.y; acc[p][6] = b1.z; acc[p][7] = b1.w;
+        }
+      }
+      const float* lb = lat + (long)b * cin * HW;
+      for (int ci = 0; ci < cin; ++ci) {
+        float v[3][PX + 2];
+#pragma unroll
+        for (int ty = 0; ty < 3; ++ty)
+#pragma unroll
+          for (int tx = 0; tx < PX + 2; ++tx) {
+            const int iy = yh + ty - 1, ix = x0 + tx - 1;
+            const bool ok = iy >= 0 && iy < H && ix >= 0 && ix < W;
+            const float t = lb[((long)ci * H + min(max(iy, 0), H - 1)) * W + min(max(ix, 0), W - 1)];
+            v[ty][tx] = ok ? t : 0.f;
+          }
+#pragma unroll
+        for (int tap = 0; tap < 9; ++tap) {
+          const float4 w0 = *reinterpret_cast<const float4*>(&wl[(((tap * cin + ci) * 2 + 0) * cchunks + cc) * 4]);
+          const float4 w1 = *reinterpret_cast<const float4*>(&wl[(((tap * cin + ci) * 2 + 1) * cchunks + cc) * 4]);
+#pragma unroll
+          for (int p = 0; p < PX; ++p) {
+            const float x = v[tap / 3][tap % 3 + p];
+            acc[p][0] = fmaf(x, w0.x, acc[p][0]); acc[p][1] = fmaf(x, w0.y, acc[p][1]);
+            acc[p][2] = fmaf(x, w0.z, acc[p][2]); acc[p][3] = fmaf(x, w0.w, acc[p][3]);
+            acc[p][4] = fmaf(x, w1.x, acc[p][4]); acc[p][5] = fmaf(x, w1.y, acc[p][5]);
+            acc[p][6] = fmaf(x, w1.z, acc[p][6]); acc[p][7] = fmaf(x, w1.w, acc[p][7]);
+          }
+        }
+      }
+#pragma unroll
+      for (int p = 0; p < PX; ++p) {
+        const u32x4 pk = pack8<T>(acc[p]);
+        *reinterpret_cast<u32x4*>(out + (long)(pix + p) * cout + cc * 8) = pk;
+        *reinterpret_cast<u32x4*>(stage + (q * PX + p) * sw + c * 8) = pk;
+      }
+    }
+    __syncthreads();
+    if (threadIdx.x < RG * cpu) {
+      const int rg = threadIdx.x / cpu, c2 = threadIdx.x - rg * cpu;
+      float cs[8] = {0.f, 0.f, 0.f, 0.f, 0.f, 0.f, 0.f, 0.f}, cq[8] = {0.f, 0.f, 0.f, 0.f, 0.f, 0.f, 0.f, 0.f};
+      for (int r = rg; r < 128; r += RG) {
+        float f[8];
+        unpack8<T>(*reinterpret_cast<const u32x4*>(stage + r * sw + c2 * 8), f);
+#pragma unroll
+        for (int k = 0; k < 8; ++k) { cs[k] += f[k]; cq[k] = fmaf(f[k], f[k], cq[k]); }
+      }
+#pragma unroll
+      for (int k = 0; k < 8; ++k) {
+        float ts = 0.f, tq = 0.f;
+#pragma unroll
+        for (int g = 0; g < RG; ++g) { ts += __shfl(cs[k], g * cpu + c2); tq += __shfl(cq[k], g * cpu + c2); }
+        if (rg == 0) *reinterpret_cast<float2*>(cols + 2 * ((long)blk * cout + (cg * cpu + c2) * 8 + k)) = make_float2(ts, tq);
+      }
+    }
+    __syncthreads();
+  }
+}
+
+template <typename T>
 __global__ void k_temb(float t_val, const float* __restrict__ t_dev, int B, int dim, unsigned short* __restrict__ out) {
   const float t = t_dev ? *t_dev : t_val;
   const int half = dim / 2;
@@ -362,7 +450,7 @@
 template <typename T>
 int groupnorm_impl(const void* x, const void* x2, int32_t batch, int32_t hw, int32_t c1, int32_t c2, int32_t groups,
                    float eps, int32_t silu, const float* gamma, const float* beta, void* out, float* stats_ws,
-                   void* stream, const float* cols1 = nullptr, const float* cols2 = nullptr) {
+                   void* stream, const float* cols1 = nullptr, const float* cols2 = nullptr, int mod1 = 0, int mod2 = 0) {
   if (!x || !gamma || !beta || !out || !stats_ws || batch < 0 || hw <= 0 || c1 <= 0 || c2 < 0 || groups <= 0 ||
       groups > 64)
     return SDN_E_INVALID;
@@ -385,10 +473,10 @@
   const size_t lds = (size_t)rt * C * 2 * sizeof(float);
   if (lds > 64 * 1024) return SDN_E_INVALID;
   if (cols1) {
-    if ((hw & 127) || (c2 > 0 && !cols2)) return SDN_E_INVALID;
+    if ((hw & 127) || (c2 > 0 && !cols2) || mod1 < 0 || mod2 < 0 || (c2 == 0 && mod2)) return SDN_E_INVALID;
     record_norm_launch({2, T::kDtype, 0, 0, 0, 0, 0, 0, 0, 0, 1, 0});
     hipLaunchKernelGGL(k_gn_finalize_cols, dim3(batch, groups), dim3(256), 0, st, cols1, cols2, hw / 128, c1, c2, groups,
-                       (float)hw * (float)(C / groups), eps, stats_ws);
+                       (float)hw * (float)(C / groups), eps, stats_ws, mod1, mod2);
   } else {
     float* partials = stats_ws + (size_t)batch * groups * 2;
     record_norm_launch({1, T::kDtype, 0, 0, nch, ct, ntiles, rows_per_tile, 0, 0, 0, 0});
@@ -463,10 +551,22 @@
 
 template <typename T>
 int conv_in_impl(const float* lat, const void* w, const float* bias, int32_t batch, int32_t cin, int32_t h, int32_t wd,
-                 int32_t cout, void* out, void* stream) {
+                 int32_t cout, void* out, void* stream, float* cols = nullptr) {
   if (!lat || !w || !bias || !out || batch < 0 || cin <= 0 || cin > 16 || h <= 0 || wd <= 0 || cout <= 0 ||
       (cout & 7) || !al16(out))
     return SDN_E_INVALID;
+  if (cols) {
+    if (((long)h * wd) % 128 != 0 || (wd & 3) || (reinterpret_cast<uintptr_t>(cols) & 7)) return SDN_E_INVALID;
+    if (batch == 0) return SDN_OK;
+    const int cch = cout / 8;
+    const int cpu = cch % 8 == 0 ? 8 : (cch % 4 == 0 ? 4 : (cch % 2 == 0 ? 2 : 1));
+    const size_t lds = (size_t)cout * 9 * cin * sizeof(float) + (size_t)128 * cpu * 8 * 2;
+    if (lds > 64 * 1024 || (long)batch * h * wd >= (1L << 31) / 16) return SDN_E_INVALID;
+    const long units = (long)batch * h * wd / 128 * (cch / cpu);
+    hipLaunchKernelGGL((k_conv_in_cols<T>), dim3((unsigned)(units < 2048 ? units : 2048)), dim3(THREADS), lds, (hipStream_t)stream, lat,
+                       (const unsigned short*)w, bias, batch, cin, h, wd, cout, cpu, (unsigned short*)out, cols);
+    return sdn_launch_status();
+  }
   if (batch == 0) return SDN_OK;
   int chunk = (int)((64 * 1024) / ((size_t)9 * cin * sizeof(float))) & ~7;
   if (chunk < 8) return SDN_E_INVALID;
@@ -547,6 +647,14 @@
     if (!cols1) return SDN_E_INVALID;                                                                                   \
     return groupnorm_impl<T>(x, x2, batch, hw, c1, c2, groups, eps, silu, gamma, beta, out, stats_ws, stream, cols1,    \
                              cols2);                                                                                    \
+  }                                                                                                                     \
+  extern "C" int sdn_groupnorm_cols_mod_##SUF(const void* x, const void* x2, int32_t batch, int32_t hw, int32_t c1,     \
+                                              int32_t c2, int32_t groups, float eps, int32_t silu, const float* gamma,  \
+                                              const float* beta, void* out, float* stats_ws, const float* cols1,        \
+                                              const float* cols2, int32_t mod1, int32_t mod2, void* stream) {           \
+    if (!cols1) return SDN_E_INVALID;                                                                                   \
+    return groupnorm_impl<T>(x, x2, batch, hw, c1, c2, groups, eps, silu, gamma, beta, out, stats_ws, stream, cols1,    \
+                             cols2, mod1, mod2);                                                                        \
   }                                                                                                                     \
   extern "C" int sdn_layernorm_##SUF(const void* x, int64_t rows, int32_t c, float eps, const float* gamma,            \
                                      const float* beta, void* out, void* stream) {                                      \
@@ -565,6 +673,11 @@
                                    int32_t h, int32_t wd, int32_t cout, void* out, void* stream) {                      \
     return conv_in_impl<T>(lat, w, bias, batch, cin, h, wd, cout, out, stream);                                         \
   }                                                                                                                     \
+  extern "C" int sdn_conv_in_stats_##SUF(const float* lat, const void* w, const float* bias, int32_t batch, int32_t cin, \
+                                         int32_t h, int32_t wd, int32_t cout, void* out, float* cols, void* stream) {    \
+    if (!cols) return SDN_E_INVALID;                                                                                    \
+    return conv_in_impl<T>(lat, w, bias, batch, cin, h, wd, cout, out, stream, cols);                                   \
+  }                                                                                                                     \
   extern "C" int sdn_timestep_embed_##SUF(float timestep, int32_t batch, int32_t dim, void* out, void* stream) {       \
     return temb_impl<T>(timestep, batch, dim, out, stream);                                                             \
   }
diff --git a/safe_denoiser_amd/csrc/sdn_plan.h b/safe_denoiser_amd/csrc/sdn_plan.h
--- a/safe_denoiser_amd/csrc/sdn_plan.h
+++ b/safe_denoiser_amd/csrc/sdn_plan.h
@@ -54,6 +54,7 @@
   Ref a, a2, w, bias, rowbias, rowgate, residual, out, aux;
   Ref q2, k2, v2, out2;
   Ref col, cols1, cols2;
+  int cols_mod1 = 0, cols_mod2 = 0;
   Ref ln_c, ln_d, ln_stats;
   int ln = 0;
   int text_kv = 0;
@@ -120,6 +121,7 @@
   int64_t off = -1, bytes = 0; int C = 0, hw = 0, side = 0;
   int64_t content = 0;
   int64_t st_off = -1, st_bytes = 0;
+  int st_mod = 0;
 };
 
 struct Plan {
@@ -168,6 +170,7 @@
   bool gemm_k320 = true;
   bool x3_expand = true;
   bool split_k = false;
+  bool gn_producer_stats = true;
   bool conv_up4 = true;
   struct GraphKey {
     int batch; const void *w, *lat, *text, *pooled, *out, *ws;
@@ -252,7 +255,8 @@
                Ref rowbias, int ld_rowbias, int out_kind = SDN_OUT_BF16, int n_valid = 0, int asym_pad = 0);
   void groupnorm(const Act& x, const Act* x2, float eps, int silu, Ref gamma, Ref beta, const Act& out);
   void layernorm(const Act& x, Ref gamma, Ref beta, const Act& out);
-  void repeat(const Act& in, const Act& out, int rep);
+  void repeat(Act& in, Act& out, int rep);
+  bool producer_stats() const { return u->gn_producer_stats && u->kind == UNET && es == 2; }
   void attention(Ref q, Ref k, Ref v, Ref out, int nq, int nk, int C, int ldq, int ldk, int ldv, bool kv_pairs = false);
 
   void gemm_ln(const Act& x, int64_t rows, int N, int K, const std::string& wname, Ref w, Ref gamma, Ref beta, Ref bias,
diff --git a/safe_denoiser_amd/csrc/sdn_plan_api.hip b/safe_denoiser_amd/csrc/sdn_plan_api.hip
--- a/safe_denoiser_amd/csrc/sdn_plan_api.hip
+++ b/safe_denoiser_amd/csrc/sdn_plan_api.hip
@@ -352,6 +352,10 @@
 
 void sdn_debug_set_gemm_k320(sdn_unet* u, int on) { if (u && u->gemm_k320 != (on != 0)) set_plan_toggle(u, &sdn_unet::gemm_k320, on != 0); }
 
+void sdn_debug_set_gn_producer_stats(sdn_unet* u, int on) {
+  if (u && u->kind == UNET && u->dtype() < 2 && u->gn_producer_stats != (on != 0)) set_plan_toggle(u, &sdn_unet::gn_producer_stats, on != 0);
+}
+
 void sdn_debug_set_ln_fold(sdn_unet* u, int on) { if (u) set_plan_toggle(u, &sdn_unet::ln_fold, on != 0); }
 
 void sdn_debug_set_ln_prepass_all(sdn_unet* u, int on) { if (u) set_plan_toggle(u, &sdn_unet::ln_prepass_all, on); }
diff --git a/safe_denoiser_amd/csrc/sdn_plan_core.hip b/safe_denoiser_amd/csrc/sdn_plan_core.hip
--- a/safe_denoiser_amd/csrc/sdn_plan_core.hip
+++ b/safe_denoiser_amd/csrc/sdn_plan_core.hip
@@ -70,7 +70,7 @@
 }
 void Builder::drop(Act& t) {
   if (t.off >= 0) { arena.release(t.off, t.bytes); tri.erase(t.off); pairs.erase(t.off); }
-  if (t.st_off >= 0) arena.release(t.st_off, t.st_bytes);
+  if (t.st_off >= 0 && t.st_bytes > 0) arena.release(t.st_off, t.st_bytes);
   t.off = -1; t.st_off = -1;
 }
 
@@ -230,8 +230,8 @@
   o.silu = silu; o.w = gamma; o.bias = beta; o.out = R(out); o.aux = gn_stats;
   if (x3t) { o.tri_out = 1; tri.insert(out.off); }
   if (x.st_off >= 0 && (!x2 || x2->st_off >= 0)) {
-    o.cols1 = Ref{SP_WS, x.st_off};
-    if (x2) o.cols2 = Ref{SP_WS, x2->st_off};
+    o.cols1 = Ref{SP_WS, x.st_off}; o.cols_mod1 = x.st_mod;
+    if (x2) { o.cols2 = Ref{SP_WS, x2->st_off}; o.cols_mod2 = x2->st_mod; }
   }
   o.bytes = 2.0 * (o.cols1.space != SP_NONE ? 2.0 : 3.0) * (double)B * x.hw * (o.c1 + o.c2);
   snprintf(o.label, sizeof(o.label), o.cols1.space != SP_NONE ? "k_gn_apply" : "k_gn_stats+apply");
@@ -245,7 +245,11 @@
   snprintf(o.label, sizeof(o.label), "k_layernorm");
   plan->ops.push_back(o);
 }
-void Builder::repeat(const Act& in, const Act& out, int rep) {
+void Builder::repeat(Act& in, Act& out, int rep) {
+  if (producer_stats() && in.st_off >= 0 && in.st_bytes > 0 && out.st_off < 0) {
+    out.st_off = in.st_off; out.st_bytes = in.st_bytes; out.st_mod = B / rep;
+    in.st_bytes = 0;
+  }
   Op o; o.kind = OP_REPEAT; o.a = R(in); o.out = R(out); o.rows = in.content; o.c1 = rep;
   o.bytes = (double)in.content * (1 + rep);
   snprintf(o.label, sizeof(o.label), "k_repeat");
diff --git a/safe_denoiser_amd/csrc/sdn_plan_run.hip b/safe_denoiser_amd/csrc/sdn_plan_run.hip
--- a/safe_denoiser_amd/csrc/sdn_plan_run.hip
+++ b/safe_denoiser_amd/csrc/sdn_plan_run.hip
@@ -165,6 +165,11 @@
       else rc = (f16 ? sdn_timestep_embed_f16 : sdn_timestep_embed_bf16)(P.scalar, o.batch, o.c1, (void*)P(o.out), stream);
       break;
     case OP_CONV_IN:
+      if (o.col.space != SP_NONE) {
+        rc = (f16 ? sdn_conv_in_stats_f16 : sdn_conv_in_stats_bf16)((const float*)P(o.a), P(o.w), (const float*)P(o.bias), o.batch, o.c1, o.hw,
+                                                                    o.hw, o.c2, (void*)P(o.out), (float*)P(o.col), stream);
+        break;
+      }
       rc = (f16 ? sdn_conv_in_f16 : sdn_conv_in_bf16)((const float*)P(o.a), P(o.w), (const float*)P(o.bias), o.batch, o.c1, o.hw, o.hw, o.c2,
                             (void*)P(o.out), stream);
       break;
@@ -227,10 +232,10 @@
       break;
     case OP_GN:
       if (o.cols1.space != SP_NONE) {
-        rc = (f16 ? sdn_groupnorm_cols_f16 : sdn_groupnorm_cols_bf16)(P(o.a), P(o.a2), o.batch, o.hw, o.c1, o.c2, o.groups, o.eps,
-                                                                      o.silu, (const float*)P(o.w), (const float*)P(o.bias),
-                                                                      (void*)P(o.out), (float*)P(o.aux), (const float*)P(o.cols1),
-                                                                      (const float*)P(o.cols2), stream);
+        rc = (f16 ? sdn_groupnorm_cols_mod_f16 : sdn_groupnorm_cols_mod_bf16)(P(o.a), P(o.a2), o.batch, o.hw, o.c1, o.c2, o.groups, o.eps,
+                                                                              o.silu, (const float*)P(o.w), (const float*)P(o.bias),
+                                                                              (void*)P(o.out), (float*)P(o.aux), (const float*)P(o.cols1),
+                                                                              (const float*)P(o.cols2), o.cols_mod1, o.cols_mod2, stream);
         break;
       }
       rc = (f16 ? sdn_groupnorm_f16 : sdn_groupnorm_bf16)(P(o.a), P(o.a2), o.batch, o.hw, o.c1, o.c2, o.groups, o.eps, o.silu,
@@ -399,6 +404,15 @@
   return n;
 }
 
+extern "C" int sdn_debug_plan_labels(sdn_unet* u, int batch, char* labels, int max_ops) {
+  if (!u || !labels || batch <= 0) return -1;
+  Plan* p = get_plan(u, batch);
+  if (p->ws_bytes < 0) return -1;
+  int n = 0;
+  for (size_t i = 0; i < p->ops.size() && n < max_ops; ++i, ++n) memcpy(labels + n * 24, p->ops[i].label, 24);
+  return n;
+}
+
 extern "C" int sdn_unet_profile_read(sdn_unet* u, sdn_profile_row* rows, int32_t max_rows) {
   if (!u || !rows || max_rows <= 0 || u->profiled_batch <= 0) return SDN_E_INVALID;
   Plan* p = get_plan(u, u->profiled_batch, u->profiled_n);
diff --git a/safe_denoiser_amd/csrc/sdn_plan_unet.hip b/safe_denoiser_amd/csrc/sdn_plan_unet.hip
--- a/safe_denoiser_amd/csrc/sdn_plan_unet.hip
+++ b/safe_denoiser_amd/csrc/sdn_plan_unet.hip
@@ -302,8 +302,11 @@
   const int rep = (c.latent_repeat > 1 && c.level_has_attn[0] && u->subbatch_bytes == 0) ? c.latent_repeat : 1;
   if (B % rep != 0) { plan->ws_bytes = -1; return; }
   const int Bfull = B, Bp = B / rep;
-  Act hp = act((int64_t)Bp * S * S, ch0, S * S, S);
+  const int ci_cpu = ch0 % 64 == 0 ? 8 : (ch0 % 32 == 0 ? 4 : (ch0 % 16 == 0 ? 2 : 1));
+  const bool ci_stats = producer_stats() && S % 4 == 0 && (int64_t)ch0 * 36 * c.in_channels + 2048 * ci_cpu <= 64 * 1024;
+  Act hp = ci_stats ? act_gn((int64_t)Bp * S * S, ch0, S * S, S) : act((int64_t)Bp * S * S, ch0, S * S, S);
   { Op o; o.kind = OP_CONV_IN; o.batch = Bp; o.c1 = c.in_channels; o.c2 = ch0; o.hw = S; o.a = Ref{SP_IN, 0}; o.w = ciw; o.bias = cib; o.out = R(hp);
+    if (hp.st_off >= 0) o.col = Ref{SP_WS, hp.st_off};
     o.flops = 2.0 * Bp * S * S * (double)ch0 * 9 * c.in_channels; o.bytes = (double)Bp * S * S * (4.0 * c.in_channels + 2.0 * ch0);
     snprintf(o.label, sizeof(o.label), "k_conv_in"); plan->ops.push_back(o);
     plan->flops += o.flops; }
```
